# massquantity/Ftrl-FFM

Hardware: AMD Instinct MI355X
Metric: train samples/sec + logloss, FFM f=39 k=16 (higher is better)
Workload: dtype f32; 1 GPU; FFM n_fields=39 n_factors=16 nnz=39, Zipf(1.1) ids, block=8192 rows, n_feats=32999967 (247.1 GB of w,n,z per GPU), warm state, reference default hyper-parameters, 64 distinct blocks streamed from page-locked host memory (H2D in the timed region); workload_key=c5|zipf|warm|rows=8192|n_feats=32999967|shards=1, n_feats=32999967, n_feats_reduced_to_fit=False, n_blocks=64

## Files before the change

ftrl-ffm_amd/csrc/engine.hip:

```cpp
#include <hip/hip_runtime.h>

#include <rocprim/device/device_radix_sort.hpp>
#include <rocprim/iterator/counting_iterator.hpp>

#include <algorithm>
#include <cmath>
#include <atomic>
#include <chrono>
#include <condition_variable>
#include <deque>
#include <functional>
#include <memory>
#include <optional>
#include <mutex>
#include <thread>
#include <cstdio>
#include <cstdlib>
#include <cstring>
#include <new>
#include <string>
#include <vector>

#include "../../include/ffm_engine.h"
#include "engine_types.h"
// ... 370 lines not shown
    }
  }
  int submit(std::function<int()> job) {
    if (prof_on) return job();
    {
      std::lock_guard<std::mutex> lock(wmu);
      if (!worker.joinable()) worker = std::thread([this] { worker_main(); });
      wjobs.push_back(std::move(job));
    }
    wcv_job.notify_one();
    return 0;
  }
  int worker_error() {
    if (worker_rc == 0) return 0;
    const int rc = worker_rc;
    worker_rc = 0;
    return fail(rc, "staging thread: " + worker_msg);
  }
  int drain() {
    std::unique_lock<std::mutex> lock(wmu);
    wcv_done.wait(lock, [&] { return wjobs.empty() && !wbusy; });
    return worker_error();
  }
  int wait_issued(int64_t seq) {
    std::unique_lock<std::mutex> lock(wmu);
    wcv_done.wait(lock, [&] { return staged_issued >= seq || (wjobs.empty() && !wbusy); });
    return worker_error();
  }
  void stop_worker() {
    {
      std::lock_guard<std::mutex> lock(wmu);
      wstop = true;
    }
    wcv_job.notify_all();
    if (worker.joinable()) worker.join();
  }
  bool prof_on = false;
  int prof_only = -1;
  std::vector<ProfRec> prof;
  std::vector<hipEvent_t> event_pool;

  template <typename T>
  int alloc(T **p, size_t count) {
    void *q = nullptr;
    if (count == 0) count = 1;
    hipError_t err = hipMalloc(&q, count * sizeof(T));
    if (err != hipSuccess)
      return fail(FFM_E_NOMEM, "hipMalloc of " + std::to_string(count * sizeof(T)) +
                                   " bytes failed: " + hipGetErrorString(err));
    allocs.push_back(q);
    *p = static_cast<T *>(q);
    return FFM_OK;
  }
  template <typename T>
  int grow(T **p, size_t *cap, size_t need) {
    if (*p && *cap >= need) return FFM_OK;
    T *q = nullptr;
    if (int rc = alloc(&q, need)) return rc;
    if (*p) {
      allocs.erase(std::find(allocs.begin(), allocs.end(), static_cast<void *>(*p)));
      (void)hipFree(*p);
    }
    *p = q;
    *cap = need;
    return FFM_OK;
  }

  hipEvent_t get_event() {
    if (!event_pool.empty()) {
      hipEvent_t e = event_pool.back();
      event_pool.pop_back();
      return e;
    }
    hipEvent_t e = nullptr;
    if (hipEventCreate(&e) != hipSuccess) return nullptr;
    return e;
  }
  void prof_begin(int kid, hipStream_t st) {
    prof_skip = !prof_on || (prof_only >= 0 && kid != prof_only);
    if (prof_skip) return;
    ProfRec r{kid, get_event(), get_event()};
    if (!r.e0 || !r.e1) {
      if (r.e0) event_pool.push_back(r.e0);
      if (r.e1) event_pool.push_back(r.e1);
      prof_skip = true;
      return;
    }
    (void)hipEventRecord(r.e0, st);
    prof.push_back(r);
  }
  bool prof_skip = true;
  void prof_end(hipStream_t st) {
    if (prof_skip) return;
    (void)hipEventRecord(prof.back().e1, st);
  }
};

static inline bool serving(const ffm_engine *e) { return e->m.lat_fmt != SERVE_NONE; }
static int serve_refuse(const char *what) {
  return fail(FFM_E_UNSUPPORTED, std::string("a serving engine holds no accumulators: ") + what + " needs a training engine");
}
#define SERVE_REFUSE(e, what) do { if ((e) && serving(e)) return serve_refuse(what); } while (0)

#define LAUNCH_ON(e, st, kid, kernel, grid, block, shmem, ...)                   \
  do {                                                                           \
    (e)->prof_begin(kid, st);                                                    \
    hipLaunchKernelGGL(kernel, dim3(grid), dim3(block), shmem, st, __VA_ARGS__); \
    (e)->prof_end(st);                                                           \
  } while (0)
#define LAUNCH(e, kid, kernel, grid, block, shmem, ...) \
  LAUNCH_ON(e, (e)->stream, kid, kernel, grid, block, shmem, __VA_ARGS__)

static inline int cdiv(int a, int b) { return (a + b - 1) / b; }
static inline int loss_grid(int n_rows) { return std::max(1, std::min(kLossParts, cdiv(n_rows, 1024))); }

static int tile_nf(const ffm_engine *e) {
  const int k = e->m.n_factors, spc = k <= 64 ? 64 / k : 1;
  return spc > 8 ? 4 : spc > 4 ? 2 : 1;
}
static bool flat_pays(const ffm_engine *e, int span4) {
  if (e->m.n_shards <= 1 || span4 <= 0) return false;
  const int lanes = (span4 + 63) / 64 * 64;
  return span4 * 6 < lanes * 5;
}

extern "C" {

int ffm_engine_abi_version(void) { return FFM_ENGINE_ABI_VERSION; }
int ffm_engine_block_segment(void) { return ftrl_dev::kSeg; }
const char *ffm_engine_last_error(void) { return g_last_error.c_str(); }

void ffm_engine_default_config(ffm_engine_config *cfg) {
  if (!cfg) return;
  std::memset(cfg, 0, sizeof(*cfg));
  cfg->model_type = FFM_MODEL_FFM;
  cfg->n_feats = 10000;
  cfg->n_fields = 8;
  cfg->n_factors = 16;
  cfg->w_alpha = 1e-4f;
  cfg->w_beta = 1.0f;
  cfg->w_l1 = 0.1f;
  cfg->w_l2 = 5.0f;
  cfg->init_mean = 0.0f;
  cfg->init_stddev = 0.02f;
  cfg->seed = 42;
  cfg->max_batch_rows = 8192;
  cfg->max_batch_nnz = 8192 * 64;
  cfg->device_id = 0;
  cfg->n_shards = 1;
  cfg->shard_rank = 0;
}

int64_t ffm_engine_row_len(const ffm_engine *e) { return e ? e->logical_len : 0; }

void ffm_engine_destroy(ffm_engine *e) {
  if (!e) return;
  (void)hipSetDevice(e->cfg.device_id);
  e->stop_worker();
  if (e->prep) (void)hipStreamSynchronize(e->prep);
  if (e->aux3) (void)hipStreamSynchronize(e->aux3);
  if (e->ev_fork) (void)hipEventDestroy(e->ev_fork);
  if (e->ev_fork2) (void)hipEventDestroy(e->ev_fork2);
  if (e->ev_join) (void)hipEventDestroy(e->ev_join);
  if (e->ev_join2) (void)hipEventDestroy(e->ev_join2);
  if (e->aux4) (void)hipStreamDestroy(e->aux4);
  if (e->stream) (void)hipStreamSynchronize(e->stream);
  for (auto &r : e->prof) { (void)hipEventDestroy(r.e0); (void)hipEventDestroy(r.e1); }
  for (auto ev : e->event_pool) (void)hipEventDestroy(ev);
  for (auto &sl : e->slots) {
    if (sl.pinned) (void)hipHostFree(sl.pinned);
    if (sl.pinned_w) (void)hipHostFree(sl.pinned_w);
    if (sl.ev_copied) (void)hipEventDestroy(sl.ev_copied);
    if (sl.ev_trained) (void)hipEventDestroy(sl.ev_trained);
  }
  for (void *p : e->allocs) (void)hipFree(p);
  for (int i = 0; i < ffm_engine::kSets; i++) {
    if (e->ev_grouped[i]) (void)hipEventDestroy(e->ev_grouped[i]);
    if (e->ev_set_free[i]) (void)hipEventDestroy(e->ev_set_free[i]);
    if (e->ev_row_done[i]) (void)hipEventDestroy(e->ev_row_done[i]);
  }
  if (e->h_pulled) (void)hipHostFree(e->h_pulled);
  if (e->h_scored) (void)hipHostFree(e->h_scored);
  if (e->h_super) (void)hipHostFree(e->h_super);
  if (e->prep) (void)hipStreamDestroy(e->prep);

  if (e->aux3) (void)hipStreamDestroy(e->aux3);
  if (e->own_stream && e->stream) (void)hipStreamDestroy(e->stream);
  delete e;
}

#include "engine_create.h"

static int eval_launch_pending(ffm_engine *e);
static int serve_vec_transfer(ffm_engine *e, float *host, bool to_host);
static int serve_rows_vec_transfer(ffm_engine *e, int nf, float *host, bool to_host);

int ffm_engine_init_weights_host(uint64_t seed, float init_mean, float init_stddev, int32_t latent,
                                 int64_t first, int64_t count, float *out) {
  if (first < 0 || count < 0 || (count > 0 && !out)) return fail(FFM_E_INVALID, "bad range or null output");
  for (int64_t j = 0; j < count; j++)
    out[j] = ftrl_rng::init_weight(seed, latent ? 1 : 0, static_cast<uint64_t>(first + j), init_mean, init_stddev);
  return FFM_OK;
}

int ffm_engine_fill_state(ffm_engine *e, uint64_t seed, float n_lo, float n_hi, float z_stddev) {
  if (!e) return fail(FFM_E_INVALID, "null engine");
  SERVE_REFUSE(e, "ffm_engine_fill_state");
  if (!(n_lo >= 0.0f) || !(n_hi >= n_lo)) return fail(FFM_E_INVALID, "need 0 <= n_lo <= n_hi");
  HIP_TRY(hipSetDevice(e->cfg.device_id));
  if (int rc_e = eval_launch_pending(e)) return rc_e;
  hipLaunchKernelGGL(fill_state_kernel, dim3(2048), dim3(256), 0, e->stream, e->m, e->logical_len, seed, n_lo, n_hi, z_stddev);
  HIP_TRY(hipGetLastError());
  HIP_TRY(hipStreamSynchronize(e->stream));
  return FFM_OK;
}

int ffm_engine_eval_sigmoid(ffm_engine *e, int32_t n, const float *x, float *y) {
  if (!e || n < 0 || (n > 0 && (!x || !y))) return fail(FFM_E_INVALID, "bad argument");
  HIP_TRY(hipSetDevice(e->cfg.device_id));
  const int chunk = static_cast<int>(std::min<int64_t>(e->stage_floats / 2, 1 << 22));
  for (int off = 0; off < n; off += chunk) {
    const int c = std::min(chunk, n - off);
    HIP_TRY(hipMemcpyAsync(e->d_stage, x + off, sizeof(float) * c, hipMemcpyHostToDevice, e->stream));
    hipLaunchKernelGGL(sigmoid_eval_kernel, dim3(cdiv(c, 256)), dim3(256), 0, e->stream, c, e->d_stage, e->d_stage + chunk);
    HIP_TRY(hipMemcpyAsync(y + off, e->d_stage + chunk, sizeof(float) * c, hipMemcpyDeviceToHost, e->stream));
    HIP_TRY(hipStreamSynchronize(e->stream));
  }
  return FFM_OK;
}

static int check_device_errors(ffm_engine *e) {
  int flags = 0;
  if (int rc_e = eval_launch_pending(e)) return rc_e;
  if (int rc_w = e->drain()) return rc_w;
  for (int i = 0; i < e->n_staged; i++) HIP_TRY(hipEventSynchronize(e->slots[e->staged[i]].ev_copied));
  HIP_TRY(hipMemcpyAsync(&flags, e->d_err, sizeof(int), hipMemcpyDeviceToHost, e->stream));
  HIP_TRY(hipStreamSynchronize(e->stream));
  if (flags) HIP_TRY(hipMemsetAsync(e->d_err, 0, sizeof(int), e->stream));
  if (flags & ERR_ROW_TOO_LONG)
    return fail(FFM_E_CAPACITY, "a row has more entries than max_row_nnz: its block was not trained "
                                "(outputs of that block are NaN)");
  if (flags & ERR_FIELD_MAP)
    return fail(FFM_E_INVALID, "an entry's feature id lies outside its field's id range (field_start): "
                               "its block was not trained");
  if (flags & ERR_SORT_BARRIER)
    return fail(FFM_E_DEVICE, "the grouping's one-launch sort could not get its workgroups on the device "
                              "together (grid barrier timed out): its block was not trained; FFM_OWN_SORT=0 "
                              "selects the library sort");
  if (flags) return fail(FFM_E_DEVICE, "device error flags " + std::to_string(flags));
  return FFM_OK;
}

int ffm_engine_sync(ffm_engine *e) {
  if (!e) return fail(FFM_E_INVALID, "null engine");
  HIP_TRY(hipSetDevice(e->cfg.device_id));
  return check_device_errors(e);
}

int ffm_engine_check_errors(ffm_engine *e) { return ffm_engine_sync(e); }

void *ffm_engine_stream(ffm_engine *e) { return e ? static_cast<void *>(e->stream) : nullptr; }

int32_t ffm_engine_default_batch_ramp(float w_alpha) {
  if (!(w_alpha > 1e-3f)) return 32;
  const double r = 32.0 * std::pow(8.0, std::log10(static_cast<double>(w_alpha) / 1e-3));
  return static_cast<int32_t>(std::min(r, 1048576.0) + 0.5);
}

int ffm_engine_shard_plan(int32_t n_fields, int32_t n_shards, int32_t field_map, int32_t *pair_owner,
                          int32_t *lin_owner, int32_t *bias_owner) {
  if (n_fields <= 0 || n_shards <= 0) return fail(FFM_E_INVALID, "n_fields and n_shards must be positive");
  const ShardPlan p = make_shard_plan(n_fields, n_shards, field_map != 0);
  for (int fa = 0; fa < n_fields; fa++)
    for (int fb = 0; fb < n_fields; fb++) {
      int owner = -1, count = 0;
      for (int r = 0; r < n_shards; r++)
        if (p.owns(r, fa, fb)) { owner = r; count++; }
      if (count != 1 || !p.owns(owner, fb, fa)) return fail(FFM_E_UNSUPPORTED, "no field-pair partition for this shape");
      if (pair_owner) pair_owner[static_cast<size_t>(fa) * n_fields + fb] = owner;
    }
  if (lin_owner) for (int f = 0; f < n_fields; f++) lin_owner[f] = p.lin_owner[f];
  if (bias_owner) *bias_owner = p.bias_owner;
  return FFM_OK;
}

#include "engine_state.h"
#include "engine_hash.h"
#include "engine_step.h"
#include "engine_stage.h"
#include "engine_refresh.h"
#include "engine_serve.h"
#include "engine_profile.h"
#include "engine_metrics.h"
#include "engine_keyed.h"
#include "engine_sketch.h"
#include "engine_ablate.h"
}

#include "engine_group.h"
```

ftrl-ffm_amd/csrc/engine_create.h:

```cpp

static int hash_ids_check(int32_t model_type, int32_t n_feats, int32_t n_fields, const int32_t *field_start);
static int serve_create_check(const ffm_engine_config *cfg);

struct Switches {
  bool hash_ids = false;
  int metrics = 0;
  char row_refresh = 0;
  std::optional<bool> serial, super_wait, prep_after_row, pull_after_row, eval_defer_off, predict_waves, few_stage, own_sort;
  std::optional<int> update_split, update_order, wide_max_nnz, grid_pull, grid_push, grid_hot, grid_small, grid_walk, grid_giant;
  std::optional<int> row_threads, row_park, row_park_budget, row_hold, super_min;
  std::optional<int> range_sort;
};
extern "C++" {
template <typename T, typename U>
static void take(T &dst, const std::optional<U> &v) { if (v) dst = static_cast<T>(*v); }
template <typename Fn>
static int lds_opt_in(Fn *kernel, size_t bytes) {
  if (kernel) HIP_TRY(hipFuncSetAttribute(reinterpret_cast<const void *>(kernel), hipFuncAttributeMaxDynamicSharedMemorySize, static_cast<int>(bytes)));
  return FFM_OK;
}
template <typename T>
static int upload(ffm_engine *e, const std::vector<T> &host, T **dev) {
  if (int rc = e->alloc(dev, host.size())) return rc;
  HIP_TRY(hipMemcpy(*dev, host.data(), host.size() * sizeof(T), hipMemcpyHostToDevice));
  return FFM_OK;
}
}

static Switches read_switches() {
  Switches sw;
  if (const char *sv = std::getenv("FFM_ENGINE_HASH_IDS")) sw.hash_ids = sv[0] == '1';
  if (const char *sv = std::getenv("FFM_ENGINE_METRICS")) sw.metrics = std::atoi(sv) & 3;
  if (const char *sv = std::getenv("FFM_ENGINE_ROW_REFRESH")) sw.row_refresh = sv[0];
  if (const char *sv = std::getenv("FFM_ENGINE_SERIAL")) sw.serial = sv[0] == '1';
  if (const char *sv = std::getenv("FFM_UPDATE_SPLIT")) sw.update_split = std::atoi(sv);
  if (const char *sv = std::getenv("FFM_UPDATE_ORDER")) {
    const int o = std::atoi(sv);
    const int d0 = o % 10, d1 = o / 10 % 10, d2 = o / 100;
    if (o >= 0 && d2 <= 2 && d0 <= 2 && d1 <= 2 && d0 != d1 && d0 != d2 && d1 != d2) sw.update_order = o;
  }
  if (const char *sv = std::getenv("FFM_SUPER_WAIT")) sw.super_wait = sv[0] != '0';
  if (const char *sv = std::getenv("FFM_PREP_AFTER_ROW")) sw.prep_after_row = sv[0] == '1';
  if (const char *sv = std::getenv("FFM_PULL_AFTER_ROW")) sw.pull_after_row = sv[0] == '1';
  if (const char *sv = std::getenv("FFM_EVAL_DEFER")) sw.eval_defer_off = sv[0] == '0';
  if (const char *sv = std::getenv("FFM_PREDICT_WAVE")) sw.predict_waves = std::atoi(sv) != 0;
  if (const char *sv = std::getenv("FFM_WIDE_NNZ")) sw.wide_max_nnz = std::atoi(sv);
  if (const char *sv = std::getenv("FFM_GRID_PULL")) sw.grid_pull = std::max(1, std::atoi(sv));
  if (const char *sv = std::getenv("FFM_GRID_PUSH")) sw.grid_push = std::min(24, std::max(1, std::atoi(sv)));
  if (const char *sv = std::getenv("FFM_GRID_HOT")) sw.grid_hot = std::max(1, std::atoi(sv));
  if (const char *sv = std::getenv("FFM_GRID_SMALL")) sw.grid_small = std::max(1, std::atoi(sv));
  if (const char *sv = std::getenv("FFM_GRID_WALK")) sw.grid_walk = std::max(1, std::atoi(sv));
  if (const char *sv = std::getenv("FFM_GRID_GIANT")) sw.grid_giant = std::max(1, std::atoi(sv));
  if (const char *sv = std::getenv("FFM_ROW_THREADS")) sw.row_threads = std::max(64, std::min(kRowMaxThreads, std::atoi(sv) / 64 * 64));
  if (const char *sv = std::getenv("FFM_ROW_PARK")) sw.row_park = std::atoi(sv);
  if (const char *sv = std::getenv("FFM_ROW_PARK_BUDGET")) sw.row_park_budget = std::atoi(sv);
  if (const char *sv = std::getenv("FFM_ROW_HOLD")) sw.row_hold = std::max(0, std::atoi(sv));
  if (const char *sv = std::getenv("FFM_SUPER_MIN")) sw.super_min = std::max(kGiantMin, std::atoi(sv));
  if (const char *sv = std::getenv("FFM_FEW_STAGE")) sw.few_stage = sv[0] != '0';
  if (const char *sv = std::getenv("FFM_OWN_SORT")) sw.own_sort = std::atoi(sv) != 0;
  if (const char *sv = std::getenv("FFM_RANGE_SORT")) sw.range_sort = std::atoi(sv);
  return sw;
}

static int check_config(const ffm_engine_config *cfg, bool hash_ids) {
  if (cfg->model_type < FFM_MODEL_LR || cfg->model_type > FFM_MODEL_FFM)
    return fail(FFM_E_INVALID, "invalid model_type, expect LR(0), FM(1) or FFM(2)");
  if (cfg->n_feats <= 0) return fail(FFM_E_INVALID, "n_feats must be positive");
  if (cfg->model_type == FFM_MODEL_FFM && cfg->n_fields <= 0)
    return fail(FFM_E_INVALID, "n_fields must be positive for FFM");
  if (cfg->model_type != FFM_MODEL_LR && cfg->n_factors <= 0)
    return fail(FFM_E_INVALID, "n_factors must be positive for FM/FFM");
  if (cfg->model_type == FFM_MODEL_FM && cfg->n_factors > kTermsCap)
    return fail(FFM_E_UNSUPPORTED, "FM n_factors above 2048 is not supported");
  if (cfg->max_batch_rows <= 0 || cfg->max_batch_nnz <= 0)
    return fail(FFM_E_INVALID, "max_batch_rows / max_batch_nnz must be positive");
  if (cfg->n_shards < 1 || cfg->shard_rank < 0 || cfg->shard_rank >= cfg->n_shards)
    return fail(FFM_E_INVALID, "invalid n_shards / shard_rank");
  if (cfg->n_shards > 1 && cfg->model_type != FFM_MODEL_FFM)
    return fail(FFM_E_UNSUPPORTED, "field-pair sharding applies to FFM only");
  if (cfg->n_shards > 1 && cfg->n_fields > 64)
    return fail(FFM_E_UNSUPPORTED, "field-pair sharding supports up to 64 fields");
  if (cfg->flags & (FFM_FLAG_SERVE_F32 | FFM_FLAG_SERVE_F16))
    if (int rc_s = serve_create_check(cfg)) return rc_s;
  if (hash_ids)
    if (int rc_h = hash_ids_check(cfg->model_type, cfg->n_feats, cfg->n_fields, cfg->field_start)) return rc_h;
  int n_dev = 0;
  if (hipGetDeviceCount(&n_dev) != hipSuccess || n_dev <= 0)
    return fail(FFM_E_DEVICE, "no HIP device available (this library has no CPU fallback)");
  if (cfg->device_id < 0 || cfg->device_id >= n_dev)
    return fail(FFM_E_INVALID, "device_id out of range");
  HIP_TRY(hipSetDevice(cfg->device_id));
  return FFM_OK;
}

static void apply_switches(ffm_engine *e, const Switches &sw) {
  const ffm_engine_config *cfg = &e->cfg;
  take(e->serial, sw.serial);
  take(e->update_split, sw.update_split);
  take(e->update_order, sw.update_order);
  take(e->super_wait, sw.super_wait);
  take(e->prep_after_row, sw.prep_after_row);
  take(e->eval_defer_off, sw.eval_defer_off);
  take(e->predict_waves, sw.predict_waves);
  take(e->wide_max_nnz, sw.wide_max_nnz);
  take(e->grid_pull, sw.grid_pull);
  take(e->grid_push, sw.grid_push);
  take(e->grid_hot, sw.grid_hot);
  take(e->grid_small, sw.grid_small);
  take(e->grid_walk, sw.grid_walk);
  take(e->grid_giant, sw.grid_giant);
  if (cfg->n_shards > 1) e->row_threads = 64;
  take(e->row_threads, sw.row_threads);
  take(e->row_park, sw.row_park);
  take(e->row_park_budget, sw.row_park_budget);
  take(e->row_hold, sw.row_hold);
  if (cfg->n_shards > 1) e->grid_single = 1152;
  if (cfg->n_shards > 1 && !sw.grid_small) e->grid_small = 1024;
  const char rr = sw.row_refresh;
  const int64_t per = cfg->n_factors % 4 == 0 ? static_cast<int64_t>(cfg->n_fields) * cfg->n_factors / 4
                                              : static_cast<int64_t>(cfg->n_fields) * cfg->n_factors;
  e->pre_refresh = cfg->model_type == FFM_MODEL_FFM && cfg->n_fields <= 64 &&
                   static_cast<int64_t>(e->max_nnz) * per < (1ll << 31) && rr != '1';
  if (rr == '0') e->refresh_mode = 1;
  if (rr == '2') e->refresh_mode = 2;
  if (rr == '3') e->refresh_mode = 3;
}

static int plan_model(ffm_engine *e, const Switches &sw, ShardPlan *plan) {
  const ffm_engine_config *cfg = &e->cfg;
  ModelDev &m = e->m;
  m.type = cfg->model_type;
  m.n_feats = cfg->n_feats;
  m.n_fields = cfg->model_type == FFM_MODEL_FFM ? cfg->n_fields : 1;
  m.n_factors = cfg->model_type == FFM_MODEL_LR ? 0 : cfg->n_factors;
  e->logical_len = cfg->model_type == FFM_MODEL_FFM ? cfg->n_fields * cfg->n_factors
                   : cfg->model_type == FFM_MODEL_FM ? cfg->n_factors : 0;
  m.n_shards = cfg->n_shards;
  m.shard_rank = cfg->shard_rank;
  m.bias_own = 1;
  m.huge_min = kHugeMin;
  m.giant_min = cfg->model_type == FFM_MODEL_FM ? kFmGiantMin : kGiantMin;
  m.range_len = cfg->model_type == FFM_MODEL_FM ? kFmRange : kRange;
  m.huge_min = std::min(m.huge_min, m.giant_min - 1);
  m.super_min = kSuperMin;
  take(m.super_min, sw.super_min);
  m.few_stage = 1;
  take(m.few_stage, sw.few_stage);
  m.lat_fmt = (cfg->flags & FFM_FLAG_SERVE_F32 ? SERVE_F32 : 0) | (cfg->flags & FFM_FLAG_SERVE_F16 ? SERVE_F16 : 0);
  m.rec_slots = m.n_fields;
  e->n_records = cfg->n_feats;
  const bool compact = cfg->n_shards > 1 && cfg->field_start != nullptr;
  if (cfg->field_start && cfg->model_type == FFM_MODEL_FFM) {
    e->field_start.assign(cfg->field_start, cfg->field_start + cfg->n_fields + 1);
    bool ok = e->field_start[0] == 0 && e->field_start[cfg->n_fields] == cfg->n_feats;
    for (int f = 0; f < cfg->n_fields; f++) ok = ok && e->field_start[f] <= e->field_start[f + 1];
    if (!ok) return fail(FFM_E_INVALID, "field_start must ascend from 0 to n_feats");
  }
  if (cfg->n_shards > 1) {
    *plan = make_shard_plan(cfg->n_fields, cfg->n_shards, compact);
    m.bias_own = plan->bias_owner == cfg->shard_rank ? 1 : 0;
    if (compact) {
      int widest = 1;
      for (int f = 0; f < cfg->n_fields; f++) widest = std::max(widest, plan->n(cfg->shard_rank, f));
      m.rec_slots = widest;
      e->n_records = 0;
      for (int f = 0; f < cfg->n_fields; f++)
        if (plan->n(cfg->shard_rank, f) > 0) e->n_records += e->field_start[f + 1] - e->field_start[f];
      if (e->n_records == 0) e->n_records = 1;
    }
  }
  m.row_len = cfg->model_type == FFM_MODEL_FFM ? m.rec_slots * cfg->n_factors
              : cfg->model_type == FFM_MODEL_FM ? cfg->n_factors : 0;
  m.h = Hyper{cfg->w_alpha, cfg->w_beta, cfg->w_l1, cfg->w_l2, 1.0f / cfg->w_alpha, 0,
              (cfg->flags & FFM_FLAG_LEARN) ? 1 : 0};
  if (static_cast<int64_t>(cfg->n_fields) * cfg->n_factors > (1 << 24))
    return fail(FFM_E_UNSUPPORTED, "n_fields*n_factors too large");
  if (static_cast<int64_t>(cfg->max_batch_nnz) / (kSmallMax + 1) * ((m.row_len + 7) / 8 + 1) >= (1ll << 31))
    return fail(FFM_E_UNSUPPORTED, "max_batch_nnz * row_len too large for 32-bit work-item ids");
  return FFM_OK;
}

static int create_streams(ffm_engine *e) {
  if (e->cfg.stream) {
    e->stream = static_cast<hipStream_t>(e->cfg.stream);
  } else {
    HIP_TRY(hipStreamCreateWithFlags(&e->stream, hipStreamNonBlocking));
    e->own_stream = true;
  }
  HIP_TRY(hipStreamCreateWithFlags(&e->aux3, hipStreamNonBlocking));
  HIP_TRY(hipStreamCreateWithFlags(&e->aux4, hipStreamNonBlocking));
  HIP_TRY(hipStreamCreateWithFlags(&e->prep, hipStreamNonBlocking));
  for (hipEvent_t *ev : {&e->ev_fork, &e->ev_fork2, &e->ev_join, &e->ev_join2})
    HIP_TRY(hipEventCreateWithFlags(ev, hipEventDisableTiming));
  for (int i = 0; i < ffm_engine::kSets; i++) {
    HIP_TRY(hipEventCreateWithFlags(&e->ev_grouped[i], hipEventDisableTiming));
    HIP_TRY(hipEventCreateWithFlags(&e->ev_set_free[i], hipEventDisableTiming));
    HIP_TRY(hipEventCreateWithFlags(&e->ev_row_done[i], hipEventDisableTiming));
  }
  return FFM_OK;
}

static int alloc_model(ffm_engine *e, const ShardPlan &plan) {
  const ffm_engine_config *cfg = &e->cfg;
  ModelDev &m = e->m;
  int rc;
  const size_t nf = static_cast<size_t>(cfg->n_feats);
  const size_t n_w = static_cast<size_t>(e->n_records) * static_cast<size_t>(m.row_len);
  const size_t n_lat = m.lat_fmt == SERVE_F16 ? n_w / 2 : m.lat_fmt == SERVE_F32 ? n_w : 3 * n_w;
  const size_t n_bias = serving(e) ? 1 : 4;
  if ((rc = e->alloc(&m.bias3, n_bias))) return rc;
  HIP_TRY(hipMemsetAsync(m.bias3, 0, n_bias * sizeof(float), e->stream));
  for (float **lin : {&m.lin_n, &m.lin_z, &m.lin_w}) {
    if (serving(e) && lin != &m.lin_w) continue;
    if ((rc = e->alloc(lin, nf))) return rc;
    HIP_TRY(hipMemsetAsync(*lin, 0, nf * sizeof(float), e->stream));
  }
  if ((rc = e->alloc(&m.lat, n_lat))) return rc;
  if (n_lat) HIP_TRY(hipMemsetAsync(m.lat, 0, n_lat * sizeof(float), e->stream));
  if (m.type == FFM_MODEL_FFM && m.n_fields <= 64) {
    std::vector<unsigned long long> own(m.n_fields, 0ull);
    for (int fa = 0; fa < m.n_fields; fa++)
      for (int fb = 0; fb < m.n_fields; fb++)
        if (m.n_shards <= 1 || plan.owns(m.shard_rank, fa, fb)) own[fa] |= 1ull << fb;
    if ((rc = upload(e, own, &e->d_ownmask))) return rc;
    m.ownmask = e->d_ownmask;
  }
  if (m.n_shards > 1) {
    const bool compact = cfg->field_start != nullptr;
    const int F = m.n_fields, r = m.shard_rank;
    std::vector<int> lo(F), cnt(F), lin(F);
    std::vector<long long> base(F, -1);
    long long next = 0;
    for (int f = 0; f < F; f++) {
      lo[f] = plan.lo(r, f);
      cnt[f] = plan.n(r, f);
      lin[f] = plan.lin_owner[f] == r ? 1 : 0;
      if (compact && cnt[f] > 0) { base[f] = next; next += e->field_start[f + 1] - e->field_start[f]; }
    }
    int *d_lo = nullptr, *d_n = nullptr, *d_lin = nullptr;
    if ((rc = upload(e, lo, &d_lo)) || (rc = upload(e, cnt, &d_n)) || (rc = upload(e, lin, &d_lin))) return rc;
    m.own_lo = d_lo;
    m.own_n = d_n;
    m.lin_own = d_lin;
    e->lin_any = std::any_of(lin.begin(), lin.end(), [](int v) { return v != 0; });
    if (compact) {
      int *d_fs = nullptr;
      long long *d_base = nullptr;
      if ((rc = upload(e, e->field_start, &d_fs)) || (rc = upload(e, base, &d_base))) return rc;
      m.field_start = d_fs;
      m.rec_base = d_base;
    }
  }
  if (e->hash_ids) {
    e->hm = ftrl_hash::Map{nullptr, cfg->n_feats, m.n_fields, m.type == FFM_MODEL_FFM ? 1 : 0};
    if (!e->field_start.empty()) {
      if ((rc = upload(e, e->field_start, &e->d_hash_start))) return rc;
      e->hm.start = e->d_hash_start;
    }
  }
  return FFM_OK;
}

static int alloc_shared(ffm_engine *e, Scratch *shared) {
  const ffm_engine_config *cfg = &e->cfg;
  const ModelDev &m = e->m;
  Scratch &s = *shared;
  int rc;
  const size_t R = static_cast<size_t>(e->max_rows), E = static_cast<size_t>(e->max_nnz);
  const size_t max_segs = E / kSeg + E / kFmGiantMin + 2, rl = static_cast<size_t>(std::max(1, m.row_len));
  const bool lat_model = cfg->model_type != FFM_MODEL_LR, ffm_m = cfg->model_type == FFM_MODEL_FFM;
  const size_t chunks = !ffm_m ? 1 : cfg->n_factors <= 64
                            ? (static_cast<size_t>(m.rec_slots) + 64 / cfg->n_factors - 1) / (64 / cfg->n_factors)
                            : static_cast<size_t>(m.rec_slots) * ((cfg->n_factors + 63) / 64);
  if ((rc = e->alloc(&s.segP, lat_model ? max_segs * rl : 1)) || (rc = e->alloc(&s.segG, lat_model ? max_segs * rl : 1)) ||
      (rc = e->alloc(&s.segD, ffm_m ? max_segs * rl : 1)) || (rc = e->alloc(&s.segF, ffm_m ? max_segs * chunks * 3 : 1)) ||
      (rc = e->alloc(&s.gcap, ffm_m ? (E / kGiantMin + 2) * rl : 1)))
    return rc;
  if ((rc = e->alloc(&e->d_err, 1))) return rc;
  HIP_TRY(hipMemsetAsync(e->d_err, 0, sizeof(int), e->stream));
  s.err = e->d_err;
  if ((rc = e->alloc(&s.head, R * static_cast<size_t>(m.n_fields))) || (rc = e->alloc(&s.next, E)) ||
      (rc = e->alloc(&s.rowtab, R * static_cast<size_t>(m.n_fields))) || (rc = e->alloc(&s.logit, R)) ||
      (rc = e->alloc(&s.tg, R)) || (rc = e->alloc(&s.loss, R)) ||
      (rc = e->alloc(&s.svx, R * static_cast<size_t>(m.type == FFM_MODEL_FM ? m.n_factors : 1))))
    return rc;
  e->sort_bits = 1;
  while (e->sort_bits < 32 && (static_cast<uint64_t>(cfg->n_feats) >> e->sort_bits) != 0) e->sort_bits++;
  unsigned *no_key = nullptr;
  int *no_occ = nullptr;
  HIP_TRY(rocprim::radix_sort_pairs<GroupSortConfig>(nullptr, e->sort_tmp_bytes, no_key, no_key,
                                    rocprim::counting_iterator<int>(0), no_occ, E, 0u, e->sort_bits, e->stream));
  e->sort_tmp_bytes = std::max(e->sort_tmp_bytes, sort_scratch_bytes(E));
  HIP_TRY(hipHostMalloc(reinterpret_cast<void **>(&e->h_super), sizeof(int) * ffm_engine::kSets, hipHostMallocMapped));
  std::memset(e->h_super, 0, sizeof(int) * ffm_engine::kSets);
  HIP_TRY(hipHostGetDevicePointer(reinterpret_cast<void **>(&s.n_super), e->h_super, 0));
  hipLaunchKernelGGL(host_word_probe_kernel, dim3(1), dim3(64), 0, e->stream, s.n_super, ffm_engine::kSets);
  HIP_TRY(hipStreamSynchronize(e->stream));
  e->super_flag_ok = true;
  for (int si = 0; si < ffm_engine::kSets; si++) e->super_flag_ok = e->super_flag_ok && e->h_super[si] == 0x5eed + si;
  std::memset(e->h_super, 0, sizeof(int) * ffm_engine::kSets);
  if ((rc = e->alloc(&e->d_ids, static_cast<size_t>(ffm_engine::kIdsCap))) || (rc = e->alloc(&e->d_row_ptr, R + 1)) ||
      (rc = e->alloc(&e->d_field, E)) || (rc = e->alloc(&e->d_feat, E)) || (rc = e->alloc(&e->d_val, E)) ||
      (rc = e->alloc(&e->d_label, R)) || (rc = e->alloc(&e->d_out, R)) || (rc = e->alloc(&e->d_loss_sum, 2)) ||
      (rc = e->alloc(&e->d_loss_part, kLossParts + 1)))
    return rc;
  HIP_TRY(hipMemsetAsync(e->d_loss_part, 0, sizeof(double) * (kLossParts + 1), e->stream));
  e->stage_floats = 16 << 20;
  if (static_cast<int64_t>(e->logical_len) > e->stage_floats) e->stage_floats = e->logical_len;
  return e->alloc(&e->d_stage, static_cast<size_t>(e->stage_floats));
}

static int alloc_set(ffm_engine *e, int si, const Scratch &shared) {
  const ModelDev &m = e->m;
  Scratch &t = e->sc[si];
  t = shared;
  t.n_super = shared.n_super + si;
  int rc;
  const size_t R = static_cast<size_t>(e->max_rows), E = static_cast<size_t>(e->max_nnz);
  if ((rc = e->alloc(&t.key, E)) || (rc = e->alloc(&t.skey, E)) || (rc = e->alloc(&t.row_of, E)) ||
      (rc = e->alloc(&t.occ, E)) || (rc = e->alloc(&t.occ2, E)) || (rc = e->alloc(&t.udesc, E)) ||
      (rc = e->alloc(&t.small, E)) || (rc = e->alloc(&t.few, E)) || (rc = e->alloc(&t.sdesc, E)) ||
      (rc = e->alloc(&t.big, E)) || (rc = e->alloc(&t.huge, E)) || (rc = e->alloc(&t.giant, E / kChainMin + 1)) ||
      (rc = e->alloc(&t.gseg, E / kChainMin + 1)) || (rc = e->alloc(&t.grange, E / kFmRange + E / kFmGiantMin + 2)) ||
      (rc = e->alloc(&t.counters, kNumCounters)) || (rc = e->alloc(&t.occpos, E)) || (rc = e->alloc(&t.uflag, E)))
    return rc;
  if (m.type == FFM_MODEL_FFM && m.n_fields <= 64)
    if ((rc = e->alloc(&t.rowmask, 2 * R)) || (rc = e->alloc(&t.gmask, E)) || (rc = e->alloc(&t.cmask, E))) return rc;
  unsigned char *tmp = nullptr;
  if ((rc = e->alloc(&tmp, e->sort_tmp_bytes))) return rc;
  e->d_sort_tmp[si] = tmp;
  HIP_TRY(hipMemsetAsync(t.counters, 0, kNumCounters * sizeof(int), e->stream));
  return FFM_OK;
}

static int choose_sort(ffm_engine *e, const Switches &sw) {
  const ffm_engine_config *cfg = &e->cfg;
  ModelDev &m = e->m;
  const double per_row = e->max_rows > 0 ? static_cast<double>(e->max_nnz) / e->max_rows : 0.0;
  const double phase_us = static_cast<double>(e->max_nnz) * std::max(0.0, per_row - 1.0) * m.n_factors / 0.44e6;
  const bool ffm4 = m.type == FFM_MODEL_FFM && m.n_factors % 4 == 0;
  e->own_sort = !(ffm4 && phase_us / std::max(1, m.n_shards) >= 100.0);
  take(e->own_sort, sw.own_sort);
  const bool have = !e->field_start.empty(), forced = sw.range_sort.has_value();
  const bool quick = cfg->n_shards == 1 && static_cast<int64_t>(e->max_nnz) <= 16384ll * std::max(1, cfg->n_fields);
  const bool want = forced ? *sw.range_sort != 0 : (have && quick);
  if (want && (m.type == FFM_MODEL_FFM || forced)) {
    const int nr = have ? cfg->n_fields : (forced && *sw.range_sort > 1 ? std::min(1024, *sw.range_sort) : std::max(1, std::min(64, cfg->n_fields)));
    std::vector<int> st(static_cast<size_t>(nr) + 1);
    for (int f = 0; f <= nr; f++)
      st[f] = have ? e->field_start[f] : static_cast<int>(static_cast<int64_t>(cfg->n_feats) * f / nr);
    if (int rc = upload(e, st, &e->d_sort_start)) return rc;
    e->n_sort_ranges = nr;
    e->range_sort = true;
    if (have && m.type == FFM_MODEL_FFM) m.sort_start = e->d_sort_start;
    if (!sw.prep_after_row) e->prep_after_row = !e->own_sort;
    e->pull_after_row = e->prep_after_row && static_cast<int64_t>(e->max_nnz) * m.n_factors >= (1ll << 22);
    take(e->pull_after_row, sw.pull_after_row);
  }
  hipDeviceProp_t prop;
  HIP_TRY(hipGetDeviceProperties(&prop, cfg->device_id));
  int per_cu = 0;
  HIP_TRY(hipOccupancyMaxActiveBlocksPerMultiprocessor(&per_cu, group_sort_kernel, kSortThreads, 0));
  e->sort_grid_cap = std::max(1, per_cu * prop.multiProcessorCount);
  if (std::strncmp(prop.gcnArchName, "gfx950", 6) != 0 && std::strncmp(prop.gcnArchName, "gfx942", 6) != 0) e->own_sort = false;
  return FFM_OK;
}

static int read_verdict(ffm_engine *e, int *bad) {
  int *counters = e->sc[0].counters;
  HIP_TRY(hipMemcpyAsync(bad, counters, sizeof(int), hipMemcpyDeviceToHost, e->stream));
  HIP_TRY(hipStreamSynchronize(e->stream));
  HIP_TRY(hipMemsetAsync(counters, 0, kNumCounters * sizeof(int), e->stream));
  return FFM_OK;
}

static int prove_fast_math(ffm_engine *e) {
  const ffm_engine_config *cfg = &e->cfg;
  ModelDev &m = e->m;
  {
    static std::atomic<int> verdict[64];
    const int dev = cfg->device_id & 63;
    int bad = verdict[dev].load() < 0 ? 1 : 0;
    if (verdict[dev].load() == 0) {
      hipLaunchKernelGGL(verify_sqrt_fast_kernel, dim3(16384), dim3(256), 0, e->stream, e->sc[0].counters);
      if (int rc = read_verdict(e, &bad)) return rc;
      verdict[dev].store(bad ? -1 : 1);
    }
    if (bad)
      return fail(FFM_E_UNSUPPORTED, "this device's v_sqrt_f32 / v_rsq_f32 do not give the correctly rounded "
                                     "square root in the short sequence the kernels use (built and proven for gfx950)");
  }
  if (cfg->w_alpha >= 0x1p-30f && cfg->w_alpha <= 0x1p30f) {
    int bad = 0;
    Hyper probe = m.h;
    probe.fast_div = 1;
    hipLaunchKernelGGL(verify_div_alpha_kernel, dim3(1u << 17), dim3(256), 0, e->stream, probe, e->sc[0].counters);
    if (int rc = read_verdict(e, &bad)) return rc;
    m.h.fast_div = bad ? 0 : 1;
    m.h.fast_w = m.h.fast_div && cfg->w_beta >= 0x1p-40f && cfg->w_beta <= 0x1p40f ? 1 : 0;
  }
  return FFM_OK;
}

static int opt_in_lds(ffm_engine *e) {
  int rc;
  const size_t lds = row_lds_bytes(e->max_row_nnz, e->m.n_fields, kTermsCap);
  if (lds > 150 * 1024) return fail(FFM_E_UNSUPPORTED, "max_row_nnz too large for the 160 KB of LDS per workgroup");
  const size_t park_budget = static_cast<size_t>(std::max(0, e->row_park_budget));
  if (lds > 32 * 1024 || park_budget > 32 * 1024) {
    const size_t bytes = std::max(lds, park_budget);
    for (int train = 0; train < 2; train++) {
      if ((rc = lds_opt_in(fm_row_fn(train), bytes))) return rc;
      for (int vec4 = 0; vec4 < 2; vec4++)
        for (int whole = 0; whole < 2; whole++)
          for (int hold = 0; hold <= 8; hold++)
            if ((rc = lds_opt_in(ffm_row_fn<>(train, vec4, whole, hold), bytes)) ||
                (rc = lds_opt_in(ffm_row_fn<const float *>(train, vec4, whole, hold), bytes)))
              return rc;
    }
  }
  for (int nf = 1; nf <= 4; nf *= 2)
    for (int kinds = 1; kinds <= UPD_ALL; kinds++)
      for (int waves : {tile_waves(nf), kWideWaves})
        if ((rc = lds_opt_in(update_all_fn(nf, kinds, waves), tile_lds_bytes(nf, waves)))) return rc;
  return FFM_OK;
}

static int init_weights(ffm_engine *e) {
  const ffm_engine_config *cfg = &e->cfg;
  const bool skip = (cfg->flags & FFM_FLAG_SKIP_INIT) != 0;
  if (!skip && serving(e))
    hipLaunchKernelGGL(serve_init_kernel, dim3(2048), dim3(256), 0, e->stream, e->m, cfg->init_mean, cfg->init_stddev, cfg->seed);
  else if (!skip)
    hipLaunchKernelGGL(init_weights_kernel, dim3(2048), dim3(256), 0, e->stream, e->m, e->logical_len,
                       cfg->init_mean, cfg->init_stddev, cfg->seed);
  HIP_TRY(hipGetLastError());
  HIP_TRY(hipStreamSynchronize(e->stream));
  return FFM_OK;
}

int ffm_engine_create(const ffm_engine_config *cfg, ffm_engine **out) {
  if (!cfg || !out) return fail(FFM_E_INVALID, "null config or output pointer");
  *out = nullptr;
  const Switches sw = read_switches();
  const bool hash_ids = (cfg->flags & FFM_FLAG_HASH_IDS) != 0 || sw.hash_ids;
  if (int rc_c = check_config(cfg, hash_ids)) return rc_c;
  std::unique_ptr<ffm_engine, void (*)(ffm_engine *)> guard(new (std::nothrow) ffm_engine, ffm_engine_destroy);
  ffm_engine *e = guard.get();
  if (!e) return fail(FFM_E_NOMEM, "host allocation failed");
  e->cfg = *cfg;
  if (hash_ids) e->cfg.flags |= FFM_FLAG_HASH_IDS;
  e->hash_ids = hash_ids;
  e->max_rows = cfg->max_batch_rows;
  e->max_nnz = cfg->max_batch_nnz;
  if (cfg->max_row_nnz > 0) e->max_row_nnz = cfg->max_row_nnz;
  else if (cfg->flags & (FFM_FLAG_SERVE_F32 | FFM_FLAG_SERVE_F16)) e->max_row_nnz = kPredLdsCap;
  apply_switches(e, sw);
  ShardPlan plan;
  Scratch shared{};
  int rc;
  if ((rc = plan_model(e, sw, &plan)) || (rc = create_streams(e)) || (rc = alloc_model(e, plan)) || (rc = alloc_shared(e, &shared)))
    return rc;
  for (int si = 0; si < ffm_engine::kSets; si++)
    if ((rc = alloc_set(e, si, shared))) return rc;
  if ((rc = choose_sort(e, sw)) || (rc = prove_fast_math(e)) || (rc = opt_in_lds(e)) || (rc = init_weights(e))) return rc;
  if (sw.metrics && cfg->shard_rank == 0)
    if ((rc = ffm_engine_metrics_enable(e, sw.metrics))) return rc;
  *out = guard.release();
  return FFM_OK;
}
```

ftrl-ffm_amd/csrc/engine_step.h:

```cpp


static int eval_launch_pending(ffm_engine *e);
static void launch_metric(ffm_engine *e, int channel, int n_rows, const float *score, int is_prob, const int *label);
static void launch_keyed(ffm_engine *e, int channel, const Rows &rows, const float *score, int is_prob);
__global__ void loss_accumulate_kernel(double *acc, const double *one) { *acc += *one; }

static int check_block(ffm_engine *e, int32_t n_rows, int32_t nnz, const void *row_ptr,
                       const void *field, const void *feat, const void *val, bool implicit_fields = false,
                       bool implicit_ones = false, bool hold_eval = false) {
  if (!e) return fail(FFM_E_INVALID, "null engine");
  if (e->eval_pending.on && !hold_eval)
    if (int rc_e = eval_launch_pending(e)) return rc_e;
  if (n_rows < 0 || nnz < 0) return fail(FFM_E_INVALID, "negative n_rows / nnz");
  if (n_rows > e->max_rows || nnz > e->max_nnz)
    return fail(FFM_E_CAPACITY, "block exceeds max_batch_rows / max_batch_nnz");
  if (!row_ptr || (nnz > 0 && (!feat || (!val && !implicit_ones)))) return fail(FFM_E_INVALID, "null CSR array");
  if (e->m.type == FFM_MODEL_FFM && nnz > 0 && !field && !implicit_fields)
    return fail(FFM_E_INVALID, "FFM requires the field array (libffm rows)");
  return FFM_OK;
}


static bool launch_row_waves(ffm_engine *e, const Rows &rows, int row_cap, float *out, int output_prob) {
  const ModelDev &m = e->m;
// ... 138 lines not shown
  const int set = (e->last_set + 1) % ffm_engine::kSets;
  pl->set = set;
  pl->rows = rows;
  pl->wait_free = e->set_used[set];
  const int ws = e->trained_set[e->n_prepared >= 1 ? 0 : 1];
  pl->ws = ws >= 0 && ws != set ? ws : -1;
  e->set_used[set] = true;
  e->last_set = set;
  e->prepared_set[e->n_prepared] = set;
  e->prepared_rows[e->n_prepared] = rows;
  e->n_prepared++;
  return FFM_OK;
}
static int prepare_submit(ffm_engine *e, const PrepPlan &pl, bool timed) {
  HIP_TRY(hipSetDevice(e->cfg.device_id));
  if (pl.wait_free) HIP_TRY(hipStreamWaitEvent(e->prep, e->ev_set_free[pl.set], 0));
  if (pl.ws >= 0) HIP_TRY(hipStreamWaitEvent(e->prep, e->prep_after_row ? e->ev_row_done[pl.ws] : e->ev_set_free[pl.ws], 0));
  int rc = launch_grouping(e, pl.set, pl.rows, e->prep, timed);
  if (rc) return rc;
  HIP_TRY(hipEventRecord(e->ev_grouped[pl.set], e->prep));
  return FFM_OK;
}

int ffm_engine_prepare_device(ffm_engine *e, int32_t n_rows, int32_t nnz, const int32_t *row_ptr,
                              const int32_t *field, const int32_t *feat, const float *val) {
  SERVE_REFUSE(e, "ffm_engine_prepare_device");
  int rc = check_block(e, n_rows, nnz, row_ptr, field, feat, val);
  if (rc) return rc;
  if ((rc = e->drain())) return rc;
  PrepPlan pl;
  if ((rc = prepare_plan(e, Rows{n_rows, nnz, row_ptr, field, feat, val, nullptr}, &pl))) return rc;
  return prepare_submit(e, pl, true);
}

struct ForwardOpts {
  int row_cap = 0;
  bool whole_step = false;
  float *logit_out = nullptr;
};

static int train_forward_core(ffm_engine *e, const Rows &rows, const float *weight, float *partial_logit,
                              const ForwardOpts &opts) {
  ScopedTimer tm_fwd("train:forward");
  SERVE_REFUSE(e, "training");
  const int32_t n_rows = rows.n_rows;
  int rc = check_block(e, n_rows, rows.nnz, rows.row_ptr, rows.field, rows.feat, rows.val);
  if (rc) return rc;
  if (n_rows > 0 && !rows.label) return fail(FFM_E_INVALID, "training needs labels");
  HIP_TRY(hipSetDevice(e->cfg.device_id));
  e->pending = rows;
  e->pending_weight = n_rows > 0 ? weight : nullptr;
  e->has_pending = true;
  e->own_tg_cur = opts.whole_step && e->m.n_shards == 1 &&
                  (e->m.type != FFM_MODEL_FM || e->m.n_factors <= 64);
  const bool use_prepared = e->n_prepared > 0 && same_block(e->prepared_rows[0], rows);
  if (e->n_prepared > 0 && !use_prepared) {
    if ((rc = e->drain())) return rc;
    for (int i = 0; i < e->n_prepared; i++) HIP_TRY(hipEventRecord(e->ev_set_free[e->prepared_set[i]], e->prep));
    e->n_prepared = 0;
  }
  e->cur_prepared = use_prepared;
  if (use_prepared) {
    e->cur = e->prepared_set[0];
    for (int i = 1; i < e->n_prepared; i++) {
      e->prepared_set[i - 1] = e->prepared_set[i];
      e->prepared_rows[i - 1] = e->prepared_rows[i];
    }
    e->n_prepared--;
    HIP_TRY(hipStreamWaitEvent(e->stream, e->ev_grouped[e->cur], 0));
  } else {
    e->cur = (e->last_set + 1) % ffm_engine::kSets;
    e->last_set = e->cur;
    if (e->set_used[e->cur]) HIP_TRY(hipStreamWaitEvent(e->stream, e->ev_set_free[e->cur], 0));
    rc = launch_grouping(e, e->cur, rows, e->stream);
    if (rc) return rc;
  }
  e->set_used[e->cur] = true;
  launch_row_kernel(e, rows, opts.row_cap, true, e->own_tg_cur ? opts.logit_out : nullptr, 0, e->own_tg_cur ? 1 : 0, e->pending_weight);
  if (e->prep_after_row) HIP_TRY(hipEventRecord(e->ev_row_done[e->cur], e->stream));
  if (partial_logit && n_rows > 0)
    HIP_TRY(hipMemcpyAsync(partial_logit, e->sc[e->cur].logit, sizeof(float) * n_rows, hipMemcpyDeviceToDevice, e->stream));
  HIP_TRY(hipGetLastError());
  return FFM_OK;
}

int ffm_engine_train_forward_device(ffm_engine *e, int32_t n_rows, int32_t nnz,
                                    const int32_t *row_ptr, const int32_t *field,
                                    const int32_t *feat, const float *val, const int32_t *label,
                                    float *partial_logit) {
  return train_forward_core(e, Rows{n_rows, nnz, row_ptr, field, feat, val, label}, nullptr, partial_logit, ForwardOpts{});
}
int ffm_engine_train_forward_device_weighted(ffm_engine *e, int32_t n_rows, int32_t nnz,
                                             const int32_t *row_ptr, const int32_t *field,
                                             const int32_t *feat, const float *val, const int32_t *label,
                                             const float *weight, float *partial_logit) {
  return train_forward_core(e, Rows{n_rows, nnz, row_ptr, field, feat, val, label}, weight, partial_logit, ForwardOpts{});
}

int ffm_engine_train_update_device(ffm_engine *e, const float *logit, float *logit_out,
                                   double *loss_sum_out) {
  if (!e) return fail(FFM_E_INVALID, "null engine");
  SERVE_REFUSE(e, "training");
  if (!e->has_pending) return fail(FFM_E_INVALID, "train_update without a preceding train_forward");
  ScopedTimer tm_upd("train:update");
  HIP_TRY(hipSetDevice(e->cfg.device_id));
  const Rows rows = e->pending;
  e->has_pending = false;
  const float *lg = logit ? logit : e->sc[e->cur].logit;
  const bool own_tg = e->own_tg_cur && !logit;
  launch_metric(e, FFM_METRIC_TRAIN, rows.n_rows, lg, 0, rows.label);
  launch_keyed(e, FFM_METRIC_TRAIN, rows, lg, 0);
  if (rows.n_rows > 0 && !own_tg) {
    if (e->pending_weight)
      LAUNCH(e, K_TMP_GRAD, tmp_grad_weighted_kernel, cdiv(rows.n_rows, 256), 256, 0, rows.n_rows, lg, rows.label, e->pending_weight, e->sc[e->cur].tg, e->sc[e->cur].loss, logit_out);
    else
      LAUNCH(e, K_TMP_GRAD, tmp_grad_kernel, cdiv(rows.n_rows, 256), 256, 0, rows.n_rows, lg, rows.label, e->sc[e->cur].tg, e->sc[e->cur].loss, logit_out);
  }
  e->pending_weight = nullptr;
  const int fm_in_row = e->m.type == FFM_MODEL_FM && own_tg && e->singles_in_row ? 1 : 0;
  const bool lin_owner = e->m.bias_own != 0 || e->lin_any;
  const bool ffm = e->m.type == FFM_MODEL_FFM && rows.nnz > 0;
  const bool vec4 = e->m.n_factors % 4 == 0;
  const bool masks = e->sc[e->cur].cmask != nullptr;
  const int lin_blocks = rows.nnz > 0 ? std::min(cdiv(rows.nnz, kUpdThreads), 1024) : 0;
  const int side_blocks = lin_owner && rows.n_rows > 0 ? 1 + lin_blocks : 0;
  bool loss_done = false;
  if (ffm && vec4 && masks) {
    const int span4 = e->m.rec_slots * (e->m.n_factors / 4);
    const bool flat = flat_pays(e, span4);
    const bool side_launches = !e->singles_in_row || flat;
    hipStream_t sst = side_launches && !e->serial ? e->aux3 : e->stream;
    if (sst != e->stream) {
      HIP_TRY(hipEventRecord(e->ev_fork, e->stream));
      HIP_TRY(hipStreamWaitEvent(sst, e->ev_fork, 0));
    }
    if (!e->singles_in_row) {
      if (flat) LAUNCH_ON(e, sst, K_LATENT_UPDATE_SINGLE, ffm_update_single_flat_kernel, e->grid_single, kUpdThreads, 0, e->m, rows, e->sc[e->cur]);
      else LAUNCH_ON(e, sst, K_LATENT_UPDATE_SINGLE, update_single_fn(span4), e->grid_single, kUpdThreads, 0, e->m, rows, e->sc[e->cur]);
    }
    bool supers = rows.nnz >= e->m.super_min;
    if (supers && e->super_flag_ok && e->cur_prepared) {
      if (e->super_wait) HIP_TRY(hipEventSynchronize(e->ev_grouped[e->cur]));
      if (hipEventQuery(e->ev_grouped[e->cur]) == hipSuccess && e->h_super[e->cur] == 0) supers = false;
    }
    const bool few_late = flat && sst != e->stream && supers;
    if (flat && !few_late) LAUNCH_ON(e, sst, K_LATENT_UPDATE_FEW, ffm_update_small_flat_kernel, e->grid_small, kUpdThreads, 0, e->m, rows, e->sc[e->cur], 1);
    if (sst != e->stream && !few_late) HIP_TRY(hipEventRecord(e->ev_join, sst));
    const int split = e->update_split >= 0 ? e->update_split
                      : (!side_launches && static_cast<int64_t>(rows.nnz) * e->m.n_factors >= (1ll << 20) ? 2 : 0);
    const int nf = tile_nf(e);
    const bool wide = nf == 1 && !side_launches && split == 0 && rows.nnz < e->wide_max_nnz;
    const int wpb = wide ? kWideWaves : tile_waves(nf), scale = wpb / kUpdWaves, threads = 64 * wpb;
    const size_t lds = tile_lds_bytes(nf, wpb);
    const size_t few_lds = few_stage_possible(e->m) ? few_stage_bytes(wpb, e->m.n_fields) : 0;
    auto sized = [&](int grid, int per_wg, int least) { return std::max(least, std::min(grid, cdiv(rows.nnz, per_wg))); };
    const int nt = cdiv(sized(e->grid_hot, 32, 64), scale), ns = flat ? 0 : cdiv(sized(e->grid_small, 128, 64), scale);
    const int nw = cdiv(sized(e->grid_walk, 1024, 16), scale);
    const int ng = rows.nnz >= kGiantMin ? sized(e->grid_giant, 256, 32) : 0;
    const int order = e->update_order;
    const int lb = loss_sum_out ? loss_grid(rows.n_rows) : 0;
    const int side = side_blocks > 0 ? 1 + cdiv(lin_blocks, scale) : 0;
    auto launch_ranges = [&](hipStream_t st, int kid, int kinds, size_t shm, int ord) {
      const int a_side = kinds & UPD_SIDE ? side : 0, a_ng = kinds & UPD_GIANT ? ng : 0, a_nt = kinds & UPD_HOT ? nt : 0;
      const int a_ns = kinds & UPD_FEW ? ns : 0, a_nw = kinds & UPD_REST ? nw : 0, a_lb = kinds & UPD_REST ? lb : 0;
      LAUNCH_ON(e, st, kid, update_all_fn(nf, kinds, wpb), a_side + a_ng + a_nt + a_ns + a_nw + a_lb, threads, shm, e->m, rows,
                e->sc[e->cur], a_side, a_ng, a_nt, a_ns, 1, a_nw, a_lb, loss_sum_out, e->d_loss_part, ord);
    };
    if (split == 2 && !e->serial) {
      HIP_TRY(hipEventRecord(e->ev_fork2, e->stream));
      if (ns + nw + lb > 0) {
        HIP_TRY(hipStreamWaitEvent(e->aux3, e->ev_fork2, 0));
        launch_ranges(e->aux3, K_LATENT_UPDATE_FEW, UPD_FEW | UPD_REST, few_lds, order);
        HIP_TRY(hipEventRecord(e->ev_join, e->aux3));
      }
      if (ng > 0) {
        HIP_TRY(hipStreamWaitEvent(e->aux4, e->ev_fork2, 0));
        launch_ranges(e->aux4, K_LATENT_UPDATE_GIANT, UPD_GIANT, lds, order);
        HIP_TRY(hipEventRecord(e->ev_join2, e->aux4));
      }
      launch_ranges(e->stream, K_LATENT_UPDATE, UPD_HOT | UPD_SIDE, lds, 1);
      if (ns + nw + lb > 0) HIP_TRY(hipStreamWaitEvent(e->stream, e->ev_join, 0));
      if (ng > 0) HIP_TRY(hipStreamWaitEvent(e->stream, e->ev_join2, 0));
    } else if (split) {
      if (ng > 0) launch_ranges(e->stream, K_LATENT_UPDATE_GIANT, UPD_GIANT, lds, order);
      launch_ranges(e->stream, K_LATENT_UPDATE, UPD_HOT | UPD_SIDE, lds, order);
      if (ns > 0) launch_ranges(e->stream, K_LATENT_UPDATE_FEW, UPD_FEW, lds, order);
      launch_ranges(e->stream, K_LATENT_UPDATE_WALK, UPD_REST, lds, order);
    } else if (ns == 0) {
      launch_ranges(e->stream, K_LATENT_UPDATE, UPD_ALL & ~UPD_FEW, lds, order);
    } else {
      launch_ranges(e->stream, K_LATENT_UPDATE, UPD_ALL, lds, order);
    }
    if (few_late) {
      HIP_TRY(hipEventRecord(e->ev_fork2, e->stream));
      HIP_TRY(hipStreamWaitEvent(sst, e->ev_fork2, 0));
      LAUNCH_ON(e, sst, K_LATENT_UPDATE_FEW, ffm_update_small_flat_kernel, e->grid_small, kUpdThreads, 0, e->m, rows, e->sc[e->cur], 1);
      HIP_TRY(hipEventRecord(e->ev_join, sst));
    }
    if (supers) {
      const int gg = e->grid_giant;
      e->prof_begin(K_LATENT_UPDATE_GIANT, e->stream);
      hipLaunchKernelGGL(update_super_b_fn(nf), dim3(gg), dim3(kUpdThreads), 0, e->stream, e->m, rows, e->sc[e->cur]);
      hipLaunchKernelGGL(ffm_update_super_join_kernel, dim3(gg), dim3(kUpdThreads), 0, e->stream, e->m, e->sc[e->cur]);
      e->prof_end(e->stream);
    }
    if (sst != e->stream) HIP_TRY(hipStreamWaitEvent(e->stream, e->ev_join, 0));
    loss_done = loss_sum_out != nullptr;
  } else {
    if (side_blocks > 0 && e->m.type != FFM_MODEL_FM) {
      LAUNCH(e, K_BIAS_UPDATE, bias_update_kernel, 1, kUpdThreads, 0, e->m, rows.n_rows, e->sc[e->cur]);
      if (rows.nnz > 0)
        LAUNCH(e, K_LINEAR_UPDATE, linear_update_kernel, lin_blocks, kUpdThreads, 0, e->m, rows, e->sc[e->cur], 0);
    }
    if (ffm) {
      LAUNCH(e, K_LATENT_UPDATE, ffm_update_generic_kernel, 2048, kUpdThreads, 0, e->m, rows, e->sc[e->cur], 0);
    } else if (e->m.type == FFM_MODEL_FM) {
      if (rows.nnz > 0) {
        LAUNCH(e, K_LATENT_UPDATE, fm_update_kernel, side_blocks + 2048, kUpdThreads, 0, e->m, rows, e->sc[e->cur], fm_in_row, side_blocks);
        if (rows.nnz >= e->m.giant_min)
          LAUNCH(e, K_LATENT_UPDATE_GIANT, fm_update_join_kernel, 256, kUpdThreads, 0, e->m, e->sc[e->cur]);
      }
      else if (side_blocks > 0)
        LAUNCH(e, K_BIAS_UPDATE, bias_update_kernel, 1, kUpdThreads, 0, e->m, rows.n_rows, e->sc[e->cur]);
    }
  }
  if (loss_sum_out && !loss_done)
    LAUNCH(e, K_LOSS_SUM, loss_sum_kernel, loss_grid(rows.n_rows), 256, 0, rows.n_rows, e->sc[e->cur].loss, loss_sum_out, e->d_loss_part);
  HIP_TRY(hipEventRecord(e->ev_set_free[e->cur], e->stream));
  e->trained_set[1] = e->trained_set[0];
  e->trained_set[0] = e->cur;
  if (e->cur_slot >= 0) {
    e->slots[e->cur_slot].free_ev = e->ev_set_free[e->cur];
    e->cur_slot = -1;
  }
  HIP_TRY(hipGetLastError());
  return FFM_OK;
}

static int train_batch_core(ffm_engine *e, const Rows &rows, const float *weight, float *logit_out, double *loss_sum_out,
                            int row_cap) {
  if (e && e->m.n_shards > 1)
    return fail(FFM_E_INVALID, "sharded engines train with train_forward + all-reduce + train_update");
  int rc = train_forward_core(e, rows, weight, nullptr, ForwardOpts{row_cap, true, logit_out});
  if (rc) return rc;
  return ffm_engine_train_update_device(e, nullptr, logit_out, loss_sum_out);
}
int ffm_engine_train_batch_device_weighted(ffm_engine *e, int32_t n_rows, int32_t nnz,
                                           const int32_t *row_ptr, const int32_t *field,
                                           const int32_t *feat, const float *val, const int32_t *label,
                                           const float *weight, float *logit_out, double *loss_sum_out) {
  return train_batch_core(e, Rows{n_rows, nnz, row_ptr, field, feat, val, label}, weight, logit_out, loss_sum_out, 0);
}
int ffm_engine_train_batch_device(ffm_engine *e, int32_t n_rows, int32_t nnz,
                                  const int32_t *row_ptr, const int32_t *field,
                                  const int32_t *feat, const float *val, const int32_t *label,
                                  float *logit_out, double *loss_sum_out) {
  return ffm_engine_train_batch_device_weighted(e, n_rows, nnz, row_ptr, field, feat, val, label, nullptr, logit_out,
                                                loss_sum_out);
}

static int predict_core(ffm_engine *e, const Rows &rows, int32_t output_prob, float *out, double *loss_sum_out, int row_cap) {
  const int32_t n_rows = rows.n_rows;
  const int32_t *const label = rows.label;
  int rc = check_block(e, n_rows, rows.nnz, rows.row_ptr, rows.field, rows.feat, rows.val);
  if (rc) return rc;
  if (e->m.n_shards > 1 && (label || output_prob || loss_sum_out))
    return fail(FFM_E_INVALID, "a sharded engine predicts partial logits only (label = NULL, output_prob = 0, "
                               "no loss): sum them across shards, then ffm_engine_predict_finish_device");
  HIP_TRY(hipSetDevice(e->cfg.device_id));
  launch_row_kernel(e, rows, row_cap, false, out ? out : e->d_out, output_prob);
  if (label) launch_metric(e, FFM_METRIC_EVAL, n_rows, out ? out : e->d_out, output_prob, label);
  if (label) launch_keyed(e, FFM_METRIC_EVAL, rows, out ? out : e->d_out, output_prob);
  if (loss_sum_out && label)
    LAUNCH(e, K_LOSS_SUM, loss_sum_kernel, loss_grid(n_rows), 256, 0, n_rows, e->sc[e->cur].loss, loss_sum_out, e->d_loss_part);
  HIP_TRY(hipGetLastError());
  return FFM_OK;
}
int ffm_engine_predict_batch_device(ffm_engine *e, int32_t n_rows, int32_t nnz,
                                    const int32_t *row_ptr, const int32_t *field,
                                    const int32_t *feat, const float *val, const int32_t *label,
                                    int32_t output_prob, float *out, double *loss_sum_out) {
  return predict_core(e, Rows{n_rows, nnz, row_ptr, field, feat, val, label}, output_prob, out, loss_sum_out, 0);
}

int ffm_engine_predict_finish_device(ffm_engine *e, int32_t n_rows, const float *logit,
                                     const int32_t *label, int32_t output_prob, float *out,
                                     double *loss_sum_out) {
  if (!e) return fail(FFM_E_INVALID, "null engine");
  if (n_rows < 0 || n_rows > e->max_rows) return fail(FFM_E_CAPACITY, "n_rows out of range");
  if (n_rows > 0 && !logit) return fail(FFM_E_INVALID, "null logit array");
  HIP_TRY(hipSetDevice(e->cfg.device_id));
  if (label) launch_metric(e, FFM_METRIC_EVAL, n_rows, logit, 0, label);
  if (n_rows > 0)
    LAUNCH(e, K_TMP_GRAD, predict_finish_kernel, cdiv(n_rows, 256), 256, 0, n_rows, logit, label, output_prob, out, e->sc[e->cur].loss);
  if (loss_sum_out) {
    if (label) LAUNCH(e, K_LOSS_SUM, loss_sum_kernel, loss_grid(n_rows), 256, 0, n_rows, e->sc[e->cur].loss, loss_sum_out, e->d_loss_part);
    else HIP_TRY(hipMemsetAsync(loss_sum_out, 0, sizeof(double), e->stream));
  }
  HIP_TRY(hipGetLastError());
  return FFM_OK;
}

static int validate_host_block(ffm_engine *e, int32_t n_rows, const int32_t *row_ptr,
                               const int32_t **field_io, const int32_t *feat, const float *val,
                               int32_t *nnz_out, int *longest_out, bool implicit_fields = false, bool hold_eval = false) {
  if (!e) return fail(FFM_E_INVALID, "null engine");
  if (e->m.type != FFM_MODEL_FFM) *field_io = nullptr;
  const int32_t *const field = *field_io;
  if (n_rows < 0) return fail(FFM_E_INVALID, "negative n_rows");
  if (!row_ptr) return fail(FFM_E_INVALID, "null row_ptr");
  if (n_rows > e->max_rows) return fail(FFM_E_CAPACITY, "block exceeds max_batch_rows");
  if (row_ptr[0] != 0) return fail(FFM_E_INVALID, "row_ptr[0] must be 0");
  for (int r = 0; r < n_rows; r++)
    if (row_ptr[r + 1] < row_ptr[r]) return fail(FFM_E_INVALID, "row_ptr must be non-decreasing");
  const int32_t nnz = row_ptr[n_rows];
// ... 108 lines not shown
```

ftrl-ffm_amd/csrc/engine_types.h:

```cpp
#pragma once
#include <stdint.h>

#include "ftrl_math.h"

namespace ftrl_dev {

struct Rows {
  int n_rows;
  int nnz;
  const int *row_ptr;
  const int *field;
  const int *feat;
  const float *val;
  const int *label;
};

struct ModelDev {
  int type;
  int n_feats;
  int n_fields;
  int n_factors;
  int row_len;
  int rec_slots;
  int n_shards, shard_rank;
  Hyper h;
  float *bias3;
  float *lin_n, *lin_z, *lin_w;
  float *lat;
  const unsigned long long *ownmask;
  const int *own_lo, *own_n;
  const int *field_start;
  const long long *rec_base;
  const int *lin_own;
  int bias_own;
  int huge_min;
  int giant_min;
  int super_min;
  const int *sort_start;
  int range_len;
  int few_stage;
  int lat_fmt;
};

enum { LAT_N = 0, LAT_Z = 1, LAT_W = 2 };

typedef float v4f_nt __attribute__((ext_vector_type(4)));
__device__ __forceinline__ float4 load_nt(const float4 *p) {
  const v4f_nt v = __builtin_nontemporal_load(reinterpret_cast<const v4f_nt *>(p));
  return make_float4(v.x, v.y, v.z, v.w);
}
__device__ __forceinline__ void store_nt(float4 *p, float4 x) {
  const v4f_nt v = {x.x, x.y, x.z, x.w};
  __builtin_nontemporal_store(v, reinterpret_cast<v4f_nt *>(p));
}


__device__ __forceinline__ bool owns_pair(const ModelDev &m, int fa, int fb) {
  if (!m.own_n) return true;
  return static_cast<unsigned>(fb - m.own_lo[fa]) < static_cast<unsigned>(m.own_n[fa]);
}
__device__ __forceinline__ unsigned long long owner_bits(const ModelDev &m, int fp) {
  return m.own_n ? m.ownmask[fp] : ~0ull;
}
__device__ __forceinline__ bool owns_bit(unsigned long long own_bits, int fa) {
  return (own_bits >> (fa & 63)) & 1ull;
}
__device__ __forceinline__ bool owns_linear(const ModelDev &m, int fa) {
  return !m.lin_own || m.lin_own[fa] != 0;
}
__device__ __forceinline__ bool keeps_field(const ModelDev &m, int fa) {
  return !m.field_start || m.own_n[fa] > 0 || m.lin_own[fa] != 0;
}

__device__ __forceinline__ float *lat_row(const ModelDev &m, int feat, int fa) {
  const long long rec = m.field_start ? m.rec_base[fa] + (feat - m.field_start[fa]) : feat;
  return m.lat + rec * 3 * m.row_len;
}
__device__ __forceinline__ int slot_of(const ModelDev &m, int fa, int fb) {
  return m.field_start ? fb - m.own_lo[fa] : fb;
}
__device__ __forceinline__ long long w_slot_offset(const ModelDev &m, int feat, int fa, int fb) {
  const long long rec = m.field_start ? m.rec_base[fa] + (feat - m.field_start[fa]) : feat;
  return rec * 3 * m.row_len + LAT_W * m.row_len + slot_of(m, fa, fb) * m.n_factors;
}

__device__ __forceinline__ int record_span(const ModelDev &m, int unit) { return m.rec_slots * unit; }
__device__ __forceinline__ int walk_field(const ModelDev &m, int fa, int c) {
  if (!m.field_start) return c < m.n_fields ? c : -1;
  return c < m.own_n[fa] ? m.own_lo[fa] + c : -1;
}

struct Scratch {
  unsigned *key;
  unsigned *skey;
  int *row_of;
  int *occ;
  int2 *occ2;
  int4 *udesc;
  int *small;
  int4 *sdesc;
  int *few;
  int *big;
  int *huge;
  int *giant;
  int *gseg;
  int2 *grange;
  float *segP, *segG, *segD;
  unsigned long long *segF;
  float *gcap;
  int *counters;
  int *n_super;
  int *err;
  int *head;
  int *next;
  int4 *rowtab;
  unsigned long long *rowmask;
  unsigned long long *gmask;
  unsigned long long *cmask;
  int *uflag;
  int *occpos;
  float *logit;
  float *tg;
  double *loss;
  float *svx;
};

enum { UF_DUP = 1 };

constexpr int kSeg = 16;

constexpr int kLineInts = 16;
enum { CNT_NUNIQ = 0, CNT_CURSOR = 1 * kLineInts, CNT_NMULTI = 2 * kLineInts, CNT_ERROR = 3 * kLineInts,
       CNT_NSMALL = 4 * kLineInts, CNT_NBIG = 5 * kLineInts, CNT_NHUGE = 6 * kLineInts,
       CNT_NFEW = 7 * kLineInts, CNT_NSINGLE = 9 * kLineInts, CNT_NGIANT = 10 * kLineInts,
       CNT_SORT_BAR = 11 * kLineInts,
       CNT_NSEG = 12 * kLineInts, CNT_NRANGE = 13 * kLineInts,
       CNT_IRREGULAR = 14 * kLineInts };
constexpr int kNumCounters = 15 * kLineInts;
enum { OCC_FEW = -1, OCC_ONCE = -2 };
#ifndef FFM_HUGE_MIN
#define FFM_HUGE_MIN 128
#endif
constexpr int kHugeMin = FFM_HUGE_MIN;
#ifndef FFM_RANGE_SEGS
#define FFM_RANGE_SEGS 16
#endif
constexpr int kRangeSegs = FFM_RANGE_SEGS;
constexpr int kRange = kRangeSegs * kSeg;
constexpr int kGiantMin = kRange + 1;
constexpr int kFmRange = 64, kFmGiantMin = kFmRange + 1;
#ifndef FFM_SUPER_MIN
#define FFM_SUPER_MIN 2048
#endif
constexpr int kSuperMin = FFM_SUPER_MIN;
constexpr int kChainMin = 64;
#ifndef FFM_SMALL_MAX
#define FFM_SMALL_MAX 10
#endif
constexpr int kSmallMax = FFM_SMALL_MAX;
enum { ERR_ROW_TOO_LONG = 1, ERR_FIELD_MAP = 2, ERR_SORT_BARRIER = 4 };

}
```

ftrl-ffm_amd/csrc/kernels_fold.h:

```cpp
#pragma once
#include "engine_types.h"
#include "kernels_touch.h"

namespace ftrl_dev {

#ifndef FFM_FOLD_BRANCHY
#define FFM_FOLD_BRANCHY 0
#endif

__device__ __forceinline__ bool fold_strict_ok(float x) {
  return __builtin_amdgcn_fmed3f(x, 0x1p-70f, 0x1p96f) == x;
}
__device__ __forceinline__ bool fold_zero_ok(float x) {
  return (__float_as_uint(x) == 0u) | (__builtin_amdgcn_fmed3f(x, 0x1p-70f, 0x1p96f) == x);
}

template <int N>
__device__ __forceinline__ void fold_root_diffs(const float (&arg)[N], const float (&nb)[N], const bool (&need)[N],
                                                float (&d)[N]) {
  bool ok = true;
#pragma unroll
#if FFM_FOLD_BRANCHY
  for (int j = 0; j < N; j++) ok = ok && (!need[j] || (fold_strict_ok(arg[j]) && fold_strict_ok(nb[j])));
#else
  for (int j = 0; j < N; j++) ok = ok & (!need[j] | (static_cast<int>(fold_strict_ok(arg[j])) & static_cast<int>(fold_strict_ok(nb[j]))));
#endif
  if (__all(ok)) {
#pragma unroll
    for (int j = 0; j < N; j++) d[j] = sqrt_fast(arg[j]) - sqrt_fast(nb[j]);
    return;
  }
  ok = true;
#pragma unroll
#if FFM_FOLD_BRANCHY
  for (int j = 0; j < N; j++) ok = ok && (!need[j] || (fold_zero_ok(arg[j]) && fold_zero_ok(nb[j])));
#else
  for (int j = 0; j < N; j++) ok = ok & (!need[j] | (static_cast<int>(fold_zero_ok(arg[j])) & static_cast<int>(fold_zero_ok(nb[j]))));
#endif
  if (__all(ok)) {
#pragma unroll
    for (int j = 0; j < N; j++) d[j] = sqrt_fast0(arg[j]) - sqrt_fast0(nb[j]);
  } else {
#pragma unroll
    for (int j = 0; j < N; j++) d[j] = sqrtf(arg[j]) - sqrtf(nb[j]);
  }
}

struct Fold {
  float P, G, D;
  float B, Gacc, Dacc;
  float ncap;
  bool any, seen, head_plain;
  __device__ __forceinline__ void init(float n0) {
    P = G = D = Gacc = Dacc = -0.0f;
    B = n0;
    ncap = 0.0f;
    any = seen = head_plain = false;
  }
  __device__ __forceinline__ void flush() {
    B = B + P;
    Gacc = Gacc + G;
    Dacc = Dacc + D;
    P = G = D = -0.0f;
  }
  __device__ __forceinline__ void plain(bool live, float g) {
    const float gg = g * g;
    G = live ? G + g : G;
    P = live ? P + gg : P;
    any = any || live;
    head_plain = any;
  }
};

template <int N>
__device__ __forceinline__ void fold_ffm_group(Fold &a, float w, const bool (&live)[N],
                                               const bool (&first)[N], const float (&tg)[N],
                                               const float (&x)[N], const float (&vp)[N]) {
  float g[N], gg[N];
  bool quirk[N], anyq = false;
#pragma unroll
  for (int j = 0; j < N; j++) {
    g[j] = tg[j] * vp[j] * x[j];
    gg[j] = g[j] * g[j];
    quirk[j] = live[j] & !first[j];
    anyq = anyq | quirk[j];
  }
  if (__any(a.seen | anyq)) {
    float arg[N], nb[N], d[N];
    bool need[N];
#pragma unroll
    for (int j = 0; j < N; j++) {
      const float nt = a.B + a.P;
      const bool flip = quirk[j] & !a.seen;
      if (__any(flip)) a.ncap = flip ? nt : a.ncap;
      a.seen = a.seen | flip;
      need[j] = a.seen & live[j];
      const float g1 = tg[j] * w * x[j];
      arg[j] = nt + (first[j] ? gg[j] : g[j] * g1);
      nb[j] = nt;
      a.P = live[j] ? a.P + gg[j] : a.P;
    }
    fold_root_diffs<N>(arg, nb, need, d);
#pragma unroll
    for (int j = 0; j < N; j++) a.D = need[j] ? a.D + d[j] : a.D;
  } else {
#pragma unroll
    for (int j = 0; j < N; j++) a.P = live[j] ? a.P + gg[j] : a.P;
  }
#pragma unroll
  for (int j = 0; j < N; j++) {
    a.G = live[j] ? a.G + g[j] : a.G;
    if (!a.any) a.head_plain = first[j];
    a.any = a.any | live[j];
  }
}

template <int N>
__device__ __forceinline__ void fold_ffm_group_regular(Fold &a, float w, bool lv, bool q118, const float (&tg)[N],
                                                       const float (&x)[N], const float (&vp)[N]) {
  float g[N], gg[N];
#pragma unroll
  for (int j = 0; j < N; j++) {
    g[j] = tg[j] * vp[j] * x[j];
    gg[j] = g[j] * g[j];
  }
  if (__any(q118)) {
    float arg[N], nb[N], d[N];
    bool need[N];
#pragma unroll
    for (int j = 0; j < N; j++) {
      const float nt = a.B + a.P;
      a.ncap = (q118 & !a.seen) ? nt : a.ncap;
      a.seen = a.seen | q118;
      need[j] = q118;
      const float g1 = tg[j] * w * x[j];
      arg[j] = nt + g[j] * g1;
      nb[j] = nt;
      a.P = a.P + gg[j];
    }
    fold_root_diffs<N>(arg, nb, need, d);
#pragma unroll
    for (int j = 0; j < N; j++) a.D = q118 ? a.D + d[j] : a.D;
  } else {
#pragma unroll
    for (int j = 0; j < N; j++) a.P = a.P + gg[j];
  }
#pragma unroll
  for (int j = 0; j < N; j++) a.G = a.G + g[j];
  a.head_plain = a.any ? a.head_plain : !q118;
  a.any = a.any | lv;
}

template <int E>
struct FoldFew {
  float P[E], G[E], D[E], ncap[E];
  bool any, seen, head_plain;
  __device__ __forceinline__ void init() {
#pragma unroll
    for (int i = 0; i < E; i++) { P[i] = G[i] = D[i] = -0.0f; ncap[i] = 0.0f; }
    any = seen = head_plain = false;
  }
  __device__ __forceinline__ void touch(const float (&n0)[E], const float (&w)[E], bool live, bool first,
                                        float tg, float x, const float (&vp)[E]) {
    float g[E], gg[E];
#pragma unroll
    for (int i = 0; i < E; i++) {
      g[i] = tg * vp[i] * x;
      gg[i] = g[i] * g[i];
    }
    const bool quirk = live && !first;
    if (__any(seen || quirk)) {
      const bool flip = quirk && !seen;
      float arg[E], nb[E], d[E];
      bool need[E];
      seen = seen || flip;
#pragma unroll
      for (int i = 0; i < E; i++) {
        const float nt = n0[i] + P[i];
        ncap[i] = flip ? nt : ncap[i];
        const float g1 = tg * w[i] * x;
        arg[i] = nt + (first ? gg[i] : g[i] * g1);
        nb[i] = nt;
        need[i] = seen && live;
      }
      fold_root_diffs<E>(arg, nb, need, d);
#pragma unroll
      for (int i = 0; i < E; i++) D[i] = need[i] ? D[i] + d[i] : D[i];
    }
#pragma unroll
    for (int i = 0; i < E; i++) {
      P[i] = live ? P[i] + gg[i] : P[i];
      G[i] = live ? G[i] + g[i] : G[i];
    }
    if (live && !any) { any = true; head_plain = first; }
  }
  __device__ __forceinline__ void touch_regular(const float (&n0)[E], const float (&w)[E], bool lv, bool q118,
                                                float tg, float x, const float (&vp)[E]) {
    float g[E], gg[E];
#pragma unroll
    for (int i = 0; i < E; i++) {
      g[i] = tg * vp[i] * x;
      gg[i] = g[i] * g[i];
    }
    if (__any(q118)) {
      float arg[E], nb[E], d[E];
      bool need[E];
#pragma unroll
      for (int i = 0; i < E; i++) {
        const float nt = n0[i] + P[i];
        ncap[i] = (q118 & !seen) ? nt : ncap[i];
        const float g1 = tg * w[i] * x;
        arg[i] = nt + g[i] * g1;
        nb[i] = nt;
        need[i] = q118;
      }
      seen = seen | q118;
      fold_root_diffs<E>(arg, nb, need, d);
#pragma unroll
      for (int i = 0; i < E; i++) D[i] = q118 ? D[i] + d[i] : D[i];
    }
#pragma unroll
    for (int i = 0; i < E; i++) {
      P[i] = P[i] + gg[i];
      G[i] = G[i] + g[i];
    }
    head_plain = any ? head_plain : (lv & !q118);
    any = any | lv;
  }
  __device__ __forceinline__ bool finish(const Hyper &h, const float (&w)[E], float (&n)[E], float (&z)[E]) {
    float nT[E], sa[E], sb[E], S[E], q[E];
#pragma unroll
    for (int i = 0; i < E; i++) {
      nT[i] = n[i] + P[i];
      sa[i] = seen ? ncap[i] : nT[i];
      sb[i] = n[i];
    }
    float ra[E], rb[E];
    sqrt_cr_n<E>(sa, ra);
    sqrt_cr_n<E>(sb, rb);
#pragma unroll
    for (int i = 0; i < E; i++) {
      float t = -0.0f;
      t = head_plain ? t + (ra[i] - rb[i]) : t;
      S[i] = t + D[i];
    }
    div_alpha_n<E>(h, S, q);
#pragma unroll
    for (int i = 0; i < E; i++) {
      if (any) {
        z[i] = (z[i] + G[i]) - q[i] * w[i];
        n[i] = nT[i];
      }
    }
    return any;
  }
};

__device__ __forceinline__ bool fold_finish_latent(const Hyper &h, Fold &a, float w, float &n, float &z) {
  a.flush();
  const float ncap = a.seen ? a.ncap : a.B;
  const float hd = sqrt_cr(ncap) - sqrt_cr(n);
  float S = -0.0f;
  S = a.head_plain ? S + hd : S;
  S = S + a.Dacc;
  const float m = div_alpha(h, S) * w;
  if (a.any) {
    z = (z + a.Gacc) - m;
    n = a.B;
  }
  return a.any;
}
__device__ __forceinline__ bool fold_finish_linear(const Hyper &h, Fold &a, float w, float &n, float &z) {
  a.flush();
  const float si = div_alpha(h, sqrt_cr(a.B) - sqrt_cr(n));
  if (a.any) {
    z = z + (a.Gacc - si * w);
    n = a.B;
  }
  return a.any;
}

}
```

ftrl-ffm_amd/csrc/kernels_group.h:

```cpp
#pragma once
#include "engine_types.h"

namespace ftrl_dev {

constexpr int kGroupThreads = 256;
#ifndef FFM_FINISH_THREADS
#define FFM_FINISH_THREADS 256
#endif
constexpr int kFinishThreads = FFM_FINISH_THREADS;

__device__ __forceinline__ int wave_append_slot(int *counter, bool pred) {
  const unsigned long long mask = __ballot(pred);
  const int lane = threadIdx.x & 63;
  const int leader = __ffsll(static_cast<long long>(mask)) - 1;
  int base = 0;
  if (pred && lane == leader) base = atomicAdd(counter, __popcll(mask));
  base = __shfl(base, leader < 0 ? 0 : leader, 64);
  return base + __popcll(mask & ((1ull << lane) - 1ull));
}

__device__ __forceinline__ int wave_reserve(int *counter, int amount) {
  const int lane = threadIdx.x & 63;
  int incl = amount;
#pragma unroll
  for (int d = 1; d < 64; d <<= 1) {
    const int v = __shfl_up(incl, d, 64);
    if (lane >= d) incl += v;
  }
  const int total = __shfl(incl, 63, 64);
  int base = 0;
  if (lane == 63) base = atomicAdd(counter, total);
  base = __shfl(base, 63, 64);
  return base + incl - amount;
}

__global__ __launch_bounds__(kGroupThreads) void group_keys_kernel(ModelDev m, Rows rows, Scratch s,
                                                                   int max_row_nnz) {
  const int pp = blockIdx.x * blockDim.x + threadIdx.x;
  const bool in = pp < rows.nnz;
  const int p = in ? pp : rows.nnz - 1;
  int lo = 0, hi = rows.n_rows;
  while (lo < hi) {
    const int mid = (lo + hi) >> 1;
    if (rows.row_ptr[mid + 1] <= p) lo = mid + 1; else hi = mid;
  }
  const int i = rows.feat[p];
  const int f = rows.field ? rows.field[p] : 0;
  bool valid = i >= 0 && i < m.n_feats;
  if (m.type == 2) valid = valid && f >= 0 && f < m.n_fields;
  if (m.field_start && valid) {
    if (in && (i < m.field_start[f] || i >= m.field_start[f + 1])) {
      atomicOr(&s.counters[CNT_ERROR], ERR_FIELD_MAP);
      atomicOr(s.err, ERR_FIELD_MAP);
    }
    valid = keeps_field(m, f);
  }
  if (m.sort_start) {
    const int b0 = rows.row_ptr[lo];
    bool regular = valid && rows.row_ptr[lo + 1] - b0 == m.n_fields && f == p - b0;
    if (regular) regular = i >= m.sort_start[f] && i < m.sort_start[f + 1];
    if (__any(in && !regular) && (threadIdx.x & 63) == 0) atomicOr(&s.counters[CNT_IRREGULAR], 1);
  }
  if (in) {
    s.row_of[p] = lo;
    s.key[p] = valid ? static_cast<unsigned>(i) : static_cast<unsigned>(m.n_feats);
    s.occpos[p] = OCC_FEW;
    s.uflag[p] = 0;
    if (s.gmask) { s.gmask[p] = 0ull; s.cmask[p] = 0ull; }
  }
  valid = valid && in;
  if (in && p == rows.row_ptr[lo] && rows.row_ptr[lo + 1] - p > max_row_nnz) {
    atomicOr(&s.counters[CNT_ERROR], ERR_ROW_TOO_LONG);
    atomicOr(s.err, ERR_ROW_TOO_LONG);
  }
  if (s.rowmask) {
    const int lane = threadIdx.x & 63;
    unsigned long long once = valid ? 1ull << f : 0ull, twice = 0ull;
    const int prev_row = __shfl_up(lo, 1, 64);
    const unsigned long long starts = __ballot(lane == 0 || prev_row != lo);
    const unsigned long long upto = lane == 63 ? ~0ull : ((2ull << lane) - 1ull);
    const int seg0 = 63 - __clzll(static_cast<long long>(starts & upto));
#pragma unroll
    for (int d = 1; d < 64; d <<= 1) {
      const unsigned long long o = __shfl_up(once, d, 64), w = __shfl_up(twice, d, 64);
      if (lane - d >= seg0) {
        twice |= w | (o & once);
        once |= o;
      }
    }
    const int next_row = __shfl_down(lo, 1, 64);
    if (in && (lane == 63 || next_row != lo || pp == rows.nnz - 1)) {
      if (once) {
        const unsigned long long before = atomicOr(&s.rowmask[2 * lo], once);
        twice |= before & once;
      }
      if (twice) atomicOr(&s.rowmask[2 * lo + 1], twice);
    }
  }
}

__device__ __forceinline__ int sorted_bound(const unsigned *skey, int n, unsigned k, bool strict) {
  int lo = 0, hi = n;
  while (lo < hi) {
    const int mid = (lo + hi) >> 1;
    const unsigned v = skey[mid];
    if (strict ? v <= k : v < k) lo = mid + 1; else hi = mid;
  }
  return lo;
}

__global__ __launch_bounds__(kFinishThreads) void group_finish_kernel(ModelDev m, Rows rows,
                                                                     Scratch s) {
  if (s.counters[CNT_ERROR]) return;
  const int nnz = rows.nnz;
  const int lane = threadIdx.x & 63;
  const int t = blockIdx.x * blockDim.x + threadIdx.x;
  const bool in = t < nnz;
  const unsigned sentinel = static_cast<unsigned>(m.n_feats);
  const unsigned K = in ? s.skey[t] : sentinel;
  const bool valid = in && K < sentinel;
  const unsigned Kprev = (in && t > 0) ? s.skey[t - 1] : 0xffffffffu;
  const unsigned Knext = (t + 1 < nnz) ? s.skey[t + 1] : 0xffffffffu;
  const bool head = valid && (t == 0 || Kprev != K);
  const bool last = valid && Knext != K;
  if (last && Knext >= sentinel) s.counters[CNT_CURSOR] = t + 1;
  const unsigned long long heads = __ballot(head), lasts = __ballot(last);
  const unsigned long long upto = lane == 63 ? ~0ull : ((2ull << lane) - 1ull);
  const unsigned long long from = ~0ull << lane;
  const unsigned long long hb = heads & upto, lb = lasts & from;
  const int hl = hb ? 63 - __clzll(static_cast<long long>(hb)) : -1;
  const int ll = lb ? __ffsll(static_cast<long long>(lb)) - 1 : -1;
  int lower0 = 0, upper63 = 0;
  if (lane == 0 && valid && !head) lower0 = sorted_bound(s.skey, nnz, K, false);
  if (lane == 63 && valid && !last) upper63 = sorted_bound(s.skey, nnz, K, true);
  lower0 = __shfl(lower0, 0, 64);
  upper63 = __shfl(upper63, 63, 64);
  int lower = 0, upper = 0;
  if (valid) {
    lower = hl >= 0 ? t - (lane - hl) : lower0;
    upper = ll >= 0 ? t + (ll - lane) + 1 : upper63;
  }
  const int c = upper - lower;
  int p = 0;
  bool dup = false;
  if (valid) {
    p = s.occ[t];
    const int r = s.row_of[p];
    s.occ2[t] = make_int2(p, r);
    s.occpos[p] = c > kSmallMax ? t : (c == 1 ? OCC_ONCE : OCC_FEW);
    dup = (!head && s.row_of[s.occ[t - 1]] == r) || (!last && s.row_of[s.occ[t + 1]] == r);
    if (dup) atomicOr(&s.uflag[lower], UF_DUP);
  }
  constexpr int kLists = 7;
  __shared__ int wave_cnt[kFinishThreads / 64][kLists];
  __shared__ int wave_base[kFinishThreads / 64][kLists];
  const int wv = threadIdx.x >> 6;
  const bool pred[kLists] = {head, head && c <= kSmallMax, head && c > 1 && c <= kSmallMax,
                             head && c > kSmallMax && c <= m.huge_min,
                             head && c > m.huge_min && c < m.giant_min, head && c == 1,
                             head && c > m.huge_min && c >= m.giant_min};
  const int which[kLists] = {CNT_NUNIQ, CNT_NSMALL, CNT_NFEW, CNT_NBIG, CNT_NHUGE, CNT_NSINGLE, CNT_NGIANT};
  unsigned long long pm[kLists];
#pragma unroll
  for (int q = 0; q < kLists; q++) {
    pm[q] = __ballot(pred[q]);
    if (lane == 0) wave_cnt[wv][q] = __popcll(pm[q]);
  }
  __syncthreads();
  if (threadIdx.x < kLists) {
    const int q = threadIdx.x;
    int total = 0;
    for (int w = 0; w < kFinishThreads / 64; w++) { wave_base[w][q] = total; total += wave_cnt[w][q]; }
    const int base = total ? atomicAdd(&s.counters[which[q]], total) : 0;
    for (int w = 0; w < kFinishThreads / 64; w++) wave_base[w][q] += base;
  }
  __syncthreads();
  int slot[kLists];
  const unsigned long long below = (1ull << lane) - 1ull;
#pragma unroll
  for (int q = 0; q < kLists; q++) slot[q] = wave_base[wv][q] + __popcll(pm[q] & below);
  const int u = slot[0], is = slot[1], iw = slot[2], ib = slot[3], ih = slot[4];
  if (head) {
    const int fld = rows.field ? rows.field[p] : 0;
    s.udesc[u] = make_int4(static_cast<int>(K), t, c, fld);
    if (c == 1) s.sdesc[slot[5]] = make_int4(static_cast<int>(K), p, s.row_of[p], fld);
    if (c > 1 && c <= kSmallMax) s.few[iw] = u;
    if (c <= kSmallMax) s.small[is] = u;
    else if (c <= m.huge_min) s.big[ib] = u;
    else if (c < m.giant_min) s.huge[ih] = u;
    else {
      const int gi = slot[6];
      s.giant[gi] = u;
      if (c >= m.super_min) __hip_atomic_store(s.n_super, 1, __ATOMIC_RELAXED, __HIP_MEMORY_SCOPE_SYSTEM);
      if (m.type != 2 || c >= m.super_min) {
        const int n_seg = (c + kSeg - 1) / kSeg, n_rng = (c + m.range_len - 1) / m.range_len;
        s.gseg[gi] = atomicAdd(&s.counters[CNT_NSEG], n_seg);
        const int rb = atomicAdd(&s.counters[CNT_NRANGE], n_rng);
        for (int r = 0; r < n_rng; r++) s.grange[rb + r] = make_int2(gi, r);
      } else {
        s.gseg[gi] = 0;
      }
    }
  }
  if (s.gmask) {
    unsigned long long tm = 0ull, tc = 0ull;
    if (valid) {
      const int r = s.row_of[p], f = rows.field[p];
      const unsigned long long once = s.rowmask[2 * r], twice = s.rowmask[2 * r + 1];
      const unsigned long long self = 1ull << f;
      tm = ((once & ~self) | (twice & self)) & m.ownmask[f];
      tc = twice & m.ownmask[f];
      if (dup) tc |= tm;
    }
    const int seg0 = hl >= 0 ? hl : 0;
#pragma unroll
    for (int d = 1; d < 64; d <<= 1) {
      const unsigned long long v = __shfl_up(tm, d, 64), vc = __shfl_up(tc, d, 64);
      if (lane - d >= seg0) { tm |= v; tc |= vc; }
    }
    const bool piece_end = valid && (last || lane == 63 || t == nnz - 1);
    if (piece_end) {
      atomicOr(&s.gmask[lower], tm);
      if (tc) atomicOr(&s.cmask[lower], tc);
    }
  }
}

__global__ void host_word_probe_kernel(int *w, int n) {
  if (static_cast<int>(threadIdx.x) < n)
    __hip_atomic_store(w + threadIdx.x, 0x5eed + static_cast<int>(threadIdx.x), __ATOMIC_RELAXED, __HIP_MEMORY_SCOPE_SYSTEM);
}

}
```

ftrl-ffm_amd/csrc/kernels_tile.h:

```cpp
#pragma once
#include "engine_types.h"
#include "kernels_touch.h"
#include "kernels_update.h"
#include "kernels_fold.h"

namespace ftrl_dev {

constexpr int kTileT = 16;
constexpr int kTileRow = 80;
constexpr int kTileNR = 2;
#ifndef FFM_TILE_G
#define FFM_TILE_G 4
#endif
#ifndef FFM_FOLD_REGULAR
#define FFM_FOLD_REGULAR 1
#endif
constexpr int kTileG = FFM_TILE_G;

__device__ __forceinline__ int tile_hiword(int off_hi, bool live, bool first) {
  return (off_hi & 0xff) | (live ? static_cast<int>(0x80000000u) : 0) | (live && first ? 0x40000000 : 0);
}

struct TileWeights {
  float4 q0, q1, q2, q3;
// ... 399 lines not shown
          P = live[j] ? P + gj * gj : P;
          if (!any) hp = first[j];
          any = any || live[j];
          q = q || (live[j] && !first[j]);
        }
      }
      if (has) {
        s.segP[seg_elem(g, seg0 + st, e)] = P;
        s.segG[seg_elem(g, seg0 + st, e)] = G;
      }
      const unsigned long long ma = __ballot(any), mh = __ballot(any && hp), mq = __ballot(q);
      if (lane == 0) {
        unsigned long long *fl = seg_flags(s, g, seg0 + st, ci);
        fl[0] = ma; fl[1] = mh; fl[2] = mq;
      }
    });
  }
}
template <int NF>
__device__ __forceinline__ void ffm_range_items_b(const ModelDev &m, const Rows &rows, const Scratch &s, unsigned wave,
                                                  unsigned n_waves, float *T, float4 *R) {
  constexpr int RS = 4 * NF;
  constexpr int kFly = 8;
  const TileGeom g = tile_geom(m);
  const int lane = threadIdx.x & 63;
  const unsigned n_items = static_cast<unsigned>(s.counters[CNT_NRANGE]) * g.per_feat;
  for (unsigned item = wave; item < n_items; item += n_waves) {
    const unsigned ri = item / g.per_feat;
    const int ci = static_cast<int>(item - ri * g.per_feat);
    const int2 gr = s.grange[ri];
    const int gi = wave_uniform(gr.x), r = wave_uniform(gr.y);
    const int4 ud = s.udesc[wave_uniform(s.giant[gi])];
    const int fa = wave_uniform(ud.w), i = wave_uniform(ud.x);
    const int start = wave_uniform(ud.y), c = wave_uniform(ud.z);
    if (c < m.super_min) continue;
    const int segb = wave_uniform(s.gseg[gi]), n_seg = (c + kSeg - 1) / kSeg, seg_lo = r * kRangeSegs;
    const TileChunk ch = tile_chunk(m, g, fa, ci);
    if (ch.fp0 < 0) continue;
    unsigned long long q_all = 0ull, q_before = 0ull;
    for (int s0 = 0; s0 < n_seg; s0 += kFly) {
      unsigned long long mq[kFly];
#pragma unroll
      for (int j = 0; j < kFly; j++) mq[j] = seg_flags(s, g, segb + min(s0 + j, n_seg - 1), ci)[2];
#pragma unroll
      for (int j = 0; j < kFly; j++) {
        q_all |= mq[j];
        if (s0 + j < seg_lo) q_before |= mq[j];
      }
    }
    if (q_all == 0ull) continue;
    const bool active = ch.inw && ch.fp >= 0 && !((s.cmask[start] >> ch.fp) & 1ull);
    const bool has = ch.inw && ch.sb + ch.es < g.slots;
    const int e = has ? (ch.sb + ch.es) * g.K + ch.ekk : 0;
    const int t_lo = r * kRange, t_hi = min(c, t_lo + kRange);
    const int steps = (t_hi - t_lo + kTileT - 1) / kTileT;
    const float *rec = lat_row(m, i, fa) + (ch.fp >= 0 ? ch.sb + ch.es : ch.sb) * g.K + ch.ekk;
    const float w = rec[LAT_W * g.RL];
    Fold acc;
    acc.init(rec[LAT_N * g.RL]);
    for (int s0 = 0; s0 < seg_lo; s0 += kFly) {
      float p[kFly];
#pragma unroll
      for (int j = 0; j < kFly; j++) p[j] = s.segP[seg_elem(g, segb + min(s0 + j, seg_lo - 1), e)];
#pragma unroll
      for (int j = 0; j < kFly; j++)
        if (s0 + j < seg_lo) acc.B = acc.B + p[j];
    }
    const bool seen_before = (q_before >> lane) & 1ull;
    acc.seen = seen_before;
    tile_stream<NF>(m, s, g, ch, rows, fa, start, t_lo / kTileT, 1, steps, c, T, R,
                    [&](int st, const float4 *Rc, const float *Tc) {
      const int cnt = min(kTileT, t_hi - t_lo - st * kTileT);
      for (int g0 = 0; g0 < cnt; g0 += kTileG) {
        FTRL_TILE_READ_GROUP(Rc, Tc, g0, active)
        fold_ffm_group<kTileG>(acc, w, live, first, tg, x, vp);
      }
      if (has) s.segD[seg_elem(g, segb + seg_lo + st, e)] = acc.D;
      acc.flush();
    });
    if (has && acc.seen && !seen_before) s.gcap[static_cast<int64_t>(gi) * g.RL + e] = acc.ncap;
  }
}
__device__ __forceinline__ void ffm_range_join(const ModelDev &m, const Scratch &s, unsigned wave, unsigned n_waves) {
  constexpr int kFly = 16;
  const TileGeom g = tile_geom(m);
  const int lane = threadIdx.x & 63;
  const unsigned n_items = static_cast<unsigned>(s.counters[CNT_NGIANT]) * g.per_feat;
  for (unsigned item = wave; item < n_items; item += n_waves) {
    const unsigned gi = item / g.per_feat;
    const int ci = static_cast<int>(item - gi * g.per_feat);
    const int4 ud = s.udesc[wave_uniform(s.giant[gi])];
    const int fa = wave_uniform(ud.w), i = wave_uniform(ud.x);
    const int start = wave_uniform(ud.y), c = wave_uniform(ud.z);
    if (c < m.super_min) continue;
    const int segb = wave_uniform(s.gseg[gi]), n_seg = (c + kSeg - 1) / kSeg;
    const TileChunk ch = tile_chunk(m, g, fa, ci);
    if (ch.fp0 < 0) continue;
    const bool active = ch.inw && ch.fp >= 0 && !((s.cmask[start] >> ch.fp) & 1ull);
    if (!__any(active && ((s.gmask[start] >> ch.fp) & 1ull))) continue;
    const int e = ch.inw && ch.sb + ch.es < g.slots ? (ch.sb + ch.es) * g.K + ch.ekk : 0;
    unsigned long long q_all = 0ull;
    for (int s0 = 0; s0 < n_seg; s0 += kFly) {
      unsigned long long mq[kFly];
#pragma unroll
      for (int j = 0; j < kFly; j++) mq[j] = seg_flags(s, g, segb + min(s0 + j, n_seg - 1), ci)[2];
#pragma unroll
      for (int j = 0; j < kFly; j++) q_all |= mq[j];
    }
    float *rec = lat_row(m, i, fa) + (ch.fp >= 0 ? ch.sb + ch.es : ch.sb) * g.K + ch.ekk;
    float n = rec[LAT_N * g.RL], z = rec[LAT_Z * g.RL];
    const float w = rec[LAT_W * g.RL];
    Fold acc;
    acc.init(n);
    for (int s0 = 0; s0 < n_seg; s0 += kFly) {
      float p[kFly], gsum[kFly], d[kFly];
      unsigned long long fa_[kFly], fh_[kFly];
#pragma unroll
      for (int j = 0; j < kFly; j++) {
        const int sg = segb + min(s0 + j, n_seg - 1);
        p[j] = s.segP[seg_elem(g, sg, e)];
        gsum[j] = s.segG[seg_elem(g, sg, e)];
        d[j] = q_all ? s.segD[seg_elem(g, sg, e)] : -0.0f;
        const unsigned long long *fl = seg_flags(s, g, sg, ci);
        fa_[j] = fl[0];
        fh_[j] = fl[1];
      }
#pragma unroll
      for (int j = 0; j < kFly; j++) {
        if (s0 + j >= n_seg) continue;
        const bool any_s = (fa_[j] >> lane) & 1ull, hp_s = (fh_[j] >> lane) & 1ull;
        acc.P = p[j];
        acc.G = gsum[j];
        acc.D = d[j];
        if (!acc.any) acc.head_plain = hp_s;
        acc.any = acc.any || any_s;
        acc.flush();
      }
    }
    acc.seen = (q_all >> lane) & 1ull;
    acc.ncap = acc.seen ? s.gcap[static_cast<int64_t>(gi) * g.RL + e] : 0.0f;
    if (fold_finish_latent(m.h, acc, w, n, z) && active) {
      rec[LAT_N * g.RL] = n;
      rec[LAT_Z * g.RL] = z;
    }
  }
}
#undef FTRL_TILE_READ_GROUP

constexpr int tile_waves(int nf) { return nf == 4 && FFM_TILE_WAVES > 4 ? 4 : nf == 2 && FFM_TILE_WAVES > 8 ? 8 : FFM_TILE_WAVES; }
constexpr size_t tile_lds_bytes(int nf, int waves) {
  return static_cast<size_t>(waves) * (kTileT * kTileRow * sizeof(float) + kTileNR * kTileT * 4 * nf * sizeof(float4));
}
constexpr size_t tile_lds_bytes(int nf) { return tile_lds_bytes(nf, tile_waves(nf)); }
static_assert(few_stage_bytes(1, 64) <= tile_lds_bytes(1, 1), "the few-occurrence range's staging fits a wave's tile region");
constexpr int kWideWaves = 8;
enum { UPD_GIANT = 1, UPD_HOT = 2, UPD_FEW = 4, UPD_SIDE = 8, UPD_REST = 16, UPD_ALL = 31 };
#ifndef FFM_OCC_ALL
#define FFM_OCC_ALL 0
#endif
#ifndef FFM_OCC_HOT
#define FFM_OCC_HOT 4
#endif
#ifndef FFM_OCC_FEW
#define FFM_OCC_FEW 0
#endif
#ifndef FFM_OCC_GIANT
#define FFM_OCC_GIANT 4
#endif
constexpr int upd_occ(int kinds, int nf) {
  return kinds == UPD_ALL ? FFM_OCC_ALL
         : (kinds & UPD_GIANT) ? (nf == 4 ? 3 : FFM_OCC_GIANT)
         : (kinds & UPD_HOT) ? (nf == 4 ? 3 : FFM_OCC_HOT)
         : (kinds & UPD_FEW) ? FFM_OCC_FEW : 0;
}
constexpr int upd_occ_min(int kinds, int nf) { return upd_occ(kinds, nf) > 0 ? upd_occ(kinds, nf) : 1; }
constexpr int upd_occ_max(int kinds, int nf) { return upd_occ(kinds, nf) > 0 ? upd_occ(kinds, nf) : 8; }
#define FFM_UPD_OCC __attribute__((amdgpu_waves_per_eu(upd_occ_min(KINDS, NF), upd_occ_max(KINDS, NF))))
template <int NF, int KINDS = UPD_ALL, int WAVES = tile_waves(NF)>
__global__ __launch_bounds__(64 * WAVES) FFM_UPD_OCC void ffm_update_all_kernel(ModelDev m, Rows rows, Scratch s,
                                                                     int side_blocks, int ng, int nt, int ns,
                                                                     int few_only, int nw, int loss_blocks,
                                                                     double *loss_out, double *loss_scratch, int order) {
  extern __shared__ __attribute__((aligned(16))) char lds_dyn[];
  __shared__ CoopLds<WAVES> lds_coop;
  int r = blockIdx.x;
  const unsigned wv = wave_uniform(threadIdx.x >> 6);
  float *T = reinterpret_cast<float *>(lds_dyn) + wv * (kTileT * kTileRow);
  float4 *R = reinterpret_cast<float4 *>(lds_dyn + WAVES * kTileT * kTileRow * sizeof(float)) + wv * (kTileNR * kTileT * 4 * NF);
  if ((KINDS & UPD_SIDE) && r < side_blocks) {
    if (r == 0) bias_update_body(m, rows.n_rows, s, reinterpret_cast<float *>(lds_dyn));
    else linear_update_body(m, rows, s, r - 1, side_blocks - 1);
    return;
  }
  r -= side_blocks;
  int kind = -1;
  for (int o = order, left = 3; left > 0 && kind < 0; left--, o /= 10) {
    const int kd = o % 10;
    const int n = kd == 0 ? ng : kd == 1 ? nt : ns;
    if (r < n) kind = kd;
    else r -= n;
  }
  if (kind == 0) {
    if (KINDS & UPD_GIANT) ffm_coop_items<NF, WAVES>(m, rows, s, r, ng, T, R, lds_coop);
  } else if (kind == 1) {
    if (KINDS & UPD_HOT) {
      ffm_range_items_a<NF>(m, rows, s, r * WAVES + wv, nt * WAVES, T, R);
      ffm_tile_items<NF>(m, rows, s, r * WAVES + wv, nt * WAVES, T, R);
    }
  } else if (kind == 2) {
    if (KINDS & UPD_FEW) ffm_small_body(m, rows, s, few_only, r, ns, few_stage_possible(m) ? reinterpret_cast<int2 *>(lds_dyn) : nullptr);
  }
  if (kind >= 0) return;
  if (KINDS & UPD_REST) {
    if (r < nw) { ffm_generic_body(m, rows, s, 1, r, nw); return; }
    loss_sum_body(rows.n_rows, s.loss, loss_out, loss_scratch, r - nw, loss_blocks);
  }
}
template <int NF>
__global__ __launch_bounds__(kUpdThreads) void ffm_update_super_b_kernel(ModelDev m, Rows rows, Scratch s) {
  __shared__ __attribute__((aligned(16))) float lds_T[kUpdWaves][kTileT * kTileRow];
  __shared__ float4 lds_R[kUpdWaves][kTileNR * kTileT * 4 * NF];
  const unsigned wv = wave_uniform(threadIdx.x >> 6);
  ffm_range_items_b<NF>(m, rows, s, blockIdx.x * kUpdWaves + wv, gridDim.x * kUpdWaves, lds_T[wv], lds_R[wv]);
}
__global__ __launch_bounds__(kUpdThreads) void ffm_update_super_join_kernel(ModelDev m, Scratch s) {
  ffm_range_join(m, s, blockIdx.x * kUpdWaves + wave_uniform(threadIdx.x >> 6), gridDim.x * kUpdWaves);
}

}
```

ftrl-ffm_amd/csrc/kernels_update.h:

```cpp
#pragma once
#include <type_traits>

#include "engine_types.h"
#include "kernels_touch.h"
#include "kernels_fold.h"

namespace ftrl_dev {

constexpr int kUpdThreads = 256;
constexpr int kUpdWaves = kUpdThreads / 64;
#ifndef FFM_TILE_WAVES
#define FFM_TILE_WAVES 4
#endif
static_assert(FFM_TILE_WAVES >= 4, "loss_sum_body sums with the first 256 threads of an update workgroup");
constexpr int kUpdMaxThreads = 64 * (FFM_TILE_WAVES > 8 ? FFM_TILE_WAVES : 8);
constexpr int kFmUnroll = 8;


__device__ __forceinline__ int64_t fact_offset(int lo, int hi) {
  return (static_cast<int64_t>(hi) << 32) | static_cast<unsigned>(lo);
}


__device__ __forceinline__ void linear_update_body(const ModelDev &m, const Rows &rows,
                                                   const Scratch &s, int block, int n_blocks,
                                                   int skip_once = 0) {
  const int n_small = s.counters[CNT_NSMALL], n_big = s.counters[CNT_NBIG];
  const int gtid = block * blockDim.x + threadIdx.x;
  for (int li = gtid; li < n_small; li += n_blocks * blockDim.x) {
    const int u = s.small[li];
    const int4 ud = s.udesc[u];
    if (!owns_linear(m, ud.w)) continue;
    const int i = ud.x;
    const int start = ud.y, c = ud.z;
    if (skip_once && c == 1) continue;
    float n = m.lin_n[i], z = m.lin_z[i];
    const float w = m.lin_w[i];
    if (s.uflag[start] & UF_DUP) {
      float sqn = sqrt_cr(n);
      for (int t = 0; t < c; t++) {
        const int2 pr = s.occ2[start + t];
        nz_step_linear_carry(m.h, w, s.tg[pr.y] * rows.val[pr.x], n, z, sqn);
      }
    } else {
      Fold a;
      a.init(n);
      for (int t = 0; t < c; t++) {
        const int2 pr = s.occ2[start + t];
        a.plain(true, s.tg[pr.y] * rows.val[pr.x]);
      }
      fold_finish_linear(m.h, a, w, n, z);
    }
    m.lin_n[i] = n;
    m.lin_z[i] = z;
  }
  const int lane = threadIdx.x & 63;
  const int upd_waves = blockDim.x >> 6;
  const int wave = block * upd_waves + wave_uniform(threadIdx.x >> 6);
  const int n_waves = n_blocks * upd_waves;
  const int n_huge = s.counters[CNT_NHUGE], n_giant = s.counters[CNT_NGIANT];
  for (int li = wave; li < n_big + n_huge + n_giant; li += n_waves) {
    const int u = wave_uniform(li < n_giant ? s.giant[li]
                               : li < n_giant + n_huge ? s.huge[li - n_giant] : s.big[li - n_giant - n_huge]);
    const int4 ud = s.udesc[u];
    if (!owns_linear(m, wave_uniform(ud.w))) continue;
    const int i = wave_uniform(ud.x);
    const int start = wave_uniform(ud.y), c = wave_uniform(ud.z);
    float n = m.lin_n[i], z = m.lin_z[i];
    const float w = m.lin_w[i];
    if (wave_uniform(s.uflag[start]) & UF_DUP) {
      if (lane == 0) {
        float sqn = sqrt_cr(n);
        for (int t = 0; t < c; t++) {
          const int2 pr = s.occ2[start + t];
          nz_step_linear_carry(m.h, w, s.tg[pr.y] * rows.val[pr.x], n, z, sqn);
        }
        m.lin_n[i] = n;
        m.lin_z[i] = z;
      }
      continue;
    }
    Fold a;
    a.init(n);
    const int n_seg = (c + kSeg - 1) / kSeg;
    for (int s0 = 0; s0 < n_seg; s0 += 64) {
      const int t0 = (s0 + lane) * kSeg;
      float P = -0.0f, G = -0.0f;
      constexpr int kFly = 8;
      for (int j0 = 0; j0 < kSeg; j0 += kFly) {
        if (t0 + j0 >= c) break;
        int2 pr[kFly];
        float tgv[kFly], xv[kFly];
#pragma unroll
        for (int j = 0; j < kFly; j++) pr[j] = s.occ2[start + min(t0 + j0 + j, c - 1)];
#pragma unroll
        for (int j = 0; j < kFly; j++) { tgv[j] = s.tg[pr[j].y]; xv[j] = rows.val[pr[j].x]; }
#pragma unroll
        for (int j = 0; j < kFly; j++) {
          if (t0 + j0 + j < c) {
            const float g = tgv[j] * xv[j];
            G = G + g;
            P = P + g * g;
          }
        }
      }
      const int cnt = min(64, n_seg - s0);
      for (int l = 0; l < cnt; l++) {
        a.P = __int_as_float(__builtin_amdgcn_readlane(__float_as_int(P), l));
        a.G = __int_as_float(__builtin_amdgcn_readlane(__float_as_int(G), l));
        a.flush();
      }
    }
    a.any = a.head_plain = true;
    fold_finish_linear(m.h, a, w, n, z);
    if (lane == 0) {
      m.lin_n[i] = n;
      m.lin_z[i] = z;
    }
  }
}
__global__ __launch_bounds__(kUpdThreads) void linear_update_kernel(ModelDev m, Rows rows,
                                                                    Scratch s, int skip_once) {
  linear_update_body(m, rows, s, blockIdx.x, gridDim.x, skip_once);
}

__device__ __forceinline__ void bias_update_body(const ModelDev &m, int n_rows, const Scratch &sc, float *buf) {
  if (!m.bias_own) return;
  if (sc.counters[CNT_ERROR]) return;
  if (n_rows <= 0) return;
  float *s_P = buf, *s_G = buf + blockDim.x;
  const int n_thr = blockDim.x;
  const float *tg = sc.tg;
  const int n_seg = (n_rows + kSeg - 1) / kSeg;
  Fold a;
  a.init(m.bias3[1]);
  for (int s0 = 0; s0 < n_seg; s0 += n_thr) {
    const int seg = s0 + threadIdx.x;
    float P = -0.0f, G = -0.0f;
    if (seg < n_seg) {
      const int r0 = seg * kSeg;
      if (r0 + kSeg <= n_rows) {
        const float4 *t4 = reinterpret_cast<const float4 *>(tg + r0);
        float4 v[kSeg / 4];
#pragma unroll
        for (int j = 0; j < kSeg / 4; j++) v[j] = t4[j];
#pragma unroll
        for (int j = 0; j < kSeg / 4; j++) {
          G = G + v[j].x; P = P + v[j].x * v[j].x;
          G = G + v[j].y; P = P + v[j].y * v[j].y;
          G = G + v[j].z; P = P + v[j].z * v[j].z;
          G = G + v[j].w; P = P + v[j].w * v[j].w;
        }
      } else {
        for (int r = r0; r < n_rows; r++) {
          const float g = tg[r];
          G = G + g;
          P = P + g * g;
        }
      }
    }
    s_P[threadIdx.x] = P;
    s_G[threadIdx.x] = G;
    __syncthreads();
    if (threadIdx.x == 0) {
      const int cnt = min(n_thr, n_seg - s0);
      for (int l = 0; l < cnt; l++) {
        a.P = s_P[l];
        a.G = s_G[l];
        a.flush();
      }
    }
    __syncthreads();
  }
  if (threadIdx.x == 0) {
    float n = m.bias3[1], z = m.bias3[2];
    a.any = a.head_plain = true;
    fold_finish_linear(m.h, a, m.bias3[0], n, z);
    m.bias3[1] = n;
    m.bias3[2] = z;
  }
}
__global__ __launch_bounds__(kUpdThreads) void bias_update_kernel(ModelDev m, int n_rows, Scratch s) {
  __shared__ float s_PG[2 * kUpdThreads];
  bias_update_body(m, n_rows, s, s_PG);
}

__device__ inline bool ffm_walk_repeated(const ModelDev &m, const Rows &rows, const Scratch &s, int occ0, int d,
                                         int r, int fp, int kk, float w, float &n, float &z) {
  constexpr int kEnd = 0x7fffffff;
  const float tg = s.tg[r];
  bool touched = false;
  auto touch = [&](int e, int q) {
    const int fm = rows.field[e];
    if (!owns_pair(m, fm, fp)) return;
    const float vp = m.lat[w_slot_offset(m, rows.feat[q], fp, fm) + kk];
    ffm_touch(m.h, e < q, tg, rows.val[e], rows.val[q], vp, w, n, z);
    touched = true;
  };
  int ea = 0, qa = s.head[static_cast<int64_t>(r) * m.n_fields + fp];
  while (ea < d || qa >= 0) {
    const int pe = ea < d ? s.occ2[occ0 + ea].x : kEnd, pq = qa >= 0 ? qa : kEnd;
    const int a = pe < pq ? pe : pq;
    const bool a_occ = pe == a, a_partner = pq == a;
    if (a_occ) ea++;
    if (a_partner) qa = s.next[qa];
    int ec = ea, qc = qa;
    while (ec < d || qc >= 0) {
      const int ce = ec < d ? s.occ2[occ0 + ec].x : kEnd, cq = qc >= 0 ? qc : kEnd;
      const int cc = ce < cq ? ce : cq;
      if (a_occ && cq == cc) touch(a, cc);
      if (a_partner && ce == cc) touch(cc, a);
      if (ce == cc) ec++;
      if (cq == cc) qc = s.next[qc];
    }
  }
  return touched;
}

__device__ __forceinline__ void ffm_generic_element(const ModelDev &m, const Rows &rows, const Scratch &s,
                                                    int4 ud, unsigned long long cm, int e, int serial_only) {
  const int RL = m.row_len, k = m.n_factors, F = m.n_fields;
  if (e >= RL) return;
  const int start = ud.y, c = ud.z, fa = ud.w;
  const int sl = e / k, kk = e - sl * k;
  const int fp = walk_field(m, fa, sl);
  if (fp < 0) return;
  const bool serial = !s.cmask || ((cm >> fp) & 1ull);
  if (serial_only && !serial) return;
  const int i = ud.x;
  float *rec = lat_row(m, i, fa);
  float n = rec[LAT_N * RL + e], z = rec[LAT_Z * RL + e];
  const float w = rec[LAT_W * RL + e];
  bool touched = false;
  if (serial) {
    for (int t = 0; t < c; t++) {
      const int2 pr = s.occ2[start + t];
      const int p = pr.x, r = pr.y;
      int d = 1;
      while (t + d < c && s.occ2[start + t + d].y == r) d++;
      if (d > 1) {
        touched |= ffm_walk_repeated(m, rows, s, start + t, d, r, fp, kk, w, n, z);
        t += d - 1;
        continue;
      }
      const int fm = rows.field[p];
      if (!owns_pair(m, fm, fp)) continue;
      const float tg = s.tg[r], xm = rows.val[p];
      for (int qq = s.head[static_cast<int64_t>(r) * F + fp]; qq >= 0; qq = s.next[qq]) {
        if (qq == p) continue;
        const float vp = m.lat[w_slot_offset(m, rows.feat[qq], fp, fm) + kk];
        ffm_touch(m.h, p < qq, tg, xm, rows.val[qq], vp, w, n, z);
        touched = true;
      }
    }
  } else {
    Fold a;
    a.init(n);
    for (int t = 0; t < c; t++) {
      if (t > 0 && t % kSeg == 0) a.flush();
      const int2 pr = s.occ2[start + t];
      const int p = pr.x, r = pr.y;
      const int fm = rows.field[p];
      if (!owns_pair(m, fm, fp)) continue;
      const int4 rt = s.rowtab[static_cast<int64_t>(r) * F + fp];
      const int q = rt.z;
      if (q < 0 || q == p) continue;
      const bool live[1] = {true}, first[1] = {p < q || m.h.learn != 0};
      const float tgv[1] = {s.tg[r]}, xv[1] = {rows.val[p] * __int_as_float(rt.y)};
      const float vp[1] = {m.lat[w_slot_offset(m, rt.x, fp, fm) + kk]};
      fold_ffm_group<1>(a, w, live, first, tgv, xv, vp);
    }
    touched = fold_finish_latent(m.h, a, w, n, z);
  }
  if (touched) {
    rec[LAT_N * RL + e] = n;
    rec[LAT_Z * RL + e] = z;
  }
}
__device__ __forceinline__ void ffm_generic_body(const ModelDev &m, const Rows &rows, const Scratch &s,
                                                 int serial_only, unsigned bidx, unsigned gdim) {
  const unsigned chunks = (m.row_len + 63) / 64;
  const int lane = threadIdx.x & 63;
  const unsigned upd_waves = blockDim.x >> 6;
  const unsigned wave = bidx * upd_waves + wave_uniform(threadIdx.x >> 6);
  const unsigned n_waves = gdim * upd_waves;
  if (serial_only) {
    const int n_few = s.counters[CNT_NFEW], n_big = n_few + s.counters[CNT_NBIG];
    const int n_huge = n_big + s.counters[CNT_NHUGE], n_multi = n_huge + s.counters[CNT_NGIANT];
    for (int base = wave * 64; base < n_multi; base += n_waves * 64) {
      const int li = base + lane;
      int4 ud = make_int4(0, 0, 0, 0);
      unsigned long long cm = 0ull;
      if (li < n_multi) {
        const int u = li < n_few ? s.few[li] : li < n_big ? s.big[li - n_few]
                      : li < n_huge ? s.huge[li - n_big] : s.giant[li - n_huge];
        ud = s.udesc[u];
        cm = s.cmask ? s.cmask[ud.y] : ~0ull;
      }
      unsigned long long todo = __ballot(cm != 0ull);
      while (todo) {
        const int l = __ffsll(static_cast<long long>(todo)) - 1;
        todo &= todo - 1ull;
        const int4 d = make_int4(__builtin_amdgcn_readlane(ud.x, l), __builtin_amdgcn_readlane(ud.y, l),
                                 __builtin_amdgcn_readlane(ud.z, l), __builtin_amdgcn_readlane(ud.w, l));
        const unsigned long long cml =
            (static_cast<unsigned long long>(static_cast<unsigned>(__builtin_amdgcn_readlane(static_cast<int>(cm >> 32), l))) << 32) |
            static_cast<unsigned>(__builtin_amdgcn_readlane(static_cast<int>(cm & 0xffffffffull), l));
        for (unsigned ci = 0; ci < chunks; ci++)
          ffm_generic_element(m, rows, s, d, cml, static_cast<int>(ci) * 64 + lane, 1);
      }
    }
    return;
  }
  const unsigned n_items = static_cast<unsigned>(s.counters[CNT_NUNIQ]) * chunks;
  for (unsigned item = wave; item < n_items; item += n_waves) {
    const unsigned u = item / chunks;
    const int4 ud = s.udesc[u];
    const unsigned long long cm = s.cmask ? s.cmask[ud.y] : ~0ull;
    ffm_generic_element(m, rows, s, ud, cm, static_cast<int>(item - u * chunks) * 64 + lane, 0);
  }
}
__global__ __launch_bounds__(kUpdThreads) void ffm_update_generic_kernel(ModelDev m, Rows rows,
                                                                         Scratch s, int serial_only) {
  ffm_generic_body(m, rows, s, serial_only, blockIdx.x, gridDim.x);
}

#ifndef FFM_SMALL_BATCH
#define FFM_SMALL_BATCH 4
#endif
constexpr int kSmallBatch = FFM_SMALL_BATCH < kSmallMax ? FFM_SMALL_BATCH : kSmallMax;
constexpr int kSmallPad = (kSmallMax + kSmallBatch - 1) / kSmallBatch * kSmallBatch;
static_assert(kSmallPad % kSmallBatch == 0 && kSmallPad >= kSmallMax && kSmallPad < kSmallMax + kSmallBatch,
              "the per-touch arrays of the few-occurrence range hold kSmallMax rounded up to whole batches");
static_assert(kSmallPad <= 64, "lane j of the owning wave fetches touch j");
#ifndef FFM_STAGE_FLY
#define FFM_STAGE_FLY 7
#endif
constexpr int kStageFly = FFM_STAGE_FLY;
constexpr size_t few_stage_bytes(int waves, int n_fields) {
  return static_cast<size_t>(waves) * kSmallPad * static_cast<size_t>(n_fields) * sizeof(int2);
}
__host__ __device__ inline bool few_stage_possible(const ModelDev &m) {
  return m.few_stage != 0 && m.sort_start != nullptr && m.n_shards == 1 && m.own_n == nullptr &&
         m.field_start == nullptr && m.h.learn == 0 && m.rec_slots * (m.n_factors >> 2) > 64;
}
#ifdef FFM_SMALL_WAVES
#define FFM_SMALL_OCC __attribute__((amdgpu_waves_per_eu(FFM_SMALL_WAVES, FFM_SMALL_WAVES)))
#else
#define FFM_SMALL_OCC
#endif
#ifndef FFM_FEW_LDS
#define FFM_FEW_LDS 1
#endif
#ifndef FFM_FOLD_REGULAR
#define FFM_FOLD_REGULAR 1
#endif
__device__ __forceinline__ void ffm_small_items(bool staged, const ModelDev &m, const Rows &rows, const Scratch &s,
                                                int few_only, unsigned bidx, unsigned gdim, bool regular,
                                                int4 *facts, float *tgs, int2 *stage) {
  const int RL = m.row_len, k = m.n_factors, F = m.n_fields;
  const int RL4 = RL >> 2, k4 = k >> 2;
  const int lane = threadIdx.x & 63;
  const int upd_waves = blockDim.x >> 6;
  const int wave = bidx * upd_waves + wave_uniform(threadIdx.x >> 6);
  const int n_waves = gdim * upd_waves;
  const int *list = few_only ? s.few : s.small;
  const int n_small = s.counters[few_only ? CNT_NFEW : CNT_NSMALL];
  const float inv_k4 = 1.0f / static_cast<float>(k4);
  const int span4 = record_span(m, k4);
  const float inv_F = 1.0f / static_cast<float>(F);
  auto uniform4 = [](int4 v) { return make_int4(wave_uniform(v.x), wave_uniform(v.y), wave_uniform(v.z), wave_uniform(v.w)); };
  int4 ud_next = make_int4(0, 0, 0, 0);
  int u_next2 = 0;
  if (wave < n_small) ud_next = uniform4(s.udesc[wave_uniform(list[wave])]);
  if (wave + n_waves < n_small) u_next2 = wave_uniform(list[wave + n_waves]);
  for (int li = wave; li < n_small; li += n_waves) {
    const int4 ud = ud_next;
    if (li + n_waves < n_small) ud_next = uniform4(s.udesc[u_next2]);
    if (li + 2 * n_waves < n_small) u_next2 = wave_uniform(list[li + 2 * n_waves]);
    const int i = ud.x;
    const int start = ud.y, c = ud.z;
    const int fa = ud.w;
    float4 *rec4 = reinterpret_cast<float4 *>(staged ? m.lat + static_cast<long long>(i) * 3 * RL : lat_row(m, i, fa));
    const unsigned long long cm = s.cmask[start];
#if FFM_FEW_LDS
    {
      int2 pr = make_int2(0, 0);
      if (lane < c) pr = s.occ2[start + lane];
      int4 f = make_int4(0, 0, 0, 0);
      float g = 0.0f;
      if (lane < c) {
        f = make_int4(pr.x, pr.y, rows.field[pr.x], __float_as_int(rows.val[pr.x]));
        g = s.tg[pr.y];
      }
      if (staged) {
        const int n_stage = c * F;
#pragma unroll 1
        for (int i0 = 0; i0 < n_stage; i0 += 64 * kStageFly) {
          int sf[kStageFly];
          float sv[kStageFly];
#pragma unroll
          for (int it = 0; it < kStageFly; it++) {
            sf[it] = 0;
            sv[it] = 0.0f;
            const int idx = i0 + it * 64 + lane;
            if (i0 + it * 64 < n_stage) {
              const int j = static_cast<int>((idx + 0.5f) * inv_F);
              const int pe = __shfl(pr.x, j < c ? j : 0);
              if (idx < n_stage) {
                const int q = pe - fa + (idx - j * F);
                sf[it] = rows.feat[q];
                sv[it] = rows.val[q];
              }
            }
          }
#pragma unroll
          for (int it = 0; it < kStageFly; it++) {
            const int idx = i0 + it * 64 + lane;
            if (idx < n_stage) stage[idx] = make_int2(sf[it], __float_as_int(sv[it]));
          }
        }
      }
      if (lane < kSmallPad) {
        facts[lane] = f;
        tgs[lane] = g;
      }
      __builtin_amdgcn_fence(__ATOMIC_RELEASE, "wavefront");
    }
#define FEW_TP(j) (facts[j].x)
#define FEW_TR(j) (facts[j].y)
#define FEW_TFM(j) (facts[j].z)
#define FEW_TXM(j) (__int_as_float(facts[j].w))
#define FEW_TTG(j) (tgs[j])
#else
    int tp[kSmallPad], tr[kSmallPad], tfm[kSmallPad];
    float txm[kSmallPad], ttg[kSmallPad];
#pragma unroll
    for (int j = 0; j < kSmallPad; j++) {
      tp[j] = tr[j] = tfm[j] = 0;
      txm[j] = ttg[j] = 0.0f;
      if (j < c) {
        const int2 pr = s.occ2[start + j];
        tp[j] = wave_uniform(pr.x);
        tr[j] = wave_uniform(pr.y);
        tfm[j] = wave_uniform(rows.field[tp[j]]);
        txm[j] = __int_as_float(wave_uniform(__float_as_int(rows.val[tp[j]])));
        ttg[j] = __int_as_float(wave_uniform(__float_as_int(s.tg[tr[j]])));
      }
    }
#define FEW_TP(j) (tp[j])
#define FEW_TR(j) (tr[j])
#define FEW_TFM(j) (tfm[j])
#define FEW_TXM(j) (txm[j])
#define FEW_TTG(j) (ttg[j])
#endif
    auto passes = [&](auto staged_tag) {
    constexpr bool STAGED = decltype(staged_tag)::value;
    for (int l0 = 0; l0 < span4; l0 += 64) {
      const int l = l0 + lane;
      const int lc = l < span4 ? l : 0;
      int sl = static_cast<int>((lc + 0.5f) * inv_k4);
      sl += (sl + 1) * k4 <= lc ? 1 : (sl * k4 > lc ? -1 : 0);
      int fp = l < span4 ? (STAGED ? sl : walk_field(m, fa, sl)) : -1;
      if (fp >= 0 && ((cm >> fp) & 1ull)) fp = -1;
      const bool mine = fp >= 0;
      fp = mine ? fp : 0;
      const int kq = lc - sl * k4;
      const unsigned long long own_bits = STAGED ? ~0ull : owner_bits(m, fp);
      float n[4] = {0.0f, 0.0f, 0.0f, 0.0f}, z[4] = {0.0f, 0.0f, 0.0f, 0.0f}, w[4] = {0.0f, 0.0f, 0.0f, 0.0f};
      if (mine) {
        const float4 n4 = load_nt(rec4 + LAT_N * RL4 + lc), z4 = load_nt(rec4 + LAT_Z * RL4 + lc), w4 = rec4[LAT_W * RL4 + lc];
        n[0] = n4.x; n[1] = n4.y; n[2] = n4.z; n[3] = n4.w;
        z[0] = z4.x; z[1] = z4.y; z[2] = z4.z; z[3] = z4.w;
        w[0] = w4.x; w[1] = w4.y; w[2] = w4.z; w[3] = w4.w;
      }
      FoldFew<4> a;
      a.init();
      const bool lv = mine && fp != fa, q118 = lv && !m.h.learn && fp < fa;
#pragma unroll
      for (int j0 = 0; j0 < kSmallMax; j0 += kSmallBatch) {
        if (j0 >= c) break;
        float4 vp4[kSmallBatch];
        if constexpr (STAGED) {
          float xp[kSmallBatch];
#pragma unroll
          for (int jj = 0; jj < kSmallBatch; jj++) {
            const int j = j0 + jj;
            xp[jj] = 0.0f;
            vp4[jj] = make_float4(0.0f, 0.0f, 0.0f, 0.0f);
            if (j < c && lv) {
              const int2 pv = stage[j * F + fp];
              xp[jj] = __int_as_float(pv.y);
              vp4[jj] = reinterpret_cast<const float4 *>(m.lat + static_cast<long long>(pv.x) * 3 * RL)[LAT_W * RL4 + fa * k4 + kq];
            }
          }
#pragma unroll
          for (int jj = 0; jj < kSmallBatch; jj++) {
            const int j = j0 + jj;
            if (j >= c) continue;
            const float vp[4] = {vp4[jj].x, vp4[jj].y, vp4[jj].z, vp4[jj].w};
            a.touch_regular(n, w, lv, q118, FEW_TTG(j), FEW_TXM(j) * xp[jj], vp);
          }
          continue;
        }
        int4 rt[kSmallBatch];
#pragma unroll
        for (int jj = 0; jj < kSmallBatch; jj++) {
          const int j = j0 + jj;
          rt[jj] = make_int4(0, 0, -1, 0);
          if (mine && j < c && owns_bit(own_bits, FEW_TFM(j))) rt[jj] = s.rowtab[static_cast<int64_t>(FEW_TR(j)) * F + fp];
        }
#pragma unroll
        for (int jj = 0; jj < kSmallBatch; jj++) {
          const int j = j0 + jj;
          vp4[jj] = make_float4(0.0f, 0.0f, 0.0f, 0.0f);
          if (j < c && rt[jj].z >= 0 && rt[jj].z != FEW_TP(j))
            vp4[jj] = reinterpret_cast<const float4 *>(lat_row(m, rt[jj].x, fp))[LAT_W * RL4 + slot_of(m, fp, FEW_TFM(j)) * k4 + kq];
        }
#pragma unroll
        for (int jj = 0; jj < kSmallBatch; jj++) {
          const int j = j0 + jj;
          if (j >= c) continue;
          const int p = FEW_TP(j), q = rt[jj].z;
          const float vp[4] = {vp4[jj].x, vp4[jj].y, vp4[jj].z, vp4[jj].w};
          if (regular) {
            a.touch_regular(n, w, lv, q118, FEW_TTG(j), FEW_TXM(j) * __int_as_float(rt[jj].y), vp);
            continue;
          }
          const bool live = q >= 0 && q != p;
          a.touch(n, w, live, p < q || m.h.learn != 0, FEW_TTG(j), FEW_TXM(j) * __int_as_float(rt[jj].y), vp);
        }
      }
      if (a.finish(m.h, w, n, z) && mine) {
        store_nt(rec4 + LAT_N * RL4 + lc, make_float4(n[0], n[1], n[2], n[3]));
        store_nt(rec4 + LAT_Z * RL4 + lc, make_float4(z[0], z[1], z[2], z[3]));
      }
    }
    };
    if (staged) passes(std::true_type{});
    else passes(std::false_type{});
#if FFM_FEW_LDS
    __builtin_amdgcn_fence(__ATOMIC_RELEASE, "wavefront");
#endif
  }
#undef FEW_TP
#undef FEW_TR
#undef FEW_TFM
#undef FEW_TXM
#undef FEW_TTG
}
__device__ __forceinline__ void ffm_small_body(const ModelDev &m, const Rows &rows, const Scratch &s,
                                               int few_only, unsigned bidx, unsigned gdim, int2 *stage_all = nullptr) {
#if FFM_FEW_LDS
  __shared__ int4 few_facts[kUpdMaxThreads / 64][kSmallPad];
  __shared__ float few_tg[kUpdMaxThreads / 64][kSmallPad];
  const int wv_in_block = wave_uniform(threadIdx.x >> 6);
  int4 *facts = few_facts[wv_in_block];
  float *tgs = few_tg[wv_in_block];
#else
  const int wv_in_block = 0;
  int4 *facts = nullptr;
  float *tgs = nullptr;
#endif
#if FFM_FOLD_REGULAR
  const bool regular = m.sort_start != nullptr && m.n_shards == 1 && m.own_n == nullptr && s.counters[CNT_IRREGULAR] == 0;
#else
  const bool regular = false;
#endif
  const bool staged = FFM_FEW_LDS && regular && stage_all != nullptr && few_stage_possible(m);
  int2 *stage = staged ? stage_all + static_cast<size_t>(wv_in_block) * kSmallPad * m.n_fields : nullptr;
  ffm_small_items(staged, m, rows, s, few_only, bidx, gdim, regular, facts, tgs, stage);
}
__global__ __launch_bounds__(kUpdThreads) FFM_SMALL_OCC void ffm_update_small_kernel(ModelDev m, Rows rows,
                                                                       Scratch s, int few_only) {
  ffm_small_body(m, rows, s, few_only, blockIdx.x, gridDim.x);
}

#ifndef FFM_FLAT_BATCH
#define FFM_FLAT_BATCH 4
#endif
constexpr int kFlatBatch = FFM_FLAT_BATCH < kSmallMax ? FFM_FLAT_BATCH : kSmallMax;
__global__ __launch_bounds__(kUpdThreads) void ffm_update_small_flat_kernel(ModelDev m, Rows rows,
                                                                            Scratch s, int few_only) {
  const int RL4 = m.row_len >> 2, k4 = m.n_factors >> 2, F = m.n_fields;
  const int span4 = record_span(m, k4);
  const int *list = few_only ? s.few : s.small;
  const unsigned total =
      static_cast<unsigned>(s.counters[few_only ? CNT_NFEW : CNT_NSMALL]) * static_cast<unsigned>(span4);
  const double inv_span = 1.0 / static_cast<double>(span4);
  const float inv_k4 = 1.0f / static_cast<float>(k4);
  const unsigned stride = gridDim.x * blockDim.x;
  const unsigned rounds = (total + stride - 1) / stride;
  for (unsigned rd = 0; rd < rounds; rd++) {
    const unsigned t = rd * stride + blockIdx.x * blockDim.x + threadIdx.x;
    const bool in = t < total;
    const unsigned tt = in ? t : 0u;
    int li = static_cast<int>((static_cast<double>(tt) + 0.5) * inv_span);
    li += static_cast<unsigned>(li + 1) * span4 <= tt ? 1 : (static_cast<unsigned>(li) * span4 > tt ? -1 : 0);
    const int l = static_cast<int>(tt - static_cast<unsigned>(li) * span4);
    int sl = static_cast<int>((l + 0.5f) * inv_k4);
    sl += (sl + 1) * k4 <= l ? 1 : (sl * k4 > l ? -1 : 0);
    const int kq = l - sl * k4;
    int4 ud = make_int4(0, 0, 0, 0);
    if (in) ud = s.udesc[list[li]];
    const int i = ud.x, start = ud.y, c = ud.z, fa = ud.w;
    int fp = in ? walk_field(m, fa, sl) : -1;
    if (fp >= 0 && ((s.cmask[start] >> fp) & 1ull)) fp = -1;
    const bool mine = fp >= 0;
    fp = mine ? fp : 0;
    const unsigned long long own_bits = owner_bits(m, fp);
    float4 *rec4 = reinterpret_cast<float4 *>(lat_row(m, i, fa));
    float n[4] = {0.0f, 0.0f, 0.0f, 0.0f}, z[4] = {0.0f, 0.0f, 0.0f, 0.0f}, w[4] = {0.0f, 0.0f, 0.0f, 0.0f};
    if (mine) {
      const float4 n4 = load_nt(rec4 + LAT_N * RL4 + l), z4 = load_nt(rec4 + LAT_Z * RL4 + l), w4 = rec4[LAT_W * RL4 + l];
      n[0] = n4.x; n[1] = n4.y; n[2] = n4.z; n[3] = n4.w;
      z[0] = z4.x; z[1] = z4.y; z[2] = z4.z; z[3] = z4.w;
      w[0] = w4.x; w[1] = w4.y; w[2] = w4.z; w[3] = w4.w;
    }
    FoldFew<4> a;
    a.init();
    for (int j0 = 0; j0 < kSmallMax; j0 += kFlatBatch) {
      if (!__any(mine && j0 < c)) break;
      int2 pr[kFlatBatch];
#pragma unroll
      for (int jj = 0; jj < kFlatBatch; jj++) {
        pr[jj] = make_int2(0, 0);
        if (mine && j0 + jj < c) pr[jj] = s.occ2[start + j0 + jj];
      }
      int fm[kFlatBatch];
      int4 rt[kFlatBatch];
      float tgv[kFlatBatch], xv[kFlatBatch];
      bool own[kFlatBatch];
#pragma unroll
      for (int jj = 0; jj < kFlatBatch; jj++) {
        fm[jj] = 0;
        own[jj] = false;
        rt[jj] = make_int4(0, 0, -1, 0);
        tgv[jj] = xv[jj] = 0.0f;
        if (mine && j0 + jj < c) {
          fm[jj] = rows.field[pr[jj].x];
          rt[jj] = s.rowtab[static_cast<int64_t>(pr[jj].y) * F + fp];
          tgv[jj] = s.tg[pr[jj].y];
          xv[jj] = rows.val[pr[jj].x];
        }
      }
      float4 v4[kFlatBatch];
      bool live[kFlatBatch];
#pragma unroll
      for (int jj = 0; jj < kFlatBatch; jj++) {
        own[jj] = mine && j0 + jj < c && owns_bit(own_bits, fm[jj]);
        live[jj] = own[jj] && rt[jj].z >= 0 && rt[jj].z != pr[jj].x;
        v4[jj] = make_float4(0.0f, 0.0f, 0.0f, 0.0f);
        if (live[jj])
          v4[jj] = reinterpret_cast<const float4 *>(lat_row(m, rt[jj].x, fp))[LAT_W * RL4 + slot_of(m, fp, fm[jj]) * k4 + kq];
      }
#pragma unroll
      for (int jj = 0; jj < kFlatBatch; jj++) {
        if (!__any(mine && j0 + jj < c)) break;
        const float vp[4] = {v4[jj].x, v4[jj].y, v4[jj].z, v4[jj].w};
        const bool first = live[jj] && (pr[jj].x < rt[jj].z || m.h.learn != 0);
        a.touch(n, w, live[jj], first, live[jj] ? tgv[jj] : 0.0f, live[jj] ? xv[jj] * __int_as_float(rt[jj].y) : 0.0f, vp);
      }
    }
    if (a.finish(m.h, w, n, z) && mine) {
      store_nt(rec4 + LAT_N * RL4 + l, make_float4(n[0], n[1], n[2], n[3]));
      store_nt(rec4 + LAT_Z * RL4 + l, make_float4(z[0], z[1], z[2], z[3]));
    }
  }
}

template <int kSingleTrips>
__global__ __launch_bounds__(kUpdThreads) void ffm_update_single_kernel(ModelDev m, Rows rows,
                                                                        Scratch s) {
  const int RL = m.row_len, k = m.n_factors, F = m.n_fields;
  const int RL4 = RL >> 2, k4 = k >> 2;
  const int lane = threadIdx.x & 63;
  const int wave = blockIdx.x * kUpdWaves + wave_uniform(threadIdx.x >> 6);
  const int n_waves = gridDim.x * kUpdWaves;
  const int n_single = s.counters[CNT_NSINGLE];
  const float inv_k4 = 1.0f / static_cast<float>(k4);
  const int span4 = record_span(m, k4);
  for (int li = wave; li < n_single; li += n_waves) {
    const int4 d = s.sdesc[li];
    const int i = wave_uniform(d.x), p = wave_uniform(d.y), r = wave_uniform(d.z);
    const int fa = wave_uniform(d.w);
    const float xm = rows.val[p], tg = s.tg[r];
    float4 *rec4 = reinterpret_cast<float4 *>(lat_row(m, i, fa));
    const unsigned long long own_fa = owner_bits(m, fa);
    const int4 *rtab = s.rowtab + static_cast<int64_t>(r) * F;
    for (int l0 = 0; l0 < span4; l0 += 64 * kSingleTrips) {
      int l[kSingleTrips], fp[kSingleTrips], kq[kSingleTrips];
      float4 n4[kSingleTrips], z4[kSingleTrips], w4[kSingleTrips], vp[kSingleTrips];
      int4 rt[kSingleTrips];
#pragma unroll
      for (int t = 0; t < kSingleTrips; t++) {
        const int lc = l0 + t * 64 + lane;
        const int ll = lc < span4 ? lc : 0;
        int sl = static_cast<int>((ll + 0.5f) * inv_k4);
        sl += (sl + 1) * k4 <= ll ? 1 : (sl * k4 > ll ? -1 : 0);
        int f = lc < span4 ? walk_field(m, fa, sl) : -1;
        if (f >= 0 && !owns_bit(own_fa, f)) f = -1;
        l[t] = f >= 0 ? ll : -1;
        kq[t] = ll - sl * k4;
        f = f < 0 ? 0 : f;
        fp[t] = f;
        if (l[t] >= 0) {
          n4[t] = load_nt(rec4 + LAT_N * RL4 + ll);
          z4[t] = load_nt(rec4 + LAT_Z * RL4 + ll);
          w4[t] = rec4[LAT_W * RL4 + ll];
          rt[t] = rtab[f];
        }
      }
#pragma unroll
      for (int t = 0; t < kSingleTrips; t++) {
        if (l[t] >= 0 && rt[t].z >= 0 && rt[t].z != p)
          vp[t] = reinterpret_cast<const float4 *>(
              lat_row(m, rt[t].x, fp[t]))[LAT_W * RL4 + slot_of(m, fp[t], fa) * k4 + kq[t]];
      }
#pragma unroll
      for (int t = 0; t < kSingleTrips; t++) {
        if (l[t] < 0) continue;
        const int q = rt[t].z;
        bool touched = false;
        if (q >= 0) {
          if (q != p) {
            ffm_touch4(m.h, p < q, tg, xm, __int_as_float(rt[t].y), vp[t], w4[t], n4[t], z4[t]);
            touched = true;
          }
        } else if (q == -2) {
          for (int qq = s.head[static_cast<int64_t>(r) * F + fp[t]]; qq >= 0; qq = s.next[qq]) {
            if (qq == p) continue;
            const float4 vq = reinterpret_cast<const float4 *>(
                lat_row(m, rows.feat[qq], fp[t]))[LAT_W * RL4 + slot_of(m, fp[t], fa) * k4 + kq[t]];
            ffm_touch4(m.h, p < qq, tg, xm, rows.val[qq], vq, w4[t], n4[t], z4[t]);
            touched = true;
          }
        }
        if (touched) {
          store_nt(rec4 + LAT_N * RL4 + l[t], n4[t]);
          store_nt(rec4 + LAT_Z * RL4 + l[t], z4[t]);
        }
      }
    }
  }
}

__global__ __launch_bounds__(kUpdThreads) void ffm_update_single_flat_kernel(ModelDev m, Rows rows,
                                                                             Scratch s) {
  const int RL4 = m.row_len >> 2, k4 = m.n_factors >> 2, F = m.n_fields;
  const int span4 = record_span(m, k4);
  const unsigned total = static_cast<unsigned>(s.counters[CNT_NSINGLE]) * static_cast<unsigned>(span4);
  const double inv_span = 1.0 / static_cast<double>(span4);
  const float inv_k4 = 1.0f / static_cast<float>(k4);
  const unsigned stride = gridDim.x * blockDim.x;
  for (unsigned t = blockIdx.x * blockDim.x + threadIdx.x; t < total; t += stride) {
    int li = static_cast<int>((static_cast<double>(t) + 0.5) * inv_span);
    li += static_cast<unsigned>(li + 1) * span4 <= t ? 1 : (static_cast<unsigned>(li) * span4 > t ? -1 : 0);
    const int ll = static_cast<int>(t - static_cast<unsigned>(li) * span4);
    int sl = static_cast<int>((ll + 0.5f) * inv_k4);
    sl += (sl + 1) * k4 <= ll ? 1 : (sl * k4 > ll ? -1 : 0);
    const int kq = ll - sl * k4;
    const int4 d = s.sdesc[li];
    const int i = d.x, p = d.y, r = d.z, fa = d.w;
    const int f = walk_field(m, fa, sl);
    if (f < 0 || !owns_bit(owner_bits(m, fa), f)) continue;
    const int4 rt = s.rowtab[static_cast<int64_t>(r) * F + f];
    const int q = rt.z;
    if (q == -1 || q == p) continue;
    float4 *rec4 = reinterpret_cast<float4 *>(lat_row(m, i, fa));
    float4 n4 = load_nt(rec4 + LAT_N * RL4 + ll), z4 = load_nt(rec4 + LAT_Z * RL4 + ll);
    const float4 w4 = rec4[LAT_W * RL4 + ll];
    const float xm = rows.val[p], tg = s.tg[r];
    bool touched = false;
// ... 234 lines not shown
```

ftrl-ffm_amd/engine.py:

```python
import ctypes
import os

import numpy as np

HERE = os.path.dirname(os.path.abspath(__file__))
LIB_PATH = os.path.join(HERE, "libffm_engine.so")

LR, FM, FFM = 0, 1, 2
MODEL_TYPES = {"LR": LR, "FM": FM, "FFM": FFM}
FLAG_SKIP_INIT = 1
FLAG_LEARN = 4
FLAG_HASH_IDS = 8
FLAG_SERVE_F32, FLAG_SERVE_F16 = 16, 32
SERVE_FLAGS = {None: 0, "none": 0, "f32": FLAG_SERVE_F32, "f16": FLAG_SERVE_F16}
E_INVALID, E_DEVICE, E_NOMEM, E_CAPACITY, E_UNSUPPORTED = -1, -2, -3, -4, -5

_i32p = ctypes.POINTER(ctypes.c_int32)
_f32p = ctypes.POINTER(ctypes.c_float)
_f64p = ctypes.POINTER(ctypes.c_double)
_vp = ctypes.c_void_p


class EngineError(RuntimeError):
    def __init__(self, code, msg):
        super().__init__("ffm_engine error %d: %s" % (code, msg))
        self.code = code


class Config(ctypes.Structure):
    _fields_ = [("model_type", ctypes.c_int32), ("n_feats", ctypes.c_int32),
                ("n_fields", ctypes.c_int32), ("n_factors", ctypes.c_int32),
                ("w_alpha", ctypes.c_float), ("w_beta", ctypes.c_float),
                ("w_l1", ctypes.c_float), ("w_l2", ctypes.c_float),
                ("init_mean", ctypes.c_float), ("init_stddev", ctypes.c_float),
                ("seed", ctypes.c_uint64), ("max_batch_rows", ctypes.c_int32),
                ("max_batch_nnz", ctypes.c_int32), ("device_id", ctypes.c_int32),
                ("n_shards", ctypes.c_int32), ("shard_rank", ctypes.c_int32),
                ("stream", ctypes.c_void_p), ("flags", ctypes.c_int32),
                ("max_row_nnz", ctypes.c_int32), ("field_start", _i32p),
                ("reserved", ctypes.c_int32 * 4)]


class Metrics(ctypes.Structure):
    _fields_ = [("n_pos", ctypes.c_int64), ("n_neg", ctypes.c_int64), ("n_nan", ctypes.c_int64),
                ("n_mixed_bins", ctypes.c_int64), ("auc", ctypes.c_double), ("auc_slack", ctypes.c_double)]

    def as_dict(self):
        return {k: getattr(self, k) for k, _ in self._fields_}


class KeyedMetrics(ctypes.Structure):
    _fields_ = [(k, ctypes.c_int64) for k in ("n_rows", "n_keys", "n_keys_mixed", "n_rows_mixed", "n_nan", "n_unkeyed",
                                              "n_overflow")] + [("gauc", ctypes.c_double)]

    def as_dict(self):
        return {k: getattr(self, k) for k, _ in self._fields_}


class RefreshStats(ctypes.Structure):
    _fields_ = [(k, ctypes.c_int64) for k in ("lin_live", "lin_nonzero", "lin_moved",
                                              "lat_live", "lat_nonzero", "lat_moved")]

    def as_dict(self):
        return {k: int(getattr(self, k)) for k, _ in self._fields_}


class PackStats(ctypes.Structure):
    _fields_ = [(k, ctypes.c_int64) for k in ("n_latent", "n_inexact", "n_to_inf", "n_to_zero")]

    def as_dict(self):
        return {k: int(getattr(self, k)) for k, _ in self._fields_}


METRIC_EVAL, METRIC_TRAIN = 0, 1
METRIC_BINS = 1 << 20
_METRIC_CHANNELS = {"eval": METRIC_EVAL, "train": METRIC_TRAIN}
_u64p = ctypes.POINTER(ctypes.c_uint64)
_i64p = ctypes.POINTER(ctypes.c_int64)

_CSR = [_i32p, _i32p, _i32p, _f32p, _i32p]
_DCSR = [_vp, _vp, _vp, _vp, _vp]
ABI = [
    ("ffm_engine_default_config", None, [ctypes.POINTER(Config)]),
    ("ffm_engine_create", ctypes.c_int, [ctypes.POINTER(Config), ctypes.POINTER(_vp)]),
    ("ffm_engine_init_weights_host", ctypes.c_int,
     [ctypes.c_uint64, ctypes.c_float, ctypes.c_float, ctypes.c_int32, ctypes.c_int64,
      ctypes.c_int64, _f32p]),
    ("ffm_engine_destroy", None, [_vp]),
    ("ffm_engine_last_error", ctypes.c_char_p, []),
    ("ffm_engine_abi_version", ctypes.c_int, []),
    ("ffm_engine_block_segment", ctypes.c_int, []),
    ("ffm_engine_row_len", ctypes.c_int64, [_vp]),
    ("ffm_engine_default_batch_ramp", ctypes.c_int32, [ctypes.c_float]),
    ("ffm_engine_shard_plan", ctypes.c_int,
     [ctypes.c_int32, ctypes.c_int32, ctypes.c_int32, _i32p, _i32p, _i32p]),
    ("ffm_engine_set_weights", ctypes.c_int, [_vp, _f32p, _f32p, _f32p]),
    ("ffm_engine_get_weights", ctypes.c_int, [_vp, _f32p, _f32p, _f32p]),
    ("ffm_engine_set_state", ctypes.c_int, [_vp] + [_f32p] * 6),
    ("ffm_engine_get_state", ctypes.c_int, [_vp] + [_f32p] * 6),
    ("ffm_engine_get_rows", ctypes.c_int, [_vp, ctypes.c_int32, _i32p] + [_f32p] * 6),
    ("ffm_engine_set_rows", ctypes.c_int, [_vp, ctypes.c_int32, _i32p] + [_f32p] * 6),
    ("ffm_engine_changed_features", ctypes.c_int,
     [_vp, _i32p, ctypes.c_int64, ctypes.POINTER(ctypes.c_int64)]),
    ("ffm_engine_train_batch", ctypes.c_int, [_vp, ctypes.c_int32] + _CSR + [_f32p, _f64p]),
    ("ffm_engine_predict_batch", ctypes.c_int,
     [_vp, ctypes.c_int32] + _CSR + [ctypes.c_int32, _f32p, _f64p]),
    ("ffm_engine_train_batch_device", ctypes.c_int,
     [_vp, ctypes.c_int32, ctypes.c_int32] + _DCSR + [_vp, _vp]),
    ("ffm_engine_predict_batch_device", ctypes.c_int,
     [_vp, ctypes.c_int32, ctypes.c_int32] + _DCSR + [ctypes.c_int32, _vp, _vp]),
    ("ffm_engine_predict_finish_device", ctypes.c_int,
     [_vp, ctypes.c_int32, _vp, _vp, ctypes.c_int32, _vp, _vp]),
    ("ffm_engine_train_batch_async", ctypes.c_int, [_vp, ctypes.c_int32] + _CSR),
    ("ffm_engine_train_batch_async_pinned", ctypes.c_int, [_vp, ctypes.c_int32] + _CSR),
    ("ffm_engine_train_flush", ctypes.c_int, [_vp, _f64p]),
    ("ffm_engine_predict_batch_async", ctypes.c_int, [_vp, ctypes.c_int32] + _CSR + [ctypes.c_int32]),
    ("ffm_engine_predict_batch_async_scores", ctypes.c_int,
     [_vp, ctypes.c_int32] + _CSR + [ctypes.c_int32, ctypes.c_int32, _vp]),
    ("ffm_engine_blocks_scored", ctypes.c_int64, [_vp]),
    ("ffm_engine_stage_batch", ctypes.c_int, [_vp, ctypes.c_int32] + _CSR + [ctypes.c_int32]),
    ("ffm_engine_blocks_pulled", ctypes.c_int64, [_vp]),
    ("ffm_engine_train_forward_staged", ctypes.c_int, [_vp, _vp]),
    ("ffm_engine_train_staged", ctypes.c_int, [_vp, _vp, _vp]),
    ("ffm_engine_pin_host", ctypes.c_int, [_vp, ctypes.c_size_t]),
    ("ffm_engine_unpin_host", ctypes.c_int, [_vp]),
    ("ffm_engine_prepare_device", ctypes.c_int,
     [_vp, ctypes.c_int32, ctypes.c_int32, _vp, _vp, _vp, _vp]),
    ("ffm_engine_train_forward_device", ctypes.c_int,
     [_vp, ctypes.c_int32, ctypes.c_int32] + _DCSR + [_vp]),
    ("ffm_engine_train_update_device", ctypes.c_int, [_vp, _vp, _vp, _vp]),
    ("ffm_engine_fill_state", ctypes.c_int,
     [_vp, ctypes.c_uint64, ctypes.c_float, ctypes.c_float, ctypes.c_float]),
    ("ffm_engine_eval_sigmoid", ctypes.c_int, [_vp, ctypes.c_int32, _f32p, _f32p]),
    ("ffm_engine_sync", ctypes.c_int, [_vp]),
    ("ffm_engine_check_errors", ctypes.c_int, [_vp]),
    ("ffm_engine_stream", ctypes.c_void_p, [_vp]),
    ("ffm_engine_profile_enable", ctypes.c_int, [_vp, ctypes.c_int32]),
    ("ffm_engine_profile_read", ctypes.c_int,
     [_vp, _i32p, _f64p, ctypes.c_char_p, ctypes.c_size_t]),
    ("ffm_engine_profile_focus", ctypes.c_int, [_vp]),
    ("ffm_engine_profile_dump", ctypes.c_int, [_vp, ctypes.c_char_p, ctypes.c_size_t]),
    ("ffm_engine_metrics_enable", ctypes.c_int, [_vp, ctypes.c_int32]),
    ("ffm_engine_metrics_read", ctypes.c_int,
     [_vp, ctypes.c_int32, ctypes.c_int32, ctypes.POINTER(Metrics)]),
    ("ffm_engine_metrics_histogram", ctypes.c_int, [_vp, ctypes.c_int32, _u64p, _u64p]),
    ("ffm_engine_metrics_from_histogram", ctypes.c_int,
     [_u64p, _u64p, ctypes.c_int64, ctypes.c_int64, ctypes.POINTER(Metrics)]),
    ("ffm_engine_metrics_key_field", ctypes.c_int, [_vp, ctypes.c_int32, ctypes.c_int32, ctypes.c_int64]),
    ("ffm_engine_metrics_read_keyed", ctypes.c_int, [_vp, ctypes.c_int32, ctypes.c_int32, ctypes.POINTER(KeyedMetrics)]),
    ("ffm_engine_metrics_keyed_table", ctypes.c_int,
     [_vp, ctypes.c_int32, ctypes.c_int64, _i32p, _i64p, _i64p, _u64p, _i64p]),
    ("ffm_engine_metrics_from_keyed", ctypes.c_int, [_i64p, _i64p, _u64p, ctypes.c_int64, ctypes.POINTER(KeyedMetrics)]),
    ("ffm_group_create", ctypes.c_int, [ctypes.POINTER(Config), ctypes.c_int32, _i32p, ctypes.POINTER(_vp)]),
    ("ffm_group_destroy", None, [_vp]),
    ("ffm_group_size", ctypes.c_int32, [_vp]),
    ("ffm_group_engine", ctypes.c_void_p, [_vp, ctypes.c_int32]),
    ("ffm_group_collective", ctypes.c_char_p, [_vp]),
    ("ffm_group_train_batch", ctypes.c_int, [_vp, ctypes.c_int32] + _CSR + [_f32p, _f64p]),
    ("ffm_group_train_batch_async", ctypes.c_int, [_vp, ctypes.c_int32] + _CSR + [ctypes.c_int32]),
    ("ffm_group_train_flush", ctypes.c_int, [_vp, _f64p]),
    ("ffm_group_blocks_pulled", ctypes.c_int64, [_vp]),
    ("ffm_group_predict_batch", ctypes.c_int,
     [_vp, ctypes.c_int32] + _CSR + [ctypes.c_int32, _f32p, _f64p]),
    ("ffm_group_metrics_enable", ctypes.c_int, [_vp, ctypes.c_int32]),
    ("ffm_group_metrics_read", ctypes.c_int,
     [_vp, ctypes.c_int32, ctypes.c_int32, ctypes.POINTER(Metrics)]),
    ("ffm_engine_train_batch_weighted", ctypes.c_int, [_vp, ctypes.c_int32] + _CSR + [_f32p, _f32p, _f64p]),
    ("ffm_engine_train_batch_device_weighted", ctypes.c_int,
     [_vp, ctypes.c_int32, ctypes.c_int32] + _DCSR + [_vp, _vp, _vp]),
    ("ffm_engine_train_forward_device_weighted", ctypes.c_int,
     [_vp, ctypes.c_int32, ctypes.c_int32] + _DCSR + [_vp, _vp]),
    ("ffm_engine_stage_batch_weighted", ctypes.c_int, [_vp, ctypes.c_int32] + _CSR + [_vp, ctypes.c_int32]),
    ("ffm_engine_train_batch_async_weighted", ctypes.c_int,
     [_vp, ctypes.c_int32] + _CSR + [_vp, ctypes.c_int32]),
    ("ffm_group_train_batch_weighted", ctypes.c_int, [_vp, ctypes.c_int32] + _CSR + [_f32p, _f32p, _f64p]),
    ("ffm_group_train_batch_async_weighted", ctypes.c_int,
     [_vp, ctypes.c_int32] + _CSR + [_vp, ctypes.c_int32]),
    ("ffm_engine_refresh_weights", ctypes.c_int, [_vp, ctypes.POINTER(RefreshStats)]),
    ("ffm_group_refresh_weights", ctypes.c_int, [_vp, ctypes.POINTER(RefreshStats)]),
    ("ffm_engine_hash_ids_device", ctypes.c_int, [_vp, ctypes.c_int32, _vp, _vp, _vp]),
    ("ffm_engine_hash_ids_host", ctypes.c_int,
     [ctypes.c_int32, ctypes.c_int32, ctypes.c_int32, _i32p, ctypes.c_int32, _i32p, _i32p, _i32p]),
    ("ffm_engine_pack_weights", ctypes.c_int, [_vp, _vp, ctypes.POINTER(PackStats)]),
    ("ffm_engine_model_bytes", ctypes.c_int64, [_vp]),
    ("ffm_engine_score_candidates", ctypes.c_int,
     [_vp, ctypes.c_int32, _i32p, _i32p, _i32p, _f32p, _i32p, ctypes.c_int32, _i32p, _i32p, _i32p, _f32p,
      ctypes.c_int32, _f32p]),
    ("ffm_engine_score_candidates_device", ctypes.c_int,
     [_vp, ctypes.c_int32, _vp, _vp, _vp, _vp, _vp, ctypes.c_int32, _vp, _vp, _vp, _vp,
      ctypes.c_int32, ctypes.c_int32, ctypes.c_int32, ctypes.c_int32, _vp]),
    ("ffm_engine_sketch_create", ctypes.c_int, [ctypes.c_int32, ctypes.c_int32, ctypes.POINTER(_vp)]),
    ("ffm_engine_sketch_add", ctypes.c_int, [_vp, ctypes.c_int32, _vp, _vp, ctypes.c_int32]),
    ("ffm_engine_sketch_add_device", ctypes.c_int, [_vp, ctypes.c_int32, _vp, _vp]),
    ("ffm_engine_sketch_read", ctypes.c_int, [_vp, _vp, _i64p, _i64p]),
    ("ffm_engine_sketch_destroy", None, [_vp]),
    ("ffm_engine_sketch_estimate", ctypes.c_int, [_vp, ctypes.c_int32, _f64p]),
    ("ffm_engine_field_ranges", ctypes.c_int, [_i64p, ctypes.c_int32, ctypes.c_int32, _i32p]),
    ("ffm_engine_ablation_enable", ctypes.c_int, [_vp, ctypes.c_int32]),
    ("ffm_engine_predict_ablated", ctypes.c_int, [_vp, ctypes.c_int32] + _CSR + [ctypes.c_int32, _f32p, _f64p]),
    ("ffm_engine_predict_ablated_device", ctypes.c_int,
     [_vp, ctypes.c_int32, ctypes.c_int32] + _DCSR + [ctypes.c_int32, _vp, _vp]),
    ("ffm_engine_ablation_read", ctypes.c_int, [_vp, ctypes.c_int32, ctypes.POINTER(Metrics)]),
]
SKETCH_REGS = 16384

_lib = None


def default_batch_ramp(w_alpha):
    return int(load_library().ffm_engine_default_batch_ramp(float(w_alpha)))


def shard_plan(n_fields, n_shards, field_map=False):
    lib = load_library()
    po = np.zeros((n_fields, n_fields), np.int32)
    lo = np.zeros(n_fields, np.int32)
    bo = ctypes.c_int32(0)
    rc = lib.ffm_engine_shard_plan(int(n_fields), int(n_shards), int(bool(field_map)), _i(po), _i(lo),
                                   ctypes.byref(bo))
    if rc != 0:
        raise EngineError(rc, lib.ffm_engine_last_error().decode())
    return dict(pair_owner=po, lin_owner=lo, bias_owner=int(bo.value))


def _channel(channel):
    return _METRIC_CHANNELS[channel] if isinstance(channel, str) else int(channel)


def metrics_from_histogram(pos, neg, n_nan=0):
    lib = load_library()
    pos = np.ascontiguousarray(pos, np.uint64)
    neg = np.ascontiguousarray(neg, np.uint64)
    if pos.shape != neg.shape or pos.ndim != 1:
        raise ValueError("pos and neg must be one-dimensional and equally long")
    m = Metrics()
    rc = lib.ffm_engine_metrics_from_histogram(pos.ctypes.data_as(_u64p), neg.ctypes.data_as(_u64p),
                                               pos.size, int(n_nan), ctypes.byref(m))
    if rc != 0:
        raise EngineError(rc, lib.ffm_engine_last_error().decode())
    return m.as_dict()


def metrics_from_keyed(pos, neg, u2):
    lib = load_library()
    pos = np.ascontiguousarray(pos, np.int64)
# ... 68 lines not shown
    fld = None if field is None or mt != FFM else np.ascontiguousarray(field, np.int32)
    fs = None if field_start is None or mt != FFM else np.ascontiguousarray(field_start, np.int32)
    if n_fields is None:
        if fs is None and fld is None and mt == FFM:
            raise ValueError("FFM rows without a field array need n_fields")
        n_fields = fs.size - 1 if fs is not None else 2 ** 31 - 1
    if fld is not None and fld.shape != feat.shape:
        raise ValueError("field and feat must be equally long")
    out = np.empty_like(feat)
    rc = lib.ffm_engine_hash_ids_host(mt, int(n_feats), int(n_fields), _i(fs), feat.size, _i(fld), _i(feat), _i(out))
    if rc != 0:
        raise EngineError(rc, lib.ffm_engine_last_error().decode())
    return out


def sketch_estimate(reg):
    lib = load_library()
    reg = np.ascontiguousarray(reg, np.uint8)
    if reg.ndim != 2 or reg.shape[1] != SKETCH_REGS:
        raise ValueError("reg: uint8 [n_fields, %d]" % SKETCH_REGS)
    out = np.zeros(reg.shape[0], np.float64)
    rc = lib.ffm_engine_sketch_estimate(reg.ctypes.data, reg.shape[0], out.ctypes.data_as(_f64p))
    if rc != 0:
        raise EngineError(rc, lib.ffm_engine_last_error().decode())
    return out


def field_ranges(count, n_feats):
    lib = load_library()
    count = np.ascontiguousarray(count, np.int64)
    if count.ndim != 1:
        raise ValueError("count: one integer per field")
    out = np.zeros(count.size + 1, np.int32)
    rc = lib.ffm_engine_field_ranges(count.ctypes.data_as(_i64p), count.size, int(n_feats), _i(out))
    if rc != 0:
        raise EngineError(rc, lib.ffm_engine_last_error().decode())
    return out


def drop_field(block, f):
    from .synth import Block
    field = np.asarray(block.field)
    keep = field != f
    kept = np.concatenate(([0], np.cumsum(keep, dtype=np.int64)))
    row_ptr = kept[np.asarray(block.row_ptr, np.int64)].astype(np.int32)
    return Block(row_ptr, np.ascontiguousarray(field[keep], np.int32), np.ascontiguousarray(np.asarray(block.feat)[keep], np.int32),
                 None if block.val is None else np.ascontiguousarray(np.asarray(block.val)[keep], np.float32), block.label)


def spell_out_candidates(ctx, cand_req_ptr, cand):
    from .synth import Block
    cand_req_ptr = np.asarray(cand_req_ptr, np.int64)
    n_req, n_cand = ctx.n_rows, cand.n_rows
    if cand_req_ptr.shape != (n_req + 1,) or cand_req_ptr[0] != 0 or cand_req_ptr[-1] != n_cand or (np.diff(cand_req_ptr) < 0).any():
        raise ValueError("cand_req_ptr must ascend from 0 to the number of candidates, one step per request")
    req = np.repeat(np.arange(n_req, dtype=np.int64), np.diff(cand_req_ptr))
    cp, kp = np.asarray(ctx.row_ptr, np.int64), np.asarray(cand.row_ptr, np.int64)
    n_ctx, n_own = np.diff(cp)[req], np.diff(kp)
    row_ptr = np.concatenate([[0], np.cumsum(n_ctx + n_own)])
    nnz = int(row_ptr[-1])
    row = np.repeat(np.arange(n_cand, dtype=np.int64), n_ctx + n_own)
    at = np.arange(nnz, dtype=np.int64) - row_ptr[row]
    from_ctx = at < n_ctx[row]
    src = np.where(from_ctx, cp[req[row]] + at, kp[row] + at - n_ctx[row])

    def merged(a, b, dtype):
        a = np.ones(int(cp[-1]), dtype) if a is None else np.asarray(a, dtype)
        b = np.ones(int(kp[-1]), dtype) if b is None else np.asarray(b, dtype)
        out = np.empty(nnz, dtype)
        out[from_ctx] = a[src[from_ctx]]
        out[~from_ctx] = b[src[~from_ctx]]
        return out
    return Block(row_ptr.astype(np.int32), merged(ctx.field, cand.field, np.int32), merged(ctx.feat, cand.feat, np.int32),
                 merged(ctx.val, cand.val, np.float32), np.zeros(n_cand, np.int32))


def load_library(path=None):
    global _lib
    if _lib is not None and path is None:
        return _lib
    path = path or os.environ.get("FFM_ENGINE_LIB") or LIB_PATH
    if not os.path.exists(path):
        raise FileNotFoundError(
            "%s not found: build it with `python ftrl-ffm_amd/build.py` (hipcc, gfx950). "
            "There is no CPU fallback." % path)
    lib = ctypes.CDLL(path)
    for name, restype, argtypes in ABI:
        fn = getattr(lib, name)
        fn.restype = restype
        fn.argtypes = argtypes
    _lib = lib
    return lib


def page_aligned(n, dtype):
    import mmap
    nbytes = max(1, int(n)) * np.dtype(dtype).itemsize
    size = (nbytes + mmap.PAGESIZE - 1) // mmap.PAGESIZE * mmap.PAGESIZE
    return np.frombuffer(mmap.mmap(-1, size), dtype=dtype, count=int(n))


def _f(a):
    return None if a is None else a.ctypes.data_as(_f32p)


def _i(a):
    return None if a is None else a.ctypes.data_as(_i32p)


def _w(weight, n_rows):
    if weight.dtype != np.float32 or weight.ndim != 1 or weight.size < n_rows or not weight.flags.c_contiguous:
        raise ValueError("weight: a contiguous float32 array of at least n_rows elements")
    return weight.ctypes.data


STATE_KEYS = ("bias3", "lin_w", "lin_n", "lin_z", "vec_w", "vec_n", "vec_z")


class Engine:

    def __init__(self, model_type="FFM", n_feats=10000, n_fields=8, n_factors=16, w_alpha=1e-4,
                 w_beta=1.0, w_l1=0.1, w_l2=5.0, init_mean=0.0, init_stddev=0.02, seed=42,
                 max_batch_rows=8192, max_batch_nnz=None, device_id=0, n_shards=1, shard_rank=0,
                 stream=None, skip_init=False, max_row_nnz=0, learn=False, field_start=None, hash_ids=False,
                 serve=None):
        self.lib = load_library()
        if serve not in SERVE_FLAGS:
            raise ValueError("serve: None, 'f32' or 'f16'")
        self.serve = serve if SERVE_FLAGS[serve] else None
        cfg = Config()
        self.lib.ffm_engine_default_config(ctypes.byref(cfg))
        cfg.model_type = MODEL_TYPES[model_type] if isinstance(model_type, str) else int(model_type)
        cfg.n_feats, cfg.n_fields, cfg.n_factors = int(n_feats), int(n_fields), int(n_factors)
        cfg.w_alpha, cfg.w_beta, cfg.w_l1, cfg.w_l2 = w_alpha, w_beta, w_l1, w_l2
        cfg.init_mean, cfg.init_stddev, cfg.seed = init_mean, init_stddev, int(seed)
        cfg.max_batch_rows = int(max_batch_rows)
        cfg.max_batch_nnz = int(max_batch_nnz if max_batch_nnz else max_batch_rows * 64)
        cfg.device_id, cfg.n_shards, cfg.shard_rank = int(device_id), int(n_shards), int(shard_rank)
        cfg.stream = stream
        cfg.flags = ((FLAG_SKIP_INIT if skip_init else 0) | (FLAG_LEARN if learn else 0) | (FLAG_HASH_IDS if hash_ids else 0)
                     | SERVE_FLAGS[serve])
        cfg.max_row_nnz = int(max_row_nnz)
        self._field_start = None
        if field_start is not None:
            self._field_start = np.ascontiguousarray(field_start, np.int32)
            cfg.field_start = _i(self._field_start)
        self.cfg = cfg
        self.h = _vp()
        self._check(self.lib.ffm_engine_create(ctypes.byref(cfg), ctypes.byref(self.h)))
        self.model_type = cfg.model_type
        self.n_feats, self.n_fields, self.n_factors = cfg.n_feats, cfg.n_fields, cfg.n_factors
        self.row_len = int(self.lib.ffm_engine_row_len(self.h))

    def _check(self, rc):
        if rc != 0:
            raise EngineError(rc, self.lib.ffm_engine_last_error().decode())

    def close(self):
        if getattr(self, "h", None) and self.h.value:
            self.lib.ffm_engine_destroy(self.h)
            self.h = _vp()

    def __del__(self):
        try:
            self.close()
        except Exception:
            pass

    def zero_state(self):
        nf, L = self.n_feats, self.row_len
        return dict(bias3=np.zeros(3, np.float32), lin_w=np.zeros(nf, np.float32),
                    lin_n=np.zeros(nf, np.float32), lin_z=np.zeros(nf, np.float32),
                    vec_w=np.zeros((nf, L), np.float32), vec_n=np.zeros((nf, L), np.float32),
                    vec_z=np.zeros((nf, L), np.float32))

    def get_weights(self):
        b = np.zeros(1, np.float32)
        lw = np.zeros(self.n_feats, np.float32)
        vw = np.zeros((self.n_feats, self.row_len), np.float32)
        self._check(self.lib.ffm_engine_get_weights(self.h, _f(b), _f(lw), _f(vw) if self.row_len else None))
        return dict(bias=b, lin_w=lw, vec_w=vw)

    def set_weights(self, bias=None, lin_w=None, vec_w=None):
        c = lambda a: None if a is None else np.ascontiguousarray(a, np.float32)
        b, lw, vw = c(bias), c(lin_w), c(vec_w)
        self._check(self.lib.ffm_engine_set_weights(self.h, _f(b.reshape(-1)[:1].copy()) if b is not None else None,
                                                    _f(lw), _f(vw) if vw is not None and vw.size else None))

    def model_bytes(self):
        return int(self.lib.ffm_engine_model_bytes(self.h))

    def pack_from(self, src):
        st = PackStats()
        self._check(self.lib.ffm_engine_pack_weights(self.h, src.h, ctypes.byref(st)))
        return st.as_dict()

    def load_sparse_weights(self, d):
        ids = np.ascontiguousarray(d["ids"], np.int32)
        if ids.size:
            self.set_rows(ids, {k: d[k] for k in ("lin_w", "vec_w") if k in d})
        b = np.ascontiguousarray(d["bias3"], np.float32)
        self._check(self.lib.ffm_engine_set_weights(self.h, _f(b[0:1].copy()), None, None))

    def get_state(self):
        if self.serve:
            raise EngineError(E_UNSUPPORTED, "a serving engine holds no accumulators: get_weights() reads what it stores")
        st = self.zero_state()
        b = np.zeros(3, np.float32)
        vw = st["vec_w"] if self.row_len else None
        vn = st["vec_n"] if self.row_len else None
        vz = st["vec_z"] if self.row_len else None
        self._check(self.lib.ffm_engine_get_weights(self.h, _f(b[0:1]), _f(st["lin_w"]), _f(vw)))
        self._check(self.lib.ffm_engine_get_state(self.h, _f(b[1:2]), _f(b[2:3]), _f(st["lin_n"]),
                                                  _f(st["lin_z"]), _f(vn), _f(vz)))
        st["bias3"] = b
        return st

    def set_state(self, st):
        st = {k: np.ascontiguousarray(v, np.float32) for k, v in st.items()}
        b = st.get("bias3")
        g = lambda k: st[k] if k in st and st[k].size else None
        self._check(self.lib.ffm_engine_set_weights(
            self.h, _f(b[0:1].copy()) if b is not None else None, _f(g("lin_w")), _f(g("vec_w"))))
        self._check(self.lib.ffm_engine_set_state(
            self.h, _f(b[1:2].copy()) if b is not None else None,
            _f(b[2:3].copy()) if b is not None else None, _f(g("lin_n")), _f(g("lin_z")),
            _f(g("vec_n")), _f(g("vec_z"))))

    ROW_KEYS = ("lin_w", "lin_n", "lin_z", "vec_w", "vec_n", "vec_z")

    def get_rows(self, ids):
        ids = np.ascontiguousarray(ids, np.int32)
        n, L = ids.size, self.row_len
        keys = ("lin_w", "vec_w") if self.serve else self.ROW_KEYS
        out = {k: np.zeros((n, L) if k.startswith("vec") else n, np.float32) for k in keys}
        args = [_f(out[k]) if k in out and out[k].size else None for k in self.ROW_KEYS]
        self._check(self.lib.ffm_engine_get_rows(self.h, n, _i(ids), *args))
        return out

    def set_rows(self, ids, st):
        ids = np.ascontiguousarray(ids, np.int32)
        st = {k: np.ascontiguousarray(v, np.float32) for k, v in st.items() if k in self.ROW_KEYS}
        args = [_f(st[k]) if k in st and st[k].size else None for k in self.ROW_KEYS]
        self._check(self.lib.ffm_engine_set_rows(self.h, ids.size, _i(ids), *args))

    def changed_features(self):
        n = ctypes.c_int64(0)
        ids = np.empty(self.n_feats, np.int32)
        self._check(self.lib.ffm_engine_changed_features(self.h, _i(ids), ids.size, ctypes.byref(n)))
        return ids[:n.value].copy()

    def refresh_weights(self):
        st = RefreshStats()
        self._check(self.lib.ffm_engine_refresh_weights(self.h, ctypes.byref(st)))
        return st.as_dict()

    def _bias3(self):
        b = np.zeros(3, np.float32)
        self._check(self.lib.ffm_engine_get_weights(self.h, _f(b[0:1]), None, None))
        self._check(self.lib.ffm_engine_get_state(self.h, _f(b[1:2]), _f(b[2:3]), None, None, None, None))
        return b

    def sparse_state(self):
        if self.serve:
            raise EngineError(E_UNSUPPORTED, "a serving engine holds no accumulators: the sparse checkpoint is a training engine's")
        ids = self.changed_features()
        out = dict(ids=ids, bias3=self._bias3())
        out.update(self.get_rows(ids))
        return out

    def load_sparse_state(self, d):
        n = ctypes.c_int64(0)
        self._check(self.lib.ffm_engine_changed_features(self.h, None, 0, ctypes.byref(n)))
        if n.value != 0:
            raise EngineError(E_INVALID, "load_sparse_state needs a fresh engine: %d features already changed" % n.value)
        ids = np.ascontiguousarray(d["ids"], np.int32)
        if ids.size:
            self.set_rows(ids, d)
        b = np.ascontiguousarray(d["bias3"], np.float32)
        self._check(self.lib.ffm_engine_set_weights(self.h, _f(b[0:1]), None, None))
        self._check(self.lib.ffm_engine_set_state(self.h, _f(b[1:2]), _f(b[2:3]), None, None, None, None))

    def _csr(self, c):
        fld = c.field if (self.model_type == FFM or c.field is not None) else None
        key = (c.n_rows, id(c.row_ptr), id(fld), id(c.feat), id(c.val), id(c.label))
        cached = getattr(c, "_ffm_csr_args", None)
        if cached is not None and cached[0] == key:
            return cached[1]
        args = (c.n_rows, _i(c.row_ptr), _i(fld), _i(c.feat), _f(c.val), _i(c.label))
        try:
            c._ffm_csr_args = (key, args, (c.row_ptr, fld, c.feat, c.val, c.label))
        except AttributeError:
            pass
        return args

    def train_batch(self, c, weight=None):
        out = np.zeros(max(c.n_rows, 1), np.float32)
        loss = ctypes.c_double(0.0)
        if weight is None:
            self._check(self.lib.ffm_engine_train_batch(self.h, *self._csr(c), _f(out),
                                                        ctypes.byref(loss)))
        else:
            _w(weight, c.n_rows)
            self._check(self.lib.ffm_engine_train_batch_weighted(self.h, *self._csr(c), _f(weight), _f(out),
                                                                 ctypes.byref(loss)))
        return out[:c.n_rows], float(loss.value)
# ... 393 lines not shown
```

include/ffm_engine.h:

```cpp
#ifndef FFM_ENGINE_H
#define FFM_ENGINE_H

#include <stddef.h>
#include <stdint.h>

#ifdef __cplusplus
extern "C" {
#endif

#define FFM_ENGINE_ABI_VERSION 4

enum { FFM_MODEL_LR = 0, FFM_MODEL_FM = 1, FFM_MODEL_FFM = 2 };

enum {
  FFM_OK = 0,
  FFM_E_INVALID = -1,
  FFM_E_DEVICE = -2,
  FFM_E_NOMEM = -3,
  FFM_E_CAPACITY = -4,
  FFM_E_UNSUPPORTED = -5
};

typedef struct ffm_engine ffm_engine;

typedef struct ffm_engine_config {
  int32_t model_type;
  int32_t n_feats;
  int32_t n_fields;
  int32_t n_factors;
  float w_alpha;
  float w_beta;
  float w_l1;
  float w_l2;
  float init_mean;
  float init_stddev;
  uint64_t seed;
  int32_t max_batch_rows;
  int32_t max_batch_nnz;
  int32_t device_id;
  int32_t n_shards;
  int32_t shard_rank;
  void *stream;
  int32_t flags;
  int32_t max_row_nnz;
  const int32_t *field_start;
  int32_t reserved[4];
} ffm_engine_config;

enum {
  FFM_FLAG_SKIP_INIT = 1,
  FFM_FLAG_LEARN = 4,
  FFM_FLAG_HASH_IDS = 8,
  FFM_FLAG_SERVE_F32 = 16,
  FFM_FLAG_SERVE_F16 = 32
};

void ffm_engine_default_config(ffm_engine_config *cfg);

int ffm_engine_create(const ffm_engine_config *cfg, ffm_engine **out);
int ffm_engine_init_weights_host(uint64_t seed, float init_mean, float init_stddev, int32_t latent,
                                 int64_t first, int64_t count, float *out);
void ffm_engine_destroy(ffm_engine *e);
const char *ffm_engine_last_error(void);
int ffm_engine_abi_version(void);
int ffm_engine_block_segment(void);

int ffm_engine_shard_plan(int32_t n_fields, int32_t n_shards, int32_t field_map, int32_t *pair_owner,
                          int32_t *lin_owner, int32_t *bias_owner);

int32_t ffm_engine_default_batch_ramp(float w_alpha);

int64_t ffm_engine_row_len(const ffm_engine *e);

int ffm_engine_set_weights(ffm_engine *e, const float *bias, const float *lin_w, const float *vec_w);
int ffm_engine_get_weights(ffm_engine *e, float *bias, float *lin_w, float *vec_w);

int ffm_engine_set_state(ffm_engine *e, const float *bias_n, const float *bias_z,
                         const float *lin_n, const float *lin_z, const float *vec_n,
                         const float *vec_z);
int ffm_engine_get_state(ffm_engine *e, float *bias_n, float *bias_z, float *lin_n, float *lin_z,
                         float *vec_n, float *vec_z);

int ffm_engine_get_rows(ffm_engine *e, int32_t n, const int32_t *feat_ids, float *lin_w,
                        float *lin_n, float *lin_z, float *vec_w, float *vec_n, float *vec_z);
int ffm_engine_set_rows(ffm_engine *e, int32_t n, const int32_t *feat_ids, const float *lin_w,
                        const float *lin_n, const float *lin_z, const float *vec_w,
                        const float *vec_n, const float *vec_z);

int ffm_engine_changed_features(ffm_engine *e, int32_t *ids, int64_t cap, int64_t *n_changed);

int ffm_engine_train_batch(ffm_engine *e, int32_t n_rows, const int32_t *row_ptr,
                           const int32_t *field, const int32_t *feat, const float *val,
                           const int32_t *label, float *logit_out, double *loss_sum_out);

int ffm_engine_predict_batch(ffm_engine *e, int32_t n_rows, const int32_t *row_ptr,
                             const int32_t *field, const int32_t *feat, const float *val,
                             const int32_t *label, int32_t output_prob, float *out,
                             double *loss_sum_out);

int ffm_engine_train_batch_device(ffm_engine *e, int32_t n_rows, int32_t nnz,
                                  const int32_t *row_ptr, const int32_t *field,
                                  const int32_t *feat, const float *val, const int32_t *label,
                                  float *logit_out, double *loss_sum_out);
int ffm_engine_predict_batch_device(ffm_engine *e, int32_t n_rows, int32_t nnz,
                                    const int32_t *row_ptr, const int32_t *field,
                                    const int32_t *feat, const float *val, const int32_t *label,
                                    int32_t output_prob, float *out, double *loss_sum_out);

int ffm_engine_predict_finish_device(ffm_engine *e, int32_t n_rows, const float *logit,
                                     const int32_t *label, int32_t output_prob, float *out,
                                     double *loss_sum_out);

int ffm_engine_train_batch_async(ffm_engine *e, int32_t n_rows, const int32_t *row_ptr,
                                 const int32_t *field, const int32_t *feat, const float *val,
                                 const int32_t *label);
int ffm_engine_train_flush(ffm_engine *e, double *loss_sum_out);
int ffm_engine_train_batch_async_pinned(ffm_engine *e, int32_t n_rows, const int32_t *row_ptr,
                                        const int32_t *field, const int32_t *feat, const float *val,
                                        const int32_t *label);

int ffm_engine_predict_batch_async(ffm_engine *e, int32_t n_rows, const int32_t *row_ptr,
                                   const int32_t *field, const int32_t *feat, const float *val,
                                   const int32_t *label, int32_t zero_copy);
int ffm_engine_predict_batch_async_scores(ffm_engine *e, int32_t n_rows, const int32_t *row_ptr,
                                          const int32_t *field, const int32_t *feat, const float *val,
                                          const int32_t *label, int32_t zero_copy, int32_t output_prob,
                                          float *scores_host);
int64_t ffm_engine_blocks_scored(ffm_engine *e);

int ffm_engine_stage_batch(ffm_engine *e, int32_t n_rows, const int32_t *row_ptr,
                           const int32_t *field, const int32_t *feat, const float *val,
                           const int32_t *label, int32_t zero_copy);
int64_t ffm_engine_blocks_pulled(ffm_engine *e);
int ffm_engine_train_forward_staged(ffm_engine *e, float *partial_logit);
int ffm_engine_train_staged(ffm_engine *e, float *logit_out, double *loss_sum_out);
int ffm_engine_pin_host(void *p, size_t bytes);
int ffm_engine_unpin_host(void *p);

int ffm_engine_prepare_device(ffm_engine *e, int32_t n_rows, int32_t nnz, const int32_t *row_ptr,
                              const int32_t *field, const int32_t *feat, const float *val);

int ffm_engine_train_forward_device(ffm_engine *e, int32_t n_rows, int32_t nnz,
                                    const int32_t *row_ptr, const int32_t *field,
                                    const int32_t *feat, const float *val, const int32_t *label,
                                    float *partial_logit);
int ffm_engine_train_update_device(ffm_engine *e, const float *logit, float *logit_out,
                                   double *loss_sum_out);

typedef struct ffm_group ffm_group;
int ffm_group_create(const ffm_engine_config *cfg, int32_t n, const int32_t *device_ids, ffm_group **out);
void ffm_group_destroy(ffm_group *g);
int32_t ffm_group_size(const ffm_group *g);
ffm_engine *ffm_group_engine(ffm_group *g, int32_t rank);
const char *ffm_group_collective(const ffm_group *g);
int ffm_group_train_batch(ffm_group *g, int32_t n_rows, const int32_t *row_ptr, const int32_t *field,
                          const int32_t *feat, const float *val, const int32_t *label,
                          float *logit_out, double *loss_sum_out);
int ffm_group_train_batch_async(ffm_group *g, int32_t n_rows, const int32_t *row_ptr,
                                const int32_t *field, const int32_t *feat, const float *val,
                                const int32_t *label, int32_t zero_copy);
int ffm_group_train_flush(ffm_group *g, double *loss_sum_out);
int64_t ffm_group_blocks_pulled(ffm_group *g);
int ffm_group_predict_batch(ffm_group *g, int32_t n_rows, const int32_t *row_ptr, const int32_t *field,
                            const int32_t *feat, const float *val, const int32_t *label,
                            int32_t output_prob, float *out, double *loss_sum_out);

int ffm_engine_train_batch_weighted(ffm_engine *e, int32_t n_rows, const int32_t *row_ptr,
                                    const int32_t *field, const int32_t *feat, const float *val,
                                    const int32_t *label, const float *weight, float *logit_out,
                                    double *loss_sum_out);
int ffm_engine_train_batch_device_weighted(ffm_engine *e, int32_t n_rows, int32_t nnz,
                                           const int32_t *row_ptr, const int32_t *field,
                                           const int32_t *feat, const float *val, const int32_t *label,
                                           const float *weight, float *logit_out, double *loss_sum_out);
int ffm_engine_train_forward_device_weighted(ffm_engine *e, int32_t n_rows, int32_t nnz,
                                             const int32_t *row_ptr, const int32_t *field,
                                             const int32_t *feat, const float *val, const int32_t *label,
                                             const float *weight, float *partial_logit);
int ffm_engine_stage_batch_weighted(ffm_engine *e, int32_t n_rows, const int32_t *row_ptr,
                                    const int32_t *field, const int32_t *feat, const float *val,
                                    const int32_t *label, const float *weight, int32_t zero_copy);
int ffm_engine_train_batch_async_weighted(ffm_engine *e, int32_t n_rows, const int32_t *row_ptr,
                                          const int32_t *field, const int32_t *feat, const float *val,
                                          const int32_t *label, const float *weight, int32_t zero_copy);
int ffm_group_train_batch_weighted(ffm_group *g, int32_t n_rows, const int32_t *row_ptr, const int32_t *field,
                                   const int32_t *feat, const float *val, const int32_t *label,
                                   const float *weight, float *logit_out, double *loss_sum_out);
int ffm_group_train_batch_async_weighted(ffm_group *g, int32_t n_rows, const int32_t *row_ptr,
                                         const int32_t *field, const int32_t *feat, const float *val,
                                         const int32_t *label, const float *weight, int32_t zero_copy);

int ffm_engine_fill_state(ffm_engine *e, uint64_t seed, float n_lo, float n_hi, float z_stddev);

int ffm_engine_eval_sigmoid(ffm_engine *e, int32_t n, const float *x, float *y);

int ffm_engine_sync(ffm_engine *e);
int ffm_engine_check_errors(ffm_engine *e);

void *ffm_engine_stream(ffm_engine *e);

int ffm_engine_profile_enable(ffm_engine *e, int32_t on);
int ffm_engine_profile_read(ffm_engine *e, int32_t *n_launches, double *total_ms,
                            char *kernel_name, size_t kernel_name_cap);
int ffm_engine_profile_focus(ffm_engine *e);
int ffm_engine_profile_dump(ffm_engine *e, char *buf, size_t cap);

enum { FFM_METRIC_EVAL = 0, FFM_METRIC_TRAIN = 1 };
#define FFM_METRIC_BINS (1 << 20)
typedef struct { int64_t n_pos, n_neg, n_nan, n_mixed_bins; double auc, auc_slack; } ffm_metrics;
int ffm_engine_metrics_enable(ffm_engine *e, int32_t channel_mask);
int ffm_engine_metrics_read(ffm_engine *e, int32_t channel, int32_t reset, ffm_metrics *out);
int ffm_engine_metrics_histogram(ffm_engine *e, int32_t channel, uint64_t *pos, uint64_t *neg);
int ffm_engine_metrics_from_histogram(const uint64_t *pos, const uint64_t *neg, int64_t n_bins,
                                      int64_t n_nan, ffm_metrics *out);
int ffm_group_metrics_enable(ffm_group *g, int32_t channel_mask);
int ffm_group_metrics_read(ffm_group *g, int32_t channel, int32_t reset, ffm_metrics *out);

typedef struct { int64_t n_rows, n_keys, n_keys_mixed, n_rows_mixed, n_nan, n_unkeyed, n_overflow; double gauc; } ffm_keyed_metrics;
int ffm_engine_metrics_key_field(ffm_engine *e, int32_t channel_mask, int32_t key_field, int64_t capacity_rows);
int ffm_engine_metrics_read_keyed(ffm_engine *e, int32_t channel, int32_t reset, ffm_keyed_metrics *out);
int ffm_engine_metrics_keyed_table(ffm_engine *e, int32_t channel, int64_t cap, int32_t *key, int64_t *pos, int64_t *neg,
                                   uint64_t *u2, int64_t *n_keys);
int ffm_engine_metrics_from_keyed(const int64_t *pos, const int64_t *neg, const uint64_t *u2, int64_t n_keys,
                                  ffm_keyed_metrics *out);

// ... 51 lines not shown
```

Before: 10.26 million samples/s.

## Make the few-occurrence bucket ceiling a runtime parameter with segmented fold

Replaces the compile-time kSmallMax ceiling on the few-occurrence update path with a per-model few_max, which can be raised up to kFewCap through FFM_FEW_MAX when LDS staging fits. The fold gains a MULTI mode that flushes partial sums every kSeg touches, and the batch loop is no longer unrolled, so longer occurrence lists can run in the few path instead of the heavier big-feature path. The default kFewMaxStaged stays at 10, the same as kSmallMax, so default behaviour is mostly unchanged except for the non-unrolled loop and the extra fold registers. LDS sizing per launch now takes the staged bytes into account.

```diff
diff --git a/ftrl-ffm_amd/csrc/engine.hip b/ftrl-ffm_amd/csrc/engine.hip
--- a/ftrl-ffm_amd/csrc/engine.hip
+++ b/ftrl-ffm_amd/csrc/engine.hip
@@ -546,6 +546,7 @@
 }
 
 int64_t ffm_engine_row_len(const ffm_engine *e) { return e ? e->logical_len : 0; }
+int ffm_engine_few_max(const ffm_engine *e) { return e ? e->m.few_max : 0; }
 
 void ffm_engine_destroy(ffm_engine *e) {
   if (!e) return;
diff --git a/ftrl-ffm_amd/csrc/engine_create.h b/ftrl-ffm_amd/csrc/engine_create.h
--- a/ftrl-ffm_amd/csrc/engine_create.h
+++ b/ftrl-ffm_amd/csrc/engine_create.h
@@ -8,7 +8,7 @@
   char row_refresh = 0;
   std::optional<bool> serial, super_wait, prep_after_row, pull_after_row, eval_defer_off, predict_waves, few_stage, own_sort;
   std::optional<int> update_split, update_order, wide_max_nnz, grid_pull, grid_push, grid_hot, grid_small, grid_walk, grid_giant;
-  std::optional<int> row_threads, row_park, row_park_budget, row_hold, super_min;
+  std::optional<int> row_threads, row_park, row_park_budget, row_hold, super_min, few_max;
   std::optional<int> range_sort;
 };
 extern "C++" {
@@ -57,6 +57,7 @@
   if (const char *sv = std::getenv("FFM_ROW_HOLD")) sw.row_hold = std::max(0, std::atoi(sv));
   if (const char *sv = std::getenv("FFM_SUPER_MIN")) sw.super_min = std::max(kGiantMin, std::atoi(sv));
   if (const char *sv = std::getenv("FFM_FEW_STAGE")) sw.few_stage = sv[0] != '0';
+  if (const char *sv = std::getenv("FFM_FEW_MAX")) sw.few_max = std::max(kSmallMax, std::min(kFewCap, std::atoi(sv)));
   if (const char *sv = std::getenv("FFM_OWN_SORT")) sw.own_sort = std::atoi(sv) != 0;
   if (const char *sv = std::getenv("FFM_RANGE_SORT")) sw.range_sort = std::atoi(sv);
   return sw;
@@ -146,6 +147,7 @@
   take(m.super_min, sw.super_min);
   m.few_stage = 1;
   take(m.few_stage, sw.few_stage);
+  m.few_max = kSmallMax;
   m.lat_fmt = (cfg->flags & FFM_FLAG_SERVE_F32 ? SERVE_F32 : 0) | (cfg->flags & FFM_FLAG_SERVE_F16 ? SERVE_F16 : 0);
   m.rec_slots = m.n_fields;
   e->n_records = cfg->n_feats;
@@ -366,6 +368,13 @@
   return FFM_OK;
 }
 
+static void choose_few_max(ffm_engine *e, const Switches &sw) {
+  ModelDev &m = e->m;
+  if (m.type != FFM_MODEL_FFM || m.n_factors % 4 != 0 || m.n_fields > 64 || !few_stage_possible(m)) return;
+  m.few_max = kFewMaxStaged;
+  take(m.few_max, sw.few_max);
+}
+
 static int read_verdict(ffm_engine *e, int *bad) {
   int *counters = e->sc[0].counters;
   HIP_TRY(hipMemcpyAsync(bad, counters, sizeof(int), hipMemcpyDeviceToHost, e->stream));
@@ -422,7 +431,7 @@
   for (int nf = 1; nf <= 4; nf *= 2)
     for (int kinds = 1; kinds <= UPD_ALL; kinds++)
       for (int waves : {tile_waves(nf), kWideWaves})
-        if ((rc = lds_opt_in(update_all_fn(nf, kinds, waves), tile_lds_bytes(nf, waves)))) return rc;
+        if ((rc = lds_opt_in(update_all_fn(nf, kinds, waves), update_lds_bytes(e->m, kinds, nf, waves)))) return rc;
   return FFM_OK;
 }
 
@@ -463,7 +472,9 @@
     return rc;
   for (int si = 0; si < ffm_engine::kSets; si++)
     if ((rc = alloc_set(e, si, shared))) return rc;
-  if ((rc = choose_sort(e, sw)) || (rc = prove_fast_math(e)) || (rc = opt_in_lds(e)) || (rc = init_weights(e))) return rc;
+  if ((rc = choose_sort(e, sw))) return rc;
+  choose_few_max(e, sw);
+  if ((rc = prove_fast_math(e)) || (rc = opt_in_lds(e)) || (rc = init_weights(e))) return rc;
   if (sw.metrics && cfg->shard_rank == 0)
     if ((rc = ffm_engine_metrics_enable(e, sw.metrics))) return rc;
   *out = guard.release();
diff --git a/ftrl-ffm_amd/csrc/engine_step.h b/ftrl-ffm_amd/csrc/engine_step.h
--- a/ftrl-ffm_amd/csrc/engine_step.h
+++ b/ftrl-ffm_amd/csrc/engine_step.h
@@ -314,7 +314,7 @@
     const bool wide = nf == 1 && !side_launches && split == 0 && rows.nnz < e->wide_max_nnz;
     const int wpb = wide ? kWideWaves : tile_waves(nf), scale = wpb / kUpdWaves, threads = 64 * wpb;
     const size_t lds = tile_lds_bytes(nf, wpb);
-    const size_t few_lds = few_stage_possible(e->m) ? few_stage_bytes(wpb, e->m.n_fields) : 0;
+    const size_t few_lds = few_stage_fits(e->m, wpb) ? few_stage_bytes(wpb, e->m.n_fields, e->m.few_max) : 0;
     auto sized = [&](int grid, int per_wg, int least) { return std::max(least, std::min(grid, cdiv(rows.nnz, per_wg))); };
     const int nt = cdiv(sized(e->grid_hot, 32, 64), scale), ns = flat ? 0 : cdiv(sized(e->grid_small, 128, 64), scale);
     const int nw = cdiv(sized(e->grid_walk, 1024, 16), scale);
@@ -323,6 +323,7 @@
     const int lb = loss_sum_out ? loss_grid(rows.n_rows) : 0;
     const int side = side_blocks > 0 ? 1 + cdiv(lin_blocks, scale) : 0;
     auto launch_ranges = [&](hipStream_t st, int kid, int kinds, size_t shm, int ord) {
+      if (kinds & UPD_FEW) shm = std::max(shm, few_lds);
       const int a_side = kinds & UPD_SIDE ? side : 0, a_ng = kinds & UPD_GIANT ? ng : 0, a_nt = kinds & UPD_HOT ? nt : 0;
       const int a_ns = kinds & UPD_FEW ? ns : 0, a_nw = kinds & UPD_REST ? nw : 0, a_lb = kinds & UPD_REST ? lb : 0;
       LAUNCH_ON(e, st, kid, update_all_fn(nf, kinds, wpb), a_side + a_ng + a_nt + a_ns + a_nw + a_lb, threads, shm, e->m, rows,
diff --git a/ftrl-ffm_amd/csrc/engine_types.h b/ftrl-ffm_amd/csrc/engine_types.h
--- a/ftrl-ffm_amd/csrc/engine_types.h
+++ b/ftrl-ffm_amd/csrc/engine_types.h
@@ -39,6 +39,7 @@
   const int *sort_start;
   int range_len;
   int few_stage;
+  int few_max;
   int lat_fmt;
 };
 
@@ -158,6 +159,8 @@
 #define FFM_SMALL_MAX 10
 #endif
 constexpr int kSmallMax = FFM_SMALL_MAX;
+constexpr int kFewCap = 32;
+static_assert(kSmallMax <= kSeg && kFewCap >= kSmallMax && kFewCap <= 64, "lane j of the owning wave fetches touch j");
 enum { ERR_ROW_TOO_LONG = 1, ERR_FIELD_MAP = 2, ERR_SORT_BARRIER = 4 };
 
 }
diff --git a/ftrl-ffm_amd/csrc/kernels_fold.h b/ftrl-ffm_amd/csrc/kernels_fold.h
--- a/ftrl-ffm_amd/csrc/kernels_fold.h
+++ b/ftrl-ffm_amd/csrc/kernels_fold.h
@@ -151,14 +151,28 @@
   a.any = a.any | lv;
 }
 
-template <int E>
+template <int E, bool MULTI = false>
 struct FoldFew {
   float P[E], G[E], D[E], ncap[E];
+  float B[E], Gacc[E], Dacc[E];
   bool any, seen, head_plain;
-  __device__ __forceinline__ void init() {
-#pragma unroll
-    for (int i = 0; i < E; i++) { P[i] = G[i] = D[i] = -0.0f; ncap[i] = 0.0f; }
+  __device__ __forceinline__ void init(const float (&n0)[E]) {
+#pragma unroll
+    for (int i = 0; i < E; i++) {
+      P[i] = G[i] = D[i] = Gacc[i] = Dacc[i] = -0.0f;
+      ncap[i] = 0.0f;
+      B[i] = n0[i];
+    }
     any = seen = head_plain = false;
+  }
+  __device__ __forceinline__ void flush() {
+#pragma unroll
+    for (int i = 0; i < E; i++) {
+      B[i] = B[i] + P[i];
+      Gacc[i] = Gacc[i] + G[i];
+      Dacc[i] = Dacc[i] + D[i];
+      P[i] = G[i] = D[i] = -0.0f;
+    }
   }
   __device__ __forceinline__ void touch(const float (&n0)[E], const float (&w)[E], bool live, bool first,
                                         float tg, float x, const float (&vp)[E]) {
@@ -176,7 +190,7 @@
       seen = seen || flip;
 #pragma unroll
       for (int i = 0; i < E; i++) {
-        const float nt = n0[i] + P[i];
+        const float nt = (MULTI ? B[i] : n0[i]) + P[i];
         ncap[i] = flip ? nt : ncap[i];
         const float g1 = tg * w[i] * x;
         arg[i] = nt + (first ? gg[i] : g[i] * g1);
@@ -207,7 +221,7 @@
       bool need[E];
 #pragma unroll
       for (int i = 0; i < E; i++) {
-        const float nt = n0[i] + P[i];
+        const float nt = (MULTI ? B[i] : n0[i]) + P[i];
         ncap[i] = (q118 & !seen) ? nt : ncap[i];
         const float g1 = tg * w[i] * x;
         arg[i] = nt + g[i] * g1;
@@ -229,9 +243,10 @@
   }
   __device__ __forceinline__ bool finish(const Hyper &h, const float (&w)[E], float (&n)[E], float (&z)[E]) {
     float nT[E], sa[E], sb[E], S[E], q[E];
-#pragma unroll
-    for (int i = 0; i < E; i++) {
-      nT[i] = n[i] + P[i];
+    if (MULTI) flush();
+#pragma unroll
+    for (int i = 0; i < E; i++) {
+      nT[i] = MULTI ? B[i] : n[i] + P[i];
       sa[i] = seen ? ncap[i] : nT[i];
       sb[i] = n[i];
     }
@@ -242,13 +257,13 @@
     for (int i = 0; i < E; i++) {
       float t = -0.0f;
       t = head_plain ? t + (ra[i] - rb[i]) : t;
-      S[i] = t + D[i];
+      S[i] = t + (MULTI ? Dacc[i] : D[i]);
     }
     div_alpha_n<E>(h, S, q);
 #pragma unroll
     for (int i = 0; i < E; i++) {
       if (any) {
-        z[i] = (z[i] + G[i]) - q[i] * w[i];
+        z[i] = (z[i] + (MULTI ? Gacc[i] : G[i])) - q[i] * w[i];
         n[i] = nT[i];
       }
     }
diff --git a/ftrl-ffm_amd/csrc/kernels_group.h b/ftrl-ffm_amd/csrc/kernels_group.h
--- a/ftrl-ffm_amd/csrc/kernels_group.h
+++ b/ftrl-ffm_amd/csrc/kernels_group.h
@@ -147,7 +147,7 @@
     p = s.occ[t];
     const int r = s.row_of[p];
     s.occ2[t] = make_int2(p, r);
-    s.occpos[p] = c > kSmallMax ? t : (c == 1 ? OCC_ONCE : OCC_FEW);
+    s.occpos[p] = c > m.few_max ? t : (c == 1 ? OCC_ONCE : OCC_FEW);
     dup = (!head && s.row_of[s.occ[t - 1]] == r) || (!last && s.row_of[s.occ[t + 1]] == r);
     if (dup) atomicOr(&s.uflag[lower], UF_DUP);
   }
@@ -155,8 +155,8 @@
   __shared__ int wave_cnt[kFinishThreads / 64][kLists];
   __shared__ int wave_base[kFinishThreads / 64][kLists];
   const int wv = threadIdx.x >> 6;
-  const bool pred[kLists] = {head, head && c <= kSmallMax, head && c > 1 && c <= kSmallMax,
-                             head && c > kSmallMax && c <= m.huge_min,
+  const bool pred[kLists] = {head, head && c <= m.few_max, head && c > 1 && c <= m.few_max,
+                             head && c > m.few_max && c <= m.huge_min,
                              head && c > m.huge_min && c < m.giant_min, head && c == 1,
                              head && c > m.huge_min && c >= m.giant_min};
   const int which[kLists] = {CNT_NUNIQ, CNT_NSMALL, CNT_NFEW, CNT_NBIG, CNT_NHUGE, CNT_NSINGLE, CNT_NGIANT};
@@ -184,8 +184,8 @@
     const int fld = rows.field ? rows.field[p] : 0;
     s.udesc[u] = make_int4(static_cast<int>(K), t, c, fld);
     if (c == 1) s.sdesc[slot[5]] = make_int4(static_cast<int>(K), p, s.row_of[p], fld);
-    if (c > 1 && c <= kSmallMax) s.few[iw] = u;
-    if (c <= kSmallMax) s.small[is] = u;
+    if (c > 1 && c <= m.few_max) s.few[iw] = u;
+    if (c <= m.few_max) s.small[is] = u;
     else if (c <= m.huge_min) s.big[ib] = u;
     else if (c < m.giant_min) s.huge[ih] = u;
     else {
diff --git a/ftrl-ffm_amd/csrc/kernels_tile.h b/ftrl-ffm_amd/csrc/kernels_tile.h
--- a/ftrl-ffm_amd/csrc/kernels_tile.h
+++ b/ftrl-ffm_amd/csrc/kernels_tile.h
@@ -575,9 +575,14 @@
   return static_cast<size_t>(waves) * (kTileT * kTileRow * sizeof(float) + kTileNR * kTileT * 4 * nf * sizeof(float4));
 }
 constexpr size_t tile_lds_bytes(int nf) { return tile_lds_bytes(nf, tile_waves(nf)); }
-static_assert(few_stage_bytes(1, 64) <= tile_lds_bytes(1, 1), "the few-occurrence range's staging fits a wave's tile region");
+static_assert(few_stage_bytes(1, 64, kSmallMax) <= tile_lds_bytes(1, 1), "the few-occurrence range's staging fits a wave's tile region");
+enum { UPD_GIANT = 1, UPD_HOT = 2, UPD_FEW = 4, UPD_SIDE = 8, UPD_REST = 16, UPD_ALL = 31 };
+inline size_t update_lds_bytes(const ModelDev &m, int kinds, int nf, int waves) {
+  const size_t tiles = tile_lds_bytes(nf, waves);
+  const size_t stage = (kinds & UPD_FEW) && few_stage_fits(m, waves) ? few_stage_bytes(waves, m.n_fields, m.few_max) : 0;
+  return tiles > stage ? tiles : stage;
+}
 constexpr int kWideWaves = 8;
-enum { UPD_GIANT = 1, UPD_HOT = 2, UPD_FEW = 4, UPD_SIDE = 8, UPD_REST = 16, UPD_ALL = 31 };
 #ifndef FFM_OCC_ALL
 #define FFM_OCC_ALL 0
 #endif
@@ -631,7 +636,7 @@
       ffm_tile_items<NF>(m, rows, s, r * WAVES + wv, nt * WAVES, T, R);
     }
   } else if (kind == 2) {
-    if (KINDS & UPD_FEW) ffm_small_body(m, rows, s, few_only, r, ns, few_stage_possible(m) ? reinterpret_cast<int2 *>(lds_dyn) : nullptr);
+    if (KINDS & UPD_FEW) ffm_small_body(m, rows, s, few_only, r, ns, few_stage_fits(m, WAVES) ? reinterpret_cast<int2 *>(lds_dyn) : nullptr);
   }
   if (kind >= 0) return;
   if (KINDS & UPD_REST) {
diff --git a/ftrl-ffm_amd/csrc/kernels_update.h b/ftrl-ffm_amd/csrc/kernels_update.h
--- a/ftrl-ffm_amd/csrc/kernels_update.h
+++ b/ftrl-ffm_amd/csrc/kernels_update.h
@@ -46,6 +46,7 @@
       Fold a;
       a.init(n);
       for (int t = 0; t < c; t++) {
+        if (t == kSeg) a.flush();
         const int2 pr = s.occ2[start + t];
         a.plain(true, s.tg[pr.y] * rows.val[pr.x]);
       }
@@ -329,28 +330,33 @@
 #define FFM_SMALL_BATCH 4
 #endif
 constexpr int kSmallBatch = FFM_SMALL_BATCH < kSmallMax ? FFM_SMALL_BATCH : kSmallMax;
-constexpr int kSmallPad = (kSmallMax + kSmallBatch - 1) / kSmallBatch * kSmallBatch;
-static_assert(kSmallPad % kSmallBatch == 0 && kSmallPad >= kSmallMax && kSmallPad < kSmallMax + kSmallBatch,
-              "the per-touch arrays of the few-occurrence range hold kSmallMax rounded up to whole batches");
+__host__ __device__ constexpr int few_pad(int few_max) { return (few_max + kSmallBatch - 1) / kSmallBatch * kSmallBatch; }
+constexpr int kSmallPad = few_pad(kFewCap);
 static_assert(kSmallPad <= 64, "lane j of the owning wave fetches touch j");
+#ifndef FFM_FEW_MAX_STAGED
+#define FFM_FEW_MAX_STAGED 10
+#endif
+constexpr int kFewMaxStaged = FFM_FEW_MAX_STAGED;
+static_assert(kFewMaxStaged >= kSmallMax && kFewMaxStaged <= kFewCap, "the boundary moves between kSmallMax and kFewCap");
 #ifndef FFM_STAGE_FLY
 #define FFM_STAGE_FLY 7
 #endif
 constexpr int kStageFly = FFM_STAGE_FLY;
-constexpr size_t few_stage_bytes(int waves, int n_fields) {
-  return static_cast<size_t>(waves) * kSmallPad * static_cast<size_t>(n_fields) * sizeof(int2);
+constexpr size_t kFewStageMaxBytes = 64 * 1024;
+__host__ __device__ constexpr size_t few_stage_bytes(int waves, int n_fields, int few_max) {
+  return static_cast<size_t>(waves) * few_pad(few_max) * static_cast<size_t>(n_fields) * sizeof(int2);
 }
 __host__ __device__ inline bool few_stage_possible(const ModelDev &m) {
   return m.few_stage != 0 && m.sort_start != nullptr && m.n_shards == 1 && m.own_n == nullptr &&
          m.field_start == nullptr && m.h.learn == 0 && m.rec_slots * (m.n_factors >> 2) > 64;
+}
+__host__ __device__ inline bool few_stage_fits(const ModelDev &m, int waves) {
+  return few_stage_possible(m) && few_stage_bytes(waves, m.n_fields, m.few_max) <= kFewStageMaxBytes;
 }
 #ifdef FFM_SMALL_WAVES
 #define FFM_SMALL_OCC __attribute__((amdgpu_waves_per_eu(FFM_SMALL_WAVES, FFM_SMALL_WAVES)))
 #else
 #define FFM_SMALL_OCC
-#endif
-#ifndef FFM_FEW_LDS
-#define FFM_FEW_LDS 1
 #endif
 #ifndef FFM_FOLD_REGULAR
 #define FFM_FOLD_REGULAR 1
@@ -383,7 +389,6 @@
     const int fa = ud.w;
     float4 *rec4 = reinterpret_cast<float4 *>(staged ? m.lat + static_cast<long long>(i) * 3 * RL : lat_row(m, i, fa));
     const unsigned long long cm = s.cmask[start];
-#if FFM_FEW_LDS
     {
       int2 pr = make_int2(0, 0);
       if (lane < c) pr = s.occ2[start + lane];
@@ -432,30 +437,11 @@
 #define FEW_TFM(j) (facts[j].z)
 #define FEW_TXM(j) (__int_as_float(facts[j].w))
 #define FEW_TTG(j) (tgs[j])
-#else
-    int tp[kSmallPad], tr[kSmallPad], tfm[kSmallPad];
-    float txm[kSmallPad], ttg[kSmallPad];
-#pragma unroll
-    for (int j = 0; j < kSmallPad; j++) {
-      tp[j] = tr[j] = tfm[j] = 0;
-      txm[j] = ttg[j] = 0.0f;
-      if (j < c) {
-        const int2 pr = s.occ2[start + j];
-        tp[j] = wave_uniform(pr.x);
-        tr[j] = wave_uniform(pr.y);
-        tfm[j] = wave_uniform(rows.field[tp[j]]);
-        txm[j] = __int_as_float(wave_uniform(__float_as_int(rows.val[tp[j]])));
-        ttg[j] = __int_as_float(wave_uniform(__float_as_int(s.tg[tr[j]])));
-      }
-    }
-#define FEW_TP(j) (tp[j])
-#define FEW_TR(j) (tr[j])
-#define FEW_TFM(j) (tfm[j])
-#define FEW_TXM(j) (txm[j])
-#define FEW_TTG(j) (ttg[j])
-#endif
-    auto passes = [&](auto staged_tag) {
+    auto passes = [&](auto staged_tag, auto multi_tag) {
     constexpr bool STAGED = decltype(staged_tag)::value;
+    constexpr bool MULTI = decltype(multi_tag)::value;
+    constexpr int BATCH = MULTI && !STAGED ? 2 : kSmallBatch;
+    static_assert(kSeg % BATCH == 0, "a segment of the fold ends between two batches");
     for (int l0 = 0; l0 < span4; l0 += 64) {
       const int l = l0 + lane;
       const int lc = l < span4 ? l : 0;
@@ -474,17 +460,17 @@
         z[0] = z4.x; z[1] = z4.y; z[2] = z4.z; z[3] = z4.w;
         w[0] = w4.x; w[1] = w4.y; w[2] = w4.z; w[3] = w4.w;
       }
-      FoldFew<4> a;
-      a.init();
+      FoldFew<4, MULTI> a;
+      a.init(n);
       const bool lv = mine && fp != fa, q118 = lv && !m.h.learn && fp < fa;
-#pragma unroll
-      for (int j0 = 0; j0 < kSmallMax; j0 += kSmallBatch) {
-        if (j0 >= c) break;
-        float4 vp4[kSmallBatch];
+#pragma unroll 1
+      for (int j0 = 0; j0 < c; j0 += BATCH) {
+        if (MULTI && j0 > 0 && j0 % kSeg == 0) a.flush();
+        float4 vp4[BATCH];
         if constexpr (STAGED) {
-          float xp[kSmallBatch];
-#pragma unroll
-          for (int jj = 0; jj < kSmallBatch; jj++) {
+          float xp[BATCH];
+#pragma unroll
+          for (int jj = 0; jj < BATCH; jj++) {
             const int j = j0 + jj;
             xp[jj] = 0.0f;
             vp4[jj] = make_float4(0.0f, 0.0f, 0.0f, 0.0f);
@@ -495,7 +481,7 @@
             }
           }
 #pragma unroll
-          for (int jj = 0; jj < kSmallBatch; jj++) {
+          for (int jj = 0; jj < BATCH; jj++) {
             const int j = j0 + jj;
             if (j >= c) continue;
             const float vp[4] = {vp4[jj].x, vp4[jj].y, vp4[jj].z, vp4[jj].w};
@@ -503,22 +489,22 @@
           }
           continue;
         }
-        int4 rt[kSmallBatch];
-#pragma unroll
-        for (int jj = 0; jj < kSmallBatch; jj++) {
+        int4 rt[BATCH];
+#pragma unroll
+        for (int jj = 0; jj < BATCH; jj++) {
           const int j = j0 + jj;
           rt[jj] = make_int4(0, 0, -1, 0);
           if (mine && j < c && owns_bit(own_bits, FEW_TFM(j))) rt[jj] = s.rowtab[static_cast<int64_t>(FEW_TR(j)) * F + fp];
         }
 #pragma unroll
-        for (int jj = 0; jj < kSmallBatch; jj++) {
+        for (int jj = 0; jj < BATCH; jj++) {
           const int j = j0 + jj;
           vp4[jj] = make_float4(0.0f, 0.0f, 0.0f, 0.0f);
           if (j < c && rt[jj].z >= 0 && rt[jj].z != FEW_TP(j))
             vp4[jj] = reinterpret_cast<const float4 *>(lat_row(m, rt[jj].x, fp))[LAT_W * RL4 + slot_of(m, fp, FEW_TFM(j)) * k4 + kq];
         }
 #pragma unroll
-        for (int jj = 0; jj < kSmallBatch; jj++) {
+        for (int jj = 0; jj < BATCH; jj++) {
           const int j = j0 + jj;
           if (j >= c) continue;
           const int p = FEW_TP(j), q = rt[jj].z;
@@ -537,11 +523,15 @@
       }
     }
     };
-    if (staged) passes(std::true_type{});
-    else passes(std::false_type{});
-#if FFM_FEW_LDS
+    if (c > kSeg) {
+      if (staged) passes(std::true_type{}, std::true_type{});
+      else passes(std::false_type{}, std::true_type{});
+    } else if (staged) {
+      passes(std::true_type{}, std::false_type{});
+    } else {
+      passes(std::false_type{}, std::false_type{});
+    }
     __builtin_amdgcn_fence(__ATOMIC_RELEASE, "wavefront");
-#endif
   }
 #undef FEW_TP
 #undef FEW_TR
@@ -551,24 +541,18 @@
 }
 __device__ __forceinline__ void ffm_small_body(const ModelDev &m, const Rows &rows, const Scratch &s,
                                                int few_only, unsigned bidx, unsigned gdim, int2 *stage_all = nullptr) {
-#if FFM_FEW_LDS
   __shared__ int4 few_facts[kUpdMaxThreads / 64][kSmallPad];
   __shared__ float few_tg[kUpdMaxThreads / 64][kSmallPad];
   const int wv_in_block = wave_uniform(threadIdx.x >> 6);
   int4 *facts = few_facts[wv_in_block];
   float *tgs = few_tg[wv_in_block];
-#else
-  const int wv_in_block = 0;
-  int4 *facts = nullptr;
-  float *tgs = nullptr;
-#endif
 #if FFM_FOLD_REGULAR
   const bool regular = m.sort_start != nullptr && m.n_shards == 1 && m.own_n == nullptr && s.counters[CNT_IRREGULAR] == 0;
 #else
   const bool regular = false;
 #endif
-  const bool staged = FFM_FEW_LDS && regular && stage_all != nullptr && few_stage_possible(m);
-  int2 *stage = staged ? stage_all + static_cast<size_t>(wv_in_block) * kSmallPad * m.n_fields : nullptr;
+  const bool staged = regular && stage_all != nullptr && few_stage_fits(m, blockDim.x >> 6);
+  int2 *stage = staged ? stage_all + static_cast<size_t>(wv_in_block) * few_pad(m.few_max) * m.n_fields : nullptr;
   ffm_small_items(staged, m, rows, s, few_only, bidx, gdim, regular, facts, tgs, stage);
 }
 __global__ __launch_bounds__(kUpdThreads) FFM_SMALL_OCC void ffm_update_small_kernel(ModelDev m, Rows rows,
@@ -618,7 +602,7 @@
       w[0] = w4.x; w[1] = w4.y; w[2] = w4.z; w[3] = w4.w;
     }
     FoldFew<4> a;
-    a.init();
+    a.init(n);
     for (int j0 = 0; j0 < kSmallMax; j0 += kFlatBatch) {
       if (!__any(mine && j0 < c)) break;
       int2 pr[kFlatBatch];
diff --git a/ftrl-ffm_amd/engine.py b/ftrl-ffm_amd/engine.py
--- a/ftrl-ffm_amd/engine.py
+++ b/ftrl-ffm_amd/engine.py
@@ -91,6 +91,7 @@
     ("ffm_engine_abi_version", ctypes.c_int, []),
     ("ffm_engine_block_segment", ctypes.c_int, []),
     ("ffm_engine_row_len", ctypes.c_int64, [_vp]),
+    ("ffm_engine_few_max", ctypes.c_int, [_vp]),
     ("ffm_engine_default_batch_ramp", ctypes.c_int32, [ctypes.c_float]),
     ("ffm_engine_shard_plan", ctypes.c_int,
      [ctypes.c_int32, ctypes.c_int32, ctypes.c_int32, _i32p, _i32p, _i32p]),
@@ -465,6 +466,9 @@
         self.n_feats, self.n_fields, self.n_factors = cfg.n_feats, cfg.n_fields, cfg.n_factors
         self.row_len = int(self.lib.ffm_engine_row_len(self.h))
 
+    def few_max(self):
+        return int(self.lib.ffm_engine_few_max(self.h))
+
     def _check(self, rc):
         if rc != 0:
             raise EngineError(rc, self.lib.ffm_engine_last_error().decode())
diff --git a/include/ffm_engine.h b/include/ffm_engine.h
--- a/include/ffm_engine.h
+++ b/include/ffm_engine.h
@@ -71,6 +71,7 @@
 int32_t ffm_engine_default_batch_ramp(float w_alpha);
 
 int64_t ffm_engine_row_len(const ffm_engine *e);
+int ffm_engine_few_max(const ffm_engine *e);
 
 int ffm_engine_set_weights(ffm_engine *e, const float *bias, const float *lin_w, const float *vec_w);
 int ffm_engine_get_weights(ffm_engine *e, float *bias, float *lin_w, float *vec_w);
```

New measurement: 10.25 million samples/s. Within noise of the previous version (-0.0%).
